# taylorlu/voicepuppet

Measured on AMD Instinct MI355X. Metric: PixReferNet G+D step frames/sec @256x256 bs=32, higher is better.
Workload: dtype bf16; 1 GPU; PixReferNet G+D training step (G + 3xD + VGG16-conv3_3 perceptual + TF-Adam x2), 256x256, ngf=ndf=64, global batch 32 = 32 per GPU; global_batch=32, per_gpu_batch=32, parallelism=dp1

## Files before the change

include/vp_hip.h:

```cpp
#ifndef VP_HIP_H_
#define VP_HIP_H_

#include <stddef.h>
#include <stdint.h>

#ifdef __cplusplus
extern "C" {
#endif

enum vp_status { VP_OK = 0, VP_ERR_ARG = -1, VP_ERR_HIP = -2, VP_ERR_WORKSPACE = -3, VP_ERR_STATE = -4 };
enum vp_dtype { VP_F32 = 0, VP_BF16 = 1 };
enum vp_act { VP_ACT_NONE = 0, VP_ACT_LRELU = 1, VP_ACT_RELU = 2, VP_ACT_TANH = 3, VP_ACT_SIGMOID = 4, VP_ACT_RELU6 = 5, VP_ACT_LEAKY = 6 };

int vp_version(void);
const char* vp_last_error(void);

typedef struct vp_pixrefer_desc {
  int batch;
  int height;
  int ngf, ndf;
  int dtype;
  int training;
  float l1_weight;
  float gan_weight;
  int per_sample_bn;
  int streams;
  int d_backward_fork;
  int d_beside_vgg;
} vp_pixrefer_desc;

size_t vp_pixrefer_desc_size(void);

typedef struct vp_pixrefer vp_pixrefer_t;

size_t vp_pixrefer_param_count(const vp_pixrefer_desc* d, int which);
int vp_pixrefer_param_info(const vp_pixrefer_desc* d, int which, int index, char* name, int name_cap,
                           size_t* offset, int* ndim, int64_t shape[4]);

size_t vp_pixrefer_workspace_bytes(const vp_pixrefer_desc* d);
int vp_pixrefer_validate_plan(const vp_pixrefer_desc* d);

int vp_pixrefer_create(const vp_pixrefer_desc* d, void* workspace, size_t workspace_bytes,
                       float* params_g, float* params_d, const float* params_vgg,
                       float* grads_g, float* grads_d, void* stream, vp_pixrefer_t** out);
void vp_pixrefer_destroy(vp_pixrefer_t* h);

int vp_pixrefer_params_changed(vp_pixrefer_t* h);
int vp_pixrefer_optimizer_stepped(vp_pixrefer_t* h);

int vp_pixrefer_forward(vp_pixrefer_t* h, const float* inputs, const float* fg_inputs,
                        const float* targets, const float* masks, void* stream);

int vp_pixrefer_forward_fg3(vp_pixrefer_t* h, const float* inputs, const float* fg_inputs3, const float* targets, void* stream);

int vp_pixrefer_backward(vp_pixrefer_t* h, void* stream);
int vp_pixrefer_backward_update(vp_pixrefer_t* h, float* m_g, float* v_g, float* m_d, float* v_d, int step_t_g, int step_t_d,
                                float lr, float beta1, float beta2, float eps, void* stream);

int vp_pixrefer_backward_d(vp_pixrefer_t* h, void* stream);
int vp_pixrefer_backward_g(vp_pixrefer_t* h, void* stream);
int vp_pixrefer_backward_d_fork(vp_pixrefer_t* h, void* stream);
int vp_pixrefer_backward_d_join(vp_pixrefer_t* h, void* stream);
void* vp_pixrefer_side_stream(vp_pixrefer_t* h);
int vp_reserve_streams(void);
void* vp_host_stream(void);
int vp_pixrefer_use_streams(vp_pixrefer_t* h, int n);
int vp_pixrefer_set_option(vp_pixrefer_t* h, const char* key, int value);
long long vp_pixrefer_counter(vp_pixrefer_t* h, const char* key);
int vp_pixrefer_fetch(vp_pixrefer_t* h, int what, void* dst, void* stream);
int vp_pixrefer_backward_g_stages(void);
int vp_pixrefer_backward_g_stage(vp_pixrefer_t* h, int stage, void* stream);
int vp_pixrefer_update_bucket(vp_pixrefer_t* h, int which, int bucket, float* m, float* v, int step_t, float lr, float beta1,
                              float beta2, float eps, void* stream);

int vp_pixrefer_tensor(vp_pixrefer_t* h, const char* name, void** ptr, int64_t shape[4], int* dtype);

int vp_profile_enable(int on);
size_t vp_profile_collect(char* json, size_t cap);

int vp_pixrefer_pack_frames(const unsigned char* example_frames, const unsigned char* current_frames, const int* crops,
                            int n, int img_size, float* inputs, float* fg_inputs, float* targets, float* masks, void* stream);

int vp_tune(const char* key, int value);
int vp_pixrefer_phase_ms(vp_pixrefer_t* h, float* ms, int cap);
float vp_pixrefer_mark_ms(vp_pixrefer_t* h, int from, int to);

int vp_grad_pack_bf16(const float* src, void* dst_bf16, size_t n, void* stream);
int vp_grad_unpack_bf16(const void* src_bf16, float* dst, size_t n, float scale, void* stream);

int vp_adam_tf(float* params, const float* grads, float* m, float* v, size_t n, int step_t,
               float lr, float beta1, float beta2, float eps, void* stream);

typedef struct vp_conv_desc {
  int kind;
  int n, h, w;
  int cin, cout;
  int ksize, stride, pad;
  int dtype;
  int in_act;
  int out_act;
} vp_conv_desc;

size_t vp_conv_workspace_bytes(const vp_conv_desc* d);
int vp_conv_fwd(const vp_conv_desc* d, const void* x, const float* in_scale, const float* in_shift,
                const float* w, const float* bias, void* y, void* workspace, void* stream);
int vp_conv_bwd_data(const vp_conv_desc* d, const void* dy, const float* w, void* dx, void* workspace, void* stream);
size_t vp_conv3x3_c64_bwd_data_pooled_workspace_bytes(const vp_conv_desc* d);
int vp_conv3x3_c64_bwd_data_pooled(const vp_conv_desc* d, const void* dy_pool, const unsigned char* code, const float* w, const void* ref,
                                   void* dx, void* workspace, int fused, void* stream);
int vp_conv_bwd_weight(const vp_conv_desc* d, const void* x, const float* in_scale, const float* in_shift,
                       const void* dy, float* dw, void* workspace, void* stream);

size_t vp_bn_workspace_bytes(int pixels, int c, int dtype);
int vp_bn_stats(const void* y, int pixels, int c, int dtype, const float* gamma, const float* beta, float eps,
                float* scale, float* shift, float* mean, float* rstd, void* workspace, void* stream);
int vp_bn_bwd(const void* y, const void* dz, void* dy, int pixels, int c, int dtype, const float* gamma,
              const float* mean, const float* rstd, float* dgamma, float* dbeta, void* workspace, void* stream);

typedef struct vp_logmel_desc {
  int sample_rate, num_mel_bins, win_length, hop_step, fft_length;
  float lower_hz, upper_hz;
  int batch, samples;
} vp_logmel_desc;
typedef struct vp_logmel vp_logmel_t;
size_t vp_logmel_workspace_bytes(const vp_logmel_desc* d);
int vp_logmel_frames(const vp_logmel_desc* d);
int vp_logmel_create(const vp_logmel_desc* d, void* workspace, size_t workspace_bytes, void* stream, vp_logmel_t** out);
void vp_logmel_destroy(vp_logmel_t* h);
int vp_logmel_forward(vp_logmel_t* h, const float* pcm, float* out, void* stream);

typedef struct vp_bfmnet_desc {
  int batch;
  int frames;
  int num_mel_bins;
  int trunk_dtype;
} vp_bfmnet_desc;
typedef struct vp_bfmnet vp_bfmnet_t;
size_t vp_bfmnet_param_count(void);
int vp_bfmnet_param_info(int index, char* name, int name_cap, size_t* offset, int* ndim, int64_t shape[4]);
size_t vp_bfmnet_workspace_bytes(const vp_bfmnet_desc* d);
int vp_bfmnet_create(const vp_bfmnet_desc* d, void* workspace, size_t workspace_bytes, const float* params,
                     void* stream, vp_bfmnet_t** out);
void vp_bfmnet_destroy(vp_bfmnet_t* h);
int vp_bfmnet_params_changed(vp_bfmnet_t* h);
int vp_bfmnet_forward(vp_bfmnet_t* h, const float* ears, const float* mfccs, const int* seq_len, float* out, void* stream);
int vp_bfmnet_set_decoder_dropout(vp_bfmnet_t* h, const float* mask0, const float* mask1);
int vp_bfmnet_tensor(vp_bfmnet_t* h, const char* name, void** ptr, int64_t shape[4]);

typedef struct vp_bfmstream_desc {
  int struct_bytes;
  int max_chunk_frames;
  int num_mel_bins;
  int trunk_dtype;
  int sample_rate;
  float lower_hz, upper_hz;
} vp_bfmstream_desc;
size_t vp_bfmstream_desc_size(void);
typedef struct vp_bfmstream vp_bfmstream_t;
int vp_bfmstream_context(const vp_bfmstream_desc* d, int* left_mel, int* right_mel, int* left_frames, int* right_frames, int* window_frames);
long long vp_bfmstream_frames_after(const vp_bfmstream_desc* d, long long samples, int finished);
size_t vp_bfmstream_workspace_bytes(const vp_bfmstream_desc* d);
int vp_bfmstream_create(const vp_bfmstream_desc* d, void* workspace, size_t workspace_bytes, const float* params, void* stream,
                        vp_bfmstream_t** out);
void vp_bfmstream_destroy(vp_bfmstream_t* h);
int vp_bfmstream_params_changed(vp_bfmstream_t* h);
int vp_bfmstream_reset(vp_bfmstream_t* h, void* stream);
int vp_bfmstream_ready(const vp_bfmstream_t* h, long long n_new_samples);
int vp_bfmstream_ready_finish(const vp_bfmstream_t* h);
int vp_bfmstream_push(vp_bfmstream_t* h, const float* pcm, long long n, const float* ears, float* coeff_out, void* stream);
int vp_bfmstream_finish(vp_bfmstream_t* h, const float* ears, float* coeff_out, void* stream);
int vp_bfmstream_tensor(vp_bfmstream_t* h, const char* name, void** ptr, int64_t shape[4]);
#define VP_BFMSTREAM_GROUP_MAX_SLOTS 128
typedef struct vp_bfmstream_group_desc {
  int struct_bytes;
  int slots;
  int max_chunk_frames;
  int num_mel_bins;
  int trunk_dtype;
  int sample_rate;
  float lower_hz, upper_hz;
} vp_bfmstream_group_desc;
size_t vp_bfmstream_group_desc_size(void);
typedef struct vp_bfmstream_group vp_bfmstream_group_t;
size_t vp_bfmstream_group_workspace_bytes(const vp_bfmstream_group_desc* d);
int vp_bfmstream_group_plan_info(const vp_bfmstream_group_desc* d, int bucket, int gemm, int info[8]);
int vp_bfmstream_group_create(const vp_bfmstream_group_desc* d, void* workspace, size_t workspace_bytes, const float* params, void* stream,
                              vp_bfmstream_group_t** out);
void vp_bfmstream_group_destroy(vp_bfmstream_group_t* h);
int vp_bfmstream_group_params_changed(vp_bfmstream_group_t* h);
// ... 379 lines not shown
```

voicepuppet_amd/_lib.py:

```python
import ctypes
import os

_HERE = os.path.dirname(os.path.abspath(__file__))
LIB_PATH = os.environ.get("VP_LIB", os.path.join(_HERE, "libvp_hip.so"))

VP_F32, VP_BF16 = 0, 1
ACT_NONE, ACT_LRELU, ACT_RELU, ACT_TANH, ACT_SIGMOID = 0, 1, 2, 3, 4
BN_PATH_PLANNER, BN_PATH_TWO_PASS, BN_PATH_ONE_LAUNCH = 0, 1, 2


class PixReferDesc(ctypes.Structure):
  _fields_ = [("batch", ctypes.c_int), ("height", ctypes.c_int), ("ngf", ctypes.c_int), ("ndf", ctypes.c_int),
              ("dtype", ctypes.c_int), ("training", ctypes.c_int), ("l1_weight", ctypes.c_float),
              ("gan_weight", ctypes.c_float), ("per_sample_bn", ctypes.c_int),
              ("streams", ctypes.c_int), ("d_backward_fork", ctypes.c_int), ("d_beside_vgg", ctypes.c_int)]


class ConvDesc(ctypes.Structure):
  _fields_ = [("kind", ctypes.c_int), ("n", ctypes.c_int), ("h", ctypes.c_int), ("w", ctypes.c_int),
              ("cin", ctypes.c_int), ("cout", ctypes.c_int), ("ksize", ctypes.c_int), ("stride", ctypes.c_int),
              ("pad", ctypes.c_int), ("dtype", ctypes.c_int), ("in_act", ctypes.c_int), ("out_act", ctypes.c_int)]


class LogMelDesc(ctypes.Structure):
  _fields_ = [("sample_rate", ctypes.c_int), ("num_mel_bins", ctypes.c_int), ("win_length", ctypes.c_int),
              ("hop_step", ctypes.c_int), ("fft_length", ctypes.c_int), ("lower_hz", ctypes.c_float),
              ("upper_hz", ctypes.c_float), ("batch", ctypes.c_int), ("samples", ctypes.c_int)]


class BfmNetDesc(ctypes.Structure):
  _fields_ = [("batch", ctypes.c_int), ("frames", ctypes.c_int), ("num_mel_bins", ctypes.c_int), ("trunk_dtype", ctypes.c_int)]


class BfmStreamDesc(ctypes.Structure):
  _fields_ = [("struct_bytes", ctypes.c_int), ("max_chunk_frames", ctypes.c_int), ("num_mel_bins", ctypes.c_int),
              ("trunk_dtype", ctypes.c_int), ("sample_rate", ctypes.c_int), ("lower_hz", ctypes.c_float), ("upper_hz", ctypes.c_float)]


class BfmStreamGroupDesc(ctypes.Structure):
  _fields_ = [("struct_bytes", ctypes.c_int), ("slots", ctypes.c_int), ("max_chunk_frames", ctypes.c_int), ("num_mel_bins", ctypes.c_int),
              ("trunk_dtype", ctypes.c_int), ("sample_rate", ctypes.c_int), ("lower_hz", ctypes.c_float), ("upper_hz", ctypes.c_float)]


BFMSTREAM_GROUP_MAX_SLOTS = 128


class PuppetDesc(ctypes.Structure):
  _fields_ = [("struct_bytes", ctypes.c_int), ("slots", ctypes.c_int), ("frame_batch", ctypes.c_int), ("img_size", ctypes.c_int),
              ("face_size", ctypes.c_int)]


PUPPET_MAX_SLOTS = 128


class JpegDesc(ctypes.Structure):
  _fields_ = [("struct_bytes", ctypes.c_uint32), ("max_frames", ctypes.c_int32), ("height", ctypes.c_int32), ("width", ctypes.c_int32),
              ("quality", ctypes.c_int32)]


class PngDesc(ctypes.Structure):
  _fields_ = [("struct_bytes", ctypes.c_uint32), ("max_frames", ctypes.c_int32), ("height", ctypes.c_int32), ("width", ctypes.c_int32),
              ("channels", ctypes.c_int32), ("filter", ctypes.c_int32)]


PNG_U8, PNG_F32 = 0, 1


class JpegDecDesc(ctypes.Structure):
  _fields_ = [("struct_bytes", ctypes.c_uint32), ("max_files", ctypes.c_int32), ("max_height", ctypes.c_int32), ("max_width", ctypes.c_int32),
              ("max_file_bytes", ctypes.c_int32), ("max_segments_per_file", ctypes.c_int32), ("bgr", ctypes.c_int32)]


class JpegDecFile(ctypes.Structure):
  _fields_ = [("meta_offset", ctypes.c_uint64), ("file_offset", ctypes.c_uint64), ("file_bytes", ctypes.c_int32), ("width", ctypes.c_int32),
              ("height", ctypes.c_int32), ("sampling", ctypes.c_int32), ("restart_interval", ctypes.c_int32), ("n_segments", ctypes.c_int32),
              ("tq", ctypes.c_uint8 * 3), ("td", ctypes.c_uint8 * 3), ("ta", ctypes.c_uint8 * 3), ("reserved", ctypes.c_uint8 * 3)]


JPEGDEC_META_BYTES = 6336


class PcmInDesc(ctypes.Structure):
  _fields_ = [("struct_bytes", ctypes.c_int), ("slots", ctypes.c_int), ("out_rate", ctypes.c_int), ("max_in_frames", ctypes.c_int),
              ("n_rates", ctypes.c_int), ("rates", ctypes.c_int * 8)]


PCMIN_MAX_SLOTS, PCMIN_MAX_CHANNELS = 128, 8
PCM_S16, PCM_F32 = 0, 1


class FrameMetricsDesc(ctypes.Structure):
  _fields_ = [("struct_bytes", ctypes.c_uint32), ("max_frames", ctypes.c_int32), ("max_height", ctypes.c_int32), ("max_width", ctypes.c_int32)]


FRAME_METRICS_MAX_FRAMES = 4096


class AviMuxDesc(ctypes.Structure):
  _fields_ = [("struct_bytes", ctypes.c_uint32), ("max_frames", ctypes.c_int32), ("row_bytes", ctypes.c_int32), ("slots", ctypes.c_int32),
              ("max_samples", ctypes.c_int32)]


AVIMUX_MAX_FRAMES, AVIMUX_MAX_SLOTS = 4096, 128


class TriptychDesc(ctypes.Structure):
  _fields_ = [("struct_bytes", ctypes.c_uint32), ("max_frames", ctypes.c_int32), ("size", ctypes.c_int32), ("face_size", ctypes.c_int32),
              ("max_side", ctypes.c_int32)]


TRIPTYCH_MAX_FRAMES, TRIPTYCH_MAX_SIZE = 4096, 1024


class BfmObserveOpts(ctypes.Structure):
  _fields_ = [("struct_bytes", ctypes.c_uint32), ("visibility", ctypes.c_int32), ("raster_scale", ctypes.c_int32), ("prefilter", ctypes.c_int32),
              ("depth_tol", ctypes.c_float)]


class BfmModel(ctypes.Structure):
  _fields_ = [("nver", ctypes.c_int), ("ntri", ctypes.c_int), ("meanshape", ctypes.c_void_p), ("idBase", ctypes.c_void_p),
              ("exBase", ctypes.c_void_p), ("meantex", ctypes.c_void_p), ("texBase", ctypes.c_void_p), ("tri", ctypes.c_void_p),
              ("point_buf", ctypes.c_void_p), ("center", ctypes.c_double * 3), ("focal", ctypes.c_double),
              ("image_center", ctypes.c_double), ("sh", ctypes.c_double * 5)]


_P = ctypes.c_void_p
_SIGNATURES = {
    "vp_version": (ctypes.c_int, []),
    "vp_last_error": (ctypes.c_char_p, []),
    "vp_pixrefer_param_count": (ctypes.c_size_t, [ctypes.POINTER(PixReferDesc), ctypes.c_int]),
    "vp_pixrefer_param_info": (ctypes.c_int, [ctypes.POINTER(PixReferDesc), ctypes.c_int, ctypes.c_int, ctypes.c_char_p,
                                              ctypes.c_int, ctypes.POINTER(ctypes.c_size_t), ctypes.POINTER(ctypes.c_int),
                                              ctypes.POINTER(ctypes.c_int64)]),
    "vp_pixrefer_workspace_bytes": (ctypes.c_size_t, [ctypes.POINTER(PixReferDesc)]),
    "vp_pixrefer_validate_plan": (ctypes.c_int, [ctypes.POINTER(PixReferDesc)]),
    "vp_pixrefer_create": (ctypes.c_int, [ctypes.POINTER(PixReferDesc), _P, ctypes.c_size_t, _P, _P, _P, _P, _P, _P,
                                          ctypes.POINTER(_P)]),
    "vp_pixrefer_destroy": (None, [_P]),
    "vp_pixrefer_params_changed": (ctypes.c_int, [_P]),
    "vp_pixrefer_optimizer_stepped": (ctypes.c_int, [_P]),
    "vp_pixrefer_forward": (ctypes.c_int, [_P, _P, _P, _P, _P, _P]),
    "vp_pixrefer_forward_fg3": (ctypes.c_int, [_P, _P, _P, _P, _P]),
    "vp_pixrefer_desc_size": (ctypes.c_size_t, []),
    "vp_pixrefer_backward": (ctypes.c_int, [_P, _P]),
    "vp_pixrefer_backward_update": (ctypes.c_int, [_P, _P, _P, _P, _P, ctypes.c_int, ctypes.c_int, ctypes.c_float, ctypes.c_float,
                                                   ctypes.c_float, ctypes.c_float, _P]),
    "vp_pixrefer_backward_d": (ctypes.c_int, [_P, _P]),
    "vp_pixrefer_backward_g": (ctypes.c_int, [_P, _P]),
    "vp_pixrefer_backward_d_fork": (ctypes.c_int, [_P, _P]),
    "vp_pixrefer_backward_d_join": (ctypes.c_int, [_P, _P]),
    "vp_pixrefer_backward_g_stages": (ctypes.c_int, []),
    "vp_pixrefer_backward_g_stage": (ctypes.c_int, [_P, ctypes.c_int, _P]),
    "vp_pixrefer_side_stream": (ctypes.c_void_p, [_P]),
    "vp_pixrefer_use_streams": (ctypes.c_int, [_P, ctypes.c_int]),
    "vp_pixrefer_set_option": (ctypes.c_int, [_P, ctypes.c_char_p, ctypes.c_int]),
    "vp_pixrefer_fetch": (ctypes.c_int, [_P, ctypes.c_int, _P, _P]),
    "vp_pixrefer_counter": (ctypes.c_longlong, [_P, ctypes.c_char_p]),
    "vp_crc32c": (ctypes.c_uint, [_P, ctypes.c_size_t, ctypes.c_uint]),
    "vp_pixrefer_phase_ms": (ctypes.c_int, [_P, ctypes.POINTER(ctypes.c_float), ctypes.c_int]),
    "vp_grad_pack_bf16": (ctypes.c_int, [_P, _P, ctypes.c_size_t, _P]),
    "vp_grad_unpack_bf16": (ctypes.c_int, [_P, _P, ctypes.c_size_t, ctypes.c_float, _P]),
    "vp_pixrefer_update_bucket": (ctypes.c_int, [_P, ctypes.c_int, ctypes.c_int, _P, _P, ctypes.c_int, ctypes.c_float, ctypes.c_float, ctypes.c_float,
                                                 ctypes.c_float, _P]),
    "vp_resize_paste_workspace_bytes": (ctypes.c_size_t, [ctypes.c_int, ctypes.c_int]),
    "vp_resize_paste_u8": (ctypes.c_int, [_P, ctypes.c_int, ctypes.c_int, ctypes.c_int, ctypes.c_int, ctypes.c_int, ctypes.c_int, _P, ctypes.c_int,
                                          ctypes.c_int, ctypes.c_int, ctypes.c_int, _P, _P]),
    "vp_resize_linear_table": (ctypes.c_int, [ctypes.c_int, ctypes.c_int, ctypes.c_int, _P, _P, _P, _P]),
    "vp_mm_workspace_bytes": (ctypes.c_size_t, [ctypes.c_int, ctypes.c_int, ctypes.c_int]),
    "vp_mm_fwd_f32": (ctypes.c_int, [_P, ctypes.c_int, _P, ctypes.c_int, ctypes.c_int, _P, _P, ctypes.c_int, ctypes.c_int, ctypes.c_int, ctypes.c_int, _P, _P]),
    "vp_mm_bwd_data_f32": (ctypes.c_int, [_P, ctypes.c_int, _P, ctypes.c_int, ctypes.c_int, _P, ctypes.c_int, ctypes.c_int, ctypes.c_int, ctypes.c_int,
                                          ctypes.c_int, _P, _P]),
    "vp_mm_bwd_weight_f32": (ctypes.c_int, [_P, ctypes.c_int, _P, ctypes.c_int, _P, ctypes.c_int, ctypes.c_int, ctypes.c_int, ctypes.c_int, _P, _P]),
    "vp_mm_packed_bytes": (ctypes.c_size_t, [ctypes.c_int, ctypes.c_int, ctypes.c_int, ctypes.c_int]),
    "vp_mm_pack_desc_bytes": (ctypes.c_size_t, []),
    "vp_mm_pack_desc": (ctypes.c_int, [ctypes.c_size_t, ctypes.c_int, ctypes.c_int, ctypes.c_int, ctypes.c_int, ctypes.c_int, ctypes.c_int, ctypes.c_size_t, _P]),
    "vp_mm_pack_table": (ctypes.c_int, [_P, ctypes.c_int, _P, _P, _P]),
    "vp_mm_fwd_f32_packed": (ctypes.c_int, [_P, ctypes.c_int, _P, _P, _P, ctypes.c_int, ctypes.c_int, ctypes.c_int, ctypes.c_int, _P, _P]),
    "vp_mm_bwd_data_f32_packed": (ctypes.c_int, [_P, ctypes.c_int, _P, _P, ctypes.c_int, ctypes.c_int, ctypes.c_int, ctypes.c_int, ctypes.c_int, _P, _P]),
    "vp_pixrefer_mark_ms": (ctypes.c_float, [_P, ctypes.c_int, ctypes.c_int]),
    "vp_profile_enable": (ctypes.c_int, [ctypes.c_int]),
    "vp_tune": (ctypes.c_int, [ctypes.c_char_p, ctypes.c_int]),
    "vp_reserve_streams": (ctypes.c_int, []),
    "vp_host_stream": (ctypes.c_void_p, []),
    "vp_pixrefer_pack_frames": (ctypes.c_int, [_P, _P, _P, ctypes.c_int, ctypes.c_int, _P, _P, _P, _P, _P]),
    "vp_profile_collect": (ctypes.c_size_t, [ctypes.c_char_p, ctypes.c_size_t]),
    "vp_pixrefer_tensor": (ctypes.c_int, [_P, ctypes.c_char_p, ctypes.POINTER(_P), ctypes.POINTER(ctypes.c_int64),
                                          ctypes.POINTER(ctypes.c_int)]),
    "vp_adam_tf": (ctypes.c_int, [_P, _P, _P, _P, ctypes.c_size_t, ctypes.c_int, ctypes.c_float, ctypes.c_float,
                                  ctypes.c_float, ctypes.c_float, _P]),
    "vp_conv_workspace_bytes": (ctypes.c_size_t, [ctypes.POINTER(ConvDesc)]),
    "vp_conv_fwd": (ctypes.c_int, [ctypes.POINTER(ConvDesc), _P, _P, _P, _P, _P, _P, _P, _P]),
    "vp_conv_bwd_data": (ctypes.c_int, [ctypes.POINTER(ConvDesc), _P, _P, _P, _P, _P]),
    "vp_conv_bwd_weight": (ctypes.c_int, [ctypes.POINTER(ConvDesc), _P, _P, _P, _P, _P, _P, _P]),
    "vp_conv3x3_c64_bwd_data_pooled_workspace_bytes": (ctypes.c_size_t, [ctypes.POINTER(ConvDesc)]),
    "vp_conv3x3_c64_bwd_data_pooled": (ctypes.c_int, [ctypes.POINTER(ConvDesc), _P, _P, _P, _P, _P, _P, ctypes.c_int, _P]),
    "vp_bn_workspace_bytes": (ctypes.c_size_t, [ctypes.c_int, ctypes.c_int, ctypes.c_int]),
    "vp_bn_stats": (ctypes.c_int, [_P, ctypes.c_int, ctypes.c_int, ctypes.c_int, _P, _P, ctypes.c_float, _P, _P, _P, _P, _P, _P]),
    "vp_logmel_workspace_bytes": (ctypes.c_size_t, [ctypes.POINTER(LogMelDesc)]),
    "vp_logmel_frames": (ctypes.c_int, [ctypes.POINTER(LogMelDesc)]),
    "vp_logmel_create": (ctypes.c_int, [ctypes.POINTER(LogMelDesc), _P, ctypes.c_size_t, _P, ctypes.POINTER(_P)]),
    "vp_logmel_destroy": (None, [_P]),
    "vp_logmel_forward": (ctypes.c_int, [_P, _P, _P, _P]),
    "vp_bfmnet_param_count": (ctypes.c_size_t, []),
    "vp_bfmnet_param_info": (ctypes.c_int, [ctypes.c_int, ctypes.c_char_p, ctypes.c_int, ctypes.POINTER(ctypes.c_size_t),
                                            ctypes.POINTER(ctypes.c_int), ctypes.POINTER(ctypes.c_int64)]),
    "vp_bfmnet_workspace_bytes": (ctypes.c_size_t, [ctypes.POINTER(BfmNetDesc)]),
    "vp_bfmnet_create": (ctypes.c_int, [ctypes.POINTER(BfmNetDesc), _P, ctypes.c_size_t, _P, _P, ctypes.POINTER(_P)]),
    "vp_bfmnet_destroy": (None, [_P]),
    "vp_bfmnet_params_changed": (ctypes.c_int, [_P]),
    "vp_bfmnet_forward": (ctypes.c_int, [_P, _P, _P, _P, _P, _P]),
    "vp_bfmnet_set_decoder_dropout": (ctypes.c_int, [_P, _P, _P]),
    "vp_bfmnet_tensor": (ctypes.c_int, [_P, ctypes.c_char_p, ctypes.POINTER(_P), ctypes.POINTER(ctypes.c_int64)]),
    "vp_bfmstream_desc_size": (ctypes.c_size_t, []),
    "vp_bfmstream_context": (ctypes.c_int, [ctypes.POINTER(BfmStreamDesc)] + [ctypes.POINTER(ctypes.c_int)] * 5),
    "vp_bfmstream_frames_after": (ctypes.c_longlong, [ctypes.POINTER(BfmStreamDesc), ctypes.c_longlong, ctypes.c_int]),
    "vp_bfmstream_workspace_bytes": (ctypes.c_size_t, [ctypes.POINTER(BfmStreamDesc)]),
    "vp_bfmstream_create": (ctypes.c_int, [ctypes.POINTER(BfmStreamDesc), _P, ctypes.c_size_t, _P, _P, ctypes.POINTER(_P)]),
    "vp_bfmstream_destroy": (None, [_P]),
    "vp_bfmstream_params_changed": (ctypes.c_int, [_P]),
    "vp_bfmstream_reset": (ctypes.c_int, [_P, _P]),
    "vp_bfmstream_ready": (ctypes.c_int, [_P, ctypes.c_longlong]),
    "vp_bfmstream_ready_finish": (ctypes.c_int, [_P]),
    "vp_bfmstream_push": (ctypes.c_int, [_P, _P, ctypes.c_longlong, _P, _P, _P]),
    "vp_bfmstream_finish": (ctypes.c_int, [_P, _P, _P, _P]),
    "vp_bfmstream_tensor": (ctypes.c_int, [_P, ctypes.c_char_p, ctypes.POINTER(_P), ctypes.POINTER(ctypes.c_int64)]),
    "vp_bfmstream_group_desc_size": (ctypes.c_size_t, []),
    "vp_puppet_desc_size": (ctypes.c_size_t, []),
    "vp_puppet_workspace_bytes": (ctypes.c_size_t, [ctypes.POINTER(PuppetDesc)]),
    "vp_puppet_create": (ctypes.c_int, [ctypes.POINTER(PuppetDesc), _P, ctypes.c_size_t, _P, ctypes.POINTER(_P)]),
    "vp_puppet_destroy": (None, [_P]),
    "vp_puppet_attach": (ctypes.c_int, [_P, ctypes.c_int, _P, _P, _P, ctypes.c_int, ctypes.c_int, ctypes.c_int, _P]),
    "vp_puppet_set_backgrounds": (ctypes.c_int, [_P, _P, ctypes.c_int]),
    "vp_puppet_splice": (ctypes.c_int, [_P, _P, ctypes.c_int, _P, ctypes.c_int, _P, _P]),
    "vp_puppet_condition": (ctypes.c_int, [_P, _P, ctypes.c_int, _P, ctypes.c_int, _P, _P, _P, _P]),
    "vp_puppet_tensor": (ctypes.c_int, [_P, ctypes.c_char_p, ctypes.POINTER(_P), ctypes.POINTER(ctypes.c_int64)]),
    "vp_puppet_slot_info": (ctypes.c_int, [_P, ctypes.c_int, ctypes.POINTER(ctypes.c_int)]),
    "vp_jpeg_desc_size": (ctypes.c_size_t, []),
    "vp_jpeg_workspace_bytes": (ctypes.c_size_t, [ctypes.POINTER(JpegDesc)]),
    "vp_jpeg_frame_capacity": (ctypes.c_size_t, [ctypes.POINTER(JpegDesc)]),
    "vp_jpeg_create": (ctypes.c_int, [ctypes.POINTER(JpegDesc), _P, ctypes.c_size_t, _P, ctypes.POINTER(_P)]),
    "vp_jpeg_encode": (ctypes.c_int, [_P, _P, ctypes.c_int, _P, ctypes.c_size_t, _P, _P]),
    "vp_jpeg_tensor": (ctypes.c_int, [_P, ctypes.c_char_p, ctypes.POINTER(_P), ctypes.POINTER(ctypes.c_int64)]),
    "vp_jpeg_header": (ctypes.c_int, [_P, _P, ctypes.c_size_t, ctypes.POINTER(ctypes.c_size_t)]),
    "vp_jpeg_destroy": (None, [_P]),
    "vp_png_desc_size": (ctypes.c_size_t, []),
    "vp_png_workspace_bytes": (ctypes.c_size_t, [ctypes.POINTER(PngDesc)]),
    "vp_png_frame_capacity": (ctypes.c_size_t, [ctypes.POINTER(PngDesc)]),
    "vp_png_rows_per_strip": (ctypes.c_int, [ctypes.POINTER(PngDesc)]),
    "vp_png_create": (ctypes.c_int, [ctypes.POINTER(PngDesc), _P, ctypes.c_size_t, _P, ctypes.POINTER(_P)]),
    "vp_png_encode": (ctypes.c_int, [_P, _P, ctypes.c_int, ctypes.c_int, ctypes.c_int, ctypes.c_int, _P, ctypes.c_size_t, _P, _P]),
    "vp_png_tensor": (ctypes.c_int, [_P, ctypes.c_char_p, ctypes.POINTER(_P), ctypes.POINTER(ctypes.c_int64)]),
    "vp_png_header": (ctypes.c_int, [_P, _P, ctypes.c_size_t, ctypes.POINTER(ctypes.c_size_t)]),
    "vp_png_destroy": (None, [_P]),
    "vp_jpegdec_desc_size": (ctypes.c_size_t, []),
    "vp_jpegdec_workspace_bytes": (ctypes.c_size_t, [ctypes.POINTER(JpegDecDesc)]),
    "vp_jpegdec_create": (ctypes.c_int, [ctypes.POINTER(JpegDecDesc), _P, ctypes.c_size_t, ctypes.POINTER(_P)]),
    "vp_jpegdec_destroy": (None, [_P]),
    "vp_jpegdec_decode": (ctypes.c_int, [_P, _P, ctypes.POINTER(JpegDecFile), ctypes.c_int, _P, ctypes.c_size_t, ctypes.c_size_t, _P, _P]),
    "vp_jpegdec_tensor": (ctypes.c_int, [_P, ctypes.c_char_p, ctypes.POINTER(_P), ctypes.POINTER(ctypes.c_int64)]),
    "vp_jpegdec_scan_workspace_bytes": (ctypes.c_size_t, [ctypes.POINTER(JpegDecDesc), ctypes.c_int]),
    "vp_jpegdec_enable_scan": (ctypes.c_int, [_P, _P, ctypes.c_size_t, ctypes.c_int, ctypes.c_int]),
    "vp_pcmin_desc_size": (ctypes.c_size_t, []),
    "vp_pcmin_ratio": (ctypes.c_int, [ctypes.c_int, ctypes.c_int] + [ctypes.POINTER(ctypes.c_int)] * 4),
    "vp_pcmin_bank": (ctypes.c_int, [ctypes.c_int, ctypes.c_int, _P]),
    "vp_pcmin_samples_after": (ctypes.c_longlong, [ctypes.c_int, ctypes.c_int, ctypes.c_longlong, ctypes.c_int]),
    "vp_pcmin_workspace_bytes": (ctypes.c_size_t, [ctypes.POINTER(PcmInDesc)]),
    "vp_pcmin_create": (ctypes.c_int, [ctypes.POINTER(PcmInDesc), _P, ctypes.c_size_t, _P, ctypes.POINTER(_P)]),
    "vp_pcmin_destroy": (None, [_P]),
    "vp_pcmin_open_slot": (ctypes.c_int, [_P, ctypes.c_int, ctypes.c_int, ctypes.c_int, ctypes.c_int, _P]),
    "vp_pcmin_ready": (ctypes.c_longlong, [_P, ctypes.POINTER(ctypes.c_longlong), ctypes.POINTER(ctypes.c_int), ctypes.POINTER(ctypes.c_longlong)]),
    "vp_pcmin_push": (ctypes.c_int, [_P, _P, ctypes.POINTER(ctypes.c_longlong), ctypes.POINTER(ctypes.c_int), _P, _P]),
    "vp_frame_metrics_desc_size": (ctypes.c_size_t, []),
    "vp_frame_metrics_workspace_bytes": (ctypes.c_size_t, [ctypes.POINTER(FrameMetricsDesc)]),
    "vp_frame_metrics_create": (ctypes.c_int, [ctypes.POINTER(FrameMetricsDesc), _P, ctypes.c_size_t, ctypes.POINTER(_P)]),
    "vp_frame_metrics_destroy": (None, [_P]),
# ... 178 lines not shown
```

voicepuppet_amd/csrc/conv_dispatch.h:

```cpp
#pragma once
#include <hip/hip_runtime.h>

#include "conv_args.h"

namespace vp {

enum ProfBytes {
  BYTES_DEFAULT,
  BYTES_ONE_CLASS,
  BYTES_F32_OUT,
};
constexpr int TILE_FROM_CFG = 0, TILE_ROWS_COUT = -1;

struct ConvKernelRow {
  int id;
  const char* name;
  int family;
  bool bf16_only;
  int& (*knob)();
  bool (*eligible)(const IgemmArgs&, int is_bf16);
  hipError_t (*launch)(const IgemmArgs&, int is_bf16, int cfg, hipStream_t);
  int prof_bc, prof_bp;
  ProfBytes prof_bytes;
};

const char* conv_kernel_name(int kern);
int conv_staging(int kern);
bool conv_kernel_ok(const IgemmArgs& a, int is_bf16);
int pick_conv_kernel(const IgemmArgs& v, int is_bf16);
hipError_t launch_igemm(const IgemmArgs& a, int is_bf16, int cfg, hipStream_t st);

}
```

voicepuppet_amd/csrc/conv_dispatch.hip:

```cpp
#include "conv_dispatch.h"

#include "conv_ops.h"
#include "conv_prof.h"
#include "errors.h"
#include "vp_common.h"

namespace vp {

typedef const IgemmArgs& Args;
hipError_t launch_igemm_generic(Args, int is_bf16, int cfg, hipStream_t);
hipError_t launch_igemm_patch(Args, int is_bf16, int bc, int bp, hipStream_t);
hipError_t launch_igemm_patch2(Args, int is_bf16, int bc, int bp, hipStream_t);
bool patch3_eligible(Args, int is_bf16); hipError_t launch_igemm_patch3(Args, int is_bf16, int bc, int bp, hipStream_t);
bool patch4_eligible(Args, int is_bf16); hipError_t launch_igemm_patch4(Args, hipStream_t);
hipError_t launch_igemm_smallp(Args, int is_bf16, hipStream_t);
bool conv_s2c64_eligible(Args, int is_bf16); hipError_t launch_conv_s2c64(Args, hipStream_t);
bool conv_cin8_eligible(Args, int is_bf16); hipError_t launch_conv_cin8(Args, hipStream_t);
bool conv_cout8_eligible(Args, int is_bf16); hipError_t launch_conv_cout8(Args, hipStream_t);
bool conv_dcout8_eligible(Args, int is_bf16); hipError_t launch_conv_dcout8(Args, hipStream_t);
bool conv_cout4_eligible(Args, int is_bf16); hipError_t launch_conv_cout4(Args, hipStream_t);
bool conv_c64_eligible(Args, int is_bf16); hipError_t launch_conv_c64(Args, hipStream_t);
bool conv_dc256_eligible(Args, int is_bf16); hipError_t launch_conv_dc256(Args, hipStream_t);
bool conv_dc64_eligible(Args, int is_bf16); hipError_t launch_conv_dc64(Args, hipStream_t);

#define VP_TILED(fn) [](Args a, int bf, int cfg, hipStream_t st) { int bc, bp; igemm_tile(cfg, &bc, &bp); return fn(a, bf, bc, bp, st); }
#define VP_BF16(fn) [](Args a, int, int, hipStream_t st) { return fn(a, st); }

static const ConvKernelRow kTable[] = {
    {CK_SMALLP, "smallp", CK_SMALLP, false, nullptr, nullptr, [](Args a, int bf, int, hipStream_t st) { return launch_igemm_smallp(a, bf, st); },
     TILE_FROM_CFG, 0, BYTES_DEFAULT},
    {CK_S2C64, "s2c64", CK_S2C64, true, nullptr, conv_s2c64_eligible, VP_BF16(launch_conv_s2c64), 128, 64, BYTES_DEFAULT},
    {CK_CIN8, "cin8", CK_IGEMM, true, nullptr, conv_cin8_eligible, VP_BF16(launch_conv_cin8), 64, 16, BYTES_ONE_CLASS},
    {CK_COUT8, "cout8", CK_IGEMM, true, nullptr, conv_cout8_eligible, VP_BF16(launch_conv_cout8), 16, 64, BYTES_ONE_CLASS},
    {CK_DCOUT8, "dcout8", CK_IGEMM, true, nullptr, conv_dcout8_eligible, VP_BF16(launch_conv_dcout8), 32, 64, BYTES_DEFAULT},
    {CK_COUT4, "cout4", CK_IGEMM, true, nullptr, conv_cout4_eligible, VP_BF16(launch_conv_cout4), 16, 16, BYTES_F32_OUT},
    {CK_C64, "c64", CK_PATCH, true, c64_knob, conv_c64_eligible, VP_BF16(launch_conv_c64), TILE_ROWS_COUT, 64, BYTES_DEFAULT},
    {CK_DC256, "dc256", CK_PATCH2, true, dc64_knob, conv_dc256_eligible, VP_BF16(launch_conv_dc256), 64, 128, BYTES_DEFAULT},
    {CK_DC64, "dc64", CK_PATCH2, true, dc64_knob, conv_dc64_eligible, VP_BF16(launch_conv_dc64), 64, 128, BYTES_DEFAULT},
    {CK_PATCH4, "patch4", CK_PATCH, true, patch4_knob, patch4_eligible, VP_BF16(launch_igemm_patch4), 128, 256, BYTES_DEFAULT},
    {CK_PATCH3, "patch3", CK_PATCH, false, patch3_knob, patch3_eligible, VP_TILED(launch_igemm_patch3), TILE_FROM_CFG, 0, BYTES_DEFAULT},
    {CK_PATCH, "patch", CK_PATCH, false, nullptr, nullptr, VP_TILED(launch_igemm_patch), TILE_FROM_CFG, 0, BYTES_DEFAULT},
    {CK_PATCH2, "patch2", CK_PATCH2, false, nullptr, nullptr, VP_TILED(launch_igemm_patch2), TILE_FROM_CFG, 0, BYTES_DEFAULT},
    {CK_IGEMM, "igemm", CK_IGEMM, false, nullptr, nullptr, launch_igemm_generic, TILE_FROM_CFG, 0, BYTES_DEFAULT},
};
#undef VP_TILED
#undef VP_BF16

static const ConvKernelRow* conv_kernel_row(int kern) {
  for (const ConvKernelRow& r : kTable) if (r.id == kern) return &r;
  return nullptr;
}
const char* conv_kernel_name(int kern) { const ConvKernelRow* r = conv_kernel_row(kern); return r ? r->name : "?"; }
int conv_staging(int kern) { const ConvKernelRow* r = conv_kernel_row(kern); return r ? r->family : CK_IGEMM; }

bool conv_kernel_ok(const IgemmArgs& a, int is_bf16) {
  if (a.pool_src && a.kern != CK_C64) return false;
  const ConvKernelRow* r = conv_kernel_row(a.kern);
  if (!r || (r->bf16_only && !is_bf16)) return false;
  return !r->eligible || r->eligible(a, is_bf16);
}

int pick_conv_kernel(const IgemmArgs& v, int is_bf16) {
  const int fam = conv_staging(v.kern);
  for (const ConvKernelRow& r : kTable) {
    if (r.id == r.family) { if (r.id == fam) return fam; continue; }
    if ((r.bf16_only && !is_bf16) || (r.knob && !r.knob())) continue;
    if (r.eligible(v, is_bf16)) return r.id;
  }
  return fam;
}

hipError_t launch_igemm(const IgemmArgs& a, int is_bf16, int cfg, hipStream_t st) {
  if (!conv_kernel_ok(a, is_bf16)) {
    set_err("launch_igemm: the arguments are outside the preconditions of the plan's kernel %s (%s, %d x %d x %d -> %d channels)",
            conv_kernel_name(a.kern), is_bf16 ? "bf16" : "f32", a.N, a.Hg, a.Wg, a.Cout);
    return hipErrorInvalidValue;
  }
  const ConvKernelRow& r = *conv_kernel_row(a.kern);
  int pbc = r.prof_bc, pbp = r.prof_bp;
  if (pbc == TILE_FROM_CFG) igemm_tile(cfg, &pbc, &pbp);
  else if (pbc == TILE_ROWS_COUT) pbc = a.Cout;
  const double Pn = (double)a.N * a.Hg * a.Wg * a.nclass;
  const double kreal = (double)a.ntaps * a.cin_real;
  const double es = is_bf16 ? 2 : 4;
  const double flops = 2.0 * Pn * a.Cout * kreal;
  const double xfull = (double)a.N * a.Hin * a.Win * a.cin_real;
  double bytes;
  if (r.prof_bytes == BYTES_ONE_CLASS) bytes = es * (xfull + kreal * a.Cout + Pn * a.Cout);
  else if (r.prof_bytes == BYTES_F32_OUT) bytes = es * (xfull + kreal * a.nclass * a.Cout) + 4.0 * Pn * a.Cout;
  else {
    const double xbytes = a.pool_src ? (es + 1) * ((double)a.N * (a.Hin / 2) * (a.Win / 2) * a.cin_real) : es * xfull;
    bytes = xbytes + es * (kreal * a.nclass * a.Cout + Pn * a.Cout);
  }
  ProfScope prof(r.name, is_bf16, pbc, pbp, flops, bytes, st);
  return r.launch(a, is_bf16, cfg, st);
}

}
```

voicepuppet_amd/csrc/conv_ops.h:

```cpp
#pragma once
#include <stdlib.h>
#include <string.h>

#include "launch.h"

namespace vp {

struct ConvGeomX : ConvGeom {
  int CoutT;
};

inline ConvGeomX make_geom(int kind, int ks, int stride, int pad, int N, int Hin, int Win, int Cin, int Cin_real, int Cout) {
  ConvGeomX g;
  g.kind = kind; g.ks = ks; g.stride = stride; g.pad = pad;
  g.N = N; g.Hin = Hin; g.Win = Win;
  if (kind == 0) { g.Hout = (Hin + 2 * pad - ks) / stride + 1; g.Wout = (Win + 2 * pad - ks) / stride + 1; }
  else { g.Hout = 2 * Hin; g.Wout = 2 * Win; }
  g.Cin = Cin; g.Cin_real = Cin_real; g.Cout = Cout;
  g.CoutT = Cout < 8 ? 8 : Cout;
  return g;
}

inline int kc_elems(int is_bf16) { return is_bf16 ? 32 : 16; }

inline int& wgrad_cost_knob(int i) { static int v[3] = {80, 15, 150}; return v[i]; }
inline int& plan_misc_knob(int i) { static int v[4] = {384, 8, 4, 512}; return v[i]; }
inline int& igemm_small_grid_knob() { static int v = 128; return v; }
inline int& thin_blocks_knob(int i) { static int v[4] = {1024, 512, 512, 512}; return v[i]; }

inline int pick_igemm_cfg(int rows, int P, int Kpad = 0) {
  if (P >= 96) {
    if (rows % 128 == 0 && igemm_small_grid_knob() > 0 && (long long)((P + 127) / 128) * (rows / 128) <= igemm_small_grid_knob()) return IG_64x128;
    if (rows % 256 == 0 && P >= 256 * 256 && Kpad >= 4096) return IG_256x256;
    if (rows % 128 == 0 && P >= 256 * 512) return IG_128x256;
    if (rows % 128 == 0) return IG_128x128;
    if (rows % 64 == 0) return IG_64x128;
    if (rows <= 16) return IG_16x128;
    return rows > 64 ? IG_128x128 : IG_64x128;
  }
  if (rows <= 64) return IG_64x32;
  return P > 16 ? IG_128x32 : IG_128x16;
}

constexpr int IGEMM_SPLITK_TARGET_DEFAULT = 64;
inline int& igemm_splitk_target_knob() { static int v = IGEMM_SPLITK_TARGET_DEFAULT; return v; }
inline int pick_igemm_splitk(int blocks, int nchunk) {
  const int target = igemm_splitk_target_knob();
  const int cap = plan_misc_knob(1);
  const int minchunk = plan_misc_knob(2);
  if (blocks >= 256 || blocks >= target) return 1;
  int s = (target + blocks - 1) / blocks;
  if (s > nchunk / minchunk) s = nchunk / minchunk;
  if (s > cap) s = cap;
  return s < 1 ? 1 : s;
}

inline void set_single_src(PixSrc& x, const void* p, int C, const float* a, const float* b, int act, int group_n) {
  x.ptr[0] = p; x.ptr[1] = nullptr; x.C[0] = C; x.C[1] = 0;
  x.aff_a[0] = a; x.aff_b[0] = b; x.aff_a[1] = nullptr; x.aff_b[1] = nullptr;
  x.act = act; x.group_n = group_n > 0 ? group_n : (1 << 30);
}

struct LaunchForm {
  bool bias = false, ref = false, xa_lrelu = false, xa_relu = false, x_affine = false;
  bool stats = false;
  int x_act = 0, ref_act = 0;
};

struct IgemmPlan {
  IgemmArgs a;
  int cfg;
  LaunchForm form;
  PackDesc pack;
  size_t pack_elems;
  size_t partial_bytes;
};

struct IgemmPin { int cfg, splitk; };

inline void finish_igemm(IgemmPlan& p, int rows, int is_bf16, const IgemmPin* pin = nullptr) {
  IgemmArgs& a = p.a;
  const int P = a.N * a.Hg * a.Wg;
  a.Kpad = round_up(a.ntaps * a.Cin, kc_elems(is_bf16));
  p.cfg = pick_igemm_cfg(rows, P, a.Kpad);
  if (!is_bf16 && a.ntaps == 1 && p.cfg == IG_128x128) {
    const long long b128 = (long long)((P + 127) / 128) * (rows / 128), b64 = 2 * b128;
    if (((b64 + 255) / 256) * 64 < ((b128 + 255) / 256) * 128) p.cfg = IG_64x128;
  }
  if (pin) p.cfg = pin->cfg;
  int bc, bp;
  igemm_tile(p.cfg, &bc, &bp);
  a.CoutPad = round_up(rows, bc);
  if (a.ntaps == 1) { a.log2Cin = 30; a.cin_mask = 0x3fffffff; }
  else { a.log2Cin = ilog2(a.Cin); a.cin_mask = a.Cin - 1; }
  const int blocks = ((P + bp - 1) / bp) * (a.CoutPad / bc) * a.nclass;
  a.splitk = pin ? pin->splitk : pick_igemm_splitk(blocks, a.Kpad / kc_elems(is_bf16));
  p.partial_bytes = a.splitk > 1 ? (size_t)a.nclass * a.splitk * P * a.CoutPad * sizeof(float) : 0;
  {
    const bool tc4 = p.cfg == IG_128x128 || p.cfg == IG_64x128 || p.cfg == IG_128x256 || p.cfg == IG_256x256;
    a.rowperm = (tc4 && rows % 64 == 0) ? 1 : 0;
    p.pack.perm = a.rowperm;
  }
  a.wp_rows = round_up(rows, 128);
  p.pack.rows_pad = a.wp_rows;
  p.pack.Kpad = a.Kpad;
  p.pack.kc = kc_elems(is_bf16);
  p.pack_elems = (size_t)a.nclass * a.wp_rows * a.Kpad;
}

inline int& patch_tiles_knob() { static int v = 7; return v; }
inline int& patch_small_knob() { static int v = 3; return v; }
inline int& patch_longk_knob() { static int v = 1; return v; }
inline int& patch3_knob() { static int v = 1; return v; }
inline int& wgrad_big_knob() { static int v = 1; return v; }
inline int& patch4_knob() { static int v = 1; return v; }
inline int& c64_knob() { static int v = 1; return v; }
inline int& pool_bwd_fused_knob() { static int v = 1; return v; }
inline int& cout1_knob() { static int v = 256; return v; }
inline int& wgrad1_rows_knob() { static int v = 512; return v; }
inline int& dc64_knob() { static int v = 1; return v; }
inline int& s2c64_knob() { static int v = 512; return v; }
inline int& s2c64_pair_knob() { static int v = 1; return v; }
constexpr int PATCH_MIN_BLOCKS_DEFAULT = 192;
inline int& patch_minblk_knob() { static int v = PATCH_MIN_BLOCKS_DEFAULT; return v; }

inline void patch_tile_hw(int bp, int* th, int* tw) { *th = bp == 128 ? 8 : 16; *tw = bp == 512 ? 32 : 16; }
inline int patch_tile_pixels(int bc) {
  const int k = patch_small_knob();
  if (bc == 256) return (k & 2) ? 128 : 256;
  return (k & 1) ? 256 : 512;
}

inline int patch_tile_rows(int rows, int on) {
  if ((on & 1) && rows % 256 == 0) return 256;
  if ((on & 2) && rows % 128 == 0) return 128;
  if ((on & 4) && rows % 64 == 0) return 64;
  return 0;
}

inline bool plan_patch_eligible(const IgemmPlan& p, int rows, int is_bf16, bool single_src, bool any_grid = false) {
  const int on = patch_tiles_knob();
  const int minblk = any_grid ? 0 : patch_minblk_knob();
  const IgemmArgs& a = p.a;
  const int kc = kc_elems(is_bf16);
  if (!on || !single_src || a.nclass != 1 || a.sh != 1 || a.sw != 1 || a.os != 1 || a.ntaps < 9 || a.Cin % kc || a.Cin < kc) return false;
  if (rows % 64 || a.Cout % 8 || a.ldY % 8 || a.Hg < 16 || a.Wg < 16 || a.Hof != a.Hg || a.Wof != a.Wg) return false;
  const bool p4 = patch4_knob() && is_bf16 && a.ntaps == 16 && rows % 128 == 0;
  if (!p4 && patch_longk_knob() && rows >= 512 && rows % 256 == 0 && a.ntaps * a.Cin >= 4096 && (long long)a.N * a.Hg * a.Wg >= 256 * 256) return false;
  const int bc = p4 ? 128 : patch_tile_rows(rows, on);
  if (!bc) return false;
  int th, tw;
  patch_tile_hw(p4 ? 256 : patch_tile_pixels(bc), &th, &tw);
  const long long blocks = (long long)a.N * ((a.Hg + th - 1) / th) * ((a.Wg + tw - 1) / tw) * (rows / bc);
  const long long p4min = (long long)a.ntaps * a.Cin >= 8192 ? 256 : 512;
  if (p4 && !any_grid && patch_minblk_knob() > 1) {
    if (blocks < p4min) return false;
  } else if (blocks < minblk) return false;
  if ((size_t)a.N * a.Hin * a.Win * a.Cin * (is_bf16 ? 2 : 4) >= 0x70000000ull) return false;
  int ks = 0;
  while (ks * ks < a.ntaps) ++ks;
  if (ks * ks != a.ntaps) return false;
  const int sh = a.taps[0].dh[ks] - a.taps[0].dh[0], sw = a.taps[0].dw[1] - a.taps[0].dw[0];
  if ((sh != 1 && sh != -1) || (sw != 1 && sw != -1)) return false;
  for (int t = 0; t < a.ntaps; ++t)
    if (a.taps[0].dh[t] != a.taps[0].dh[0] + (t / ks) * sh || a.taps[0].dw[t] != a.taps[0].dw[0] + (t % ks) * sw) return false;
  return true;
}
inline void plan_make_patch(IgemmPlan& p, int rows, int is_bf16) {
  IgemmArgs& a = p.a;
  const bool p4 = patch4_knob() && is_bf16 && a.ntaps == 16 && rows % 128 == 0;
  const int bc = p4 ? 128 : patch_tile_rows(rows, patch_tiles_knob());
  int ks = 0;
  while (ks * ks < a.ntaps) ++ks;
  a.kern = CK_PATCH; a.p_kw = ks;
  a.p_dhf = a.taps[0].dh[0]; a.p_dwf = a.taps[0].dw[0];
  a.p_dhs = a.taps[0].dh[ks] - a.taps[0].dh[0]; a.p_dws = a.taps[0].dw[1] - a.taps[0].dw[0];
  const int bp = p4 ? 256 : patch_tile_pixels(bc);
  p.cfg = bc == 256 ? (bp == 128 ? PATCH_256x128 : PATCH_256x256) : (bc == 128 ? (bp == 256 ? PATCH_128x256 : PATCH_128x512) : (bp == 256 ? PATCH_64x256 : PATCH_64x512));
  a.CoutPad = round_up(rows, bc);
  a.splitk = 1;
  p.partial_bytes = 0;
  a.rowperm = 1;
  p.pack.perm = 1;
  p.pack.kswap = 1;
}

inline int& patch_xcd_knob() { static int v = 0; return v; }
inline int& patch2_knob() { static int v = 1; return v; }
inline bool plan_patch2_eligible(const IgemmPlan& p, int rows, int is_bf16, int c0, int c1) {
  const IgemmArgs& a = p.a;
  const int kc = kc_elems(is_bf16);
  if (!patch2_knob() || a.nclass != 4 || a.ntaps != 4 || a.os != 2 || a.sh != 1 || a.sw != 1) return false;
  if (c0 + c1 != a.Cin || c0 % (2 * kc) || c1 % (2 * kc) || c0 < 2 * kc) return false;
  if (rows % 64 || rows > 128 || a.Cout % 8 || a.ldY % 8 || a.Hg < 16 || a.Wg < 16 || a.Hof != 2 * a.Hg || a.Wof != 2 * a.Wg) return false;
  const long long blocks = (long long)a.N * ((a.Hg + 15) / 16) * ((a.Wg + 15) / 16) * 4;
  if (blocks < patch_minblk_knob()) return false;
  const size_t cmax = c0 > c1 ? c0 : c1;
  if ((size_t)a.N * a.Hin * a.Win * cmax * (is_bf16 ? 2 : 4) >= 0x70000000ull) return false;
  for (int cls = 0; cls < 4; ++cls)
    for (int t = 0; t < 4; ++t)
      if (a.taps[cls].dh[t] != a.taps[cls].dh[3] + 1 - (t >> 1) || a.taps[cls].dw[t] != a.taps[cls].dw[3] + 1 - (t & 1)) return false;
  return true;
}
inline void plan_make_patch2(IgemmPlan& p, int rows, int is_bf16) {
  IgemmArgs& a = p.a;
// ... 11 lines not shown
inline int& smallp_knob() { static int v = 256; return v; }
inline bool plan_smallp_eligible(const IgemmPlan& p, int rows, int is_bf16, int c0, int c1) {
  const IgemmArgs& a = p.a;
  const int kc = kc_elems(is_bf16);
  const long long Pc = (long long)a.N * a.Hg * a.Wg;
  if (smallp_knob() <= 0 || Pc > smallp_knob() || a.ntaps > 16 || a.nclass > 4) return false;
  if (rows % 32 || a.Cout != rows || a.ldY % 8) return false;
  if (a.Cin < kc || (a.Cin & (a.Cin - 1)) || c0 + c1 != a.Cin || c0 % kc || c1 % kc) return false;
  if ((long long)a.N * a.Hin * a.Win * (c0 > c1 ? c0 : c1) >= (1ll << 30)) return false;
  return true;
}
inline int smallp_counters(const IgemmArgs& a) {
  const int PT = a.sp_npt * 16;
  const int Pc = a.N * a.Hg * a.Wg;
  return (a.CoutPad / 32) * a.nclass * ((Pc + PT - 1) / PT) + a.CoutPad / 32;
}
inline void plan_make_smallp(IgemmPlan& p, int rows, int is_bf16) {
  IgemmArgs& a = p.a;
  const int kc = kc_elems(is_bf16);
  const int Pc = a.N * a.Hg * a.Wg;
  a.kern = CK_SMALLP;
  a.sp_npt = Pc <= 16 ? 1 : (Pc <= 32 ? 2 : 4);
  p.cfg = a.sp_npt == 1 ? SMALLP_32x16 : (a.sp_npt == 2 ? SMALLP_32x32 : SMALLP_32x64);
  a.sp_lcpt = ilog2(a.Cin / kc);
  a.CoutPad = round_up(rows, 32);
  a.rowperm = 0; p.pack.perm = 0; p.pack.kswap = 0;
  int minchunks = 1 << 30;
  for (int cls = 0; cls < a.nclass; ++cls) {
    unsigned m = 0;
    for (int t = 0; t < a.ntaps; ++t) {
      bool okh = false, okw = false;
      for (int q = 0; q < a.Hg && !okh; ++q) { const int ih = q * a.sh + a.taps[cls].dh[t]; okh = ih >= 0 && ih < a.Hin; }
      for (int r = 0; r < a.Wg && !okw; ++r) { const int iw = r * a.sw + a.taps[cls].dw[t]; okw = iw >= 0 && iw < a.Win; }
      if (okh && okw) m |= 1u << t;
    }
    a.sp_mask[cls] = (unsigned short)m;
    const int chunks = __builtin_popcount(m) * (a.Cin / kc);
    if (chunks < minchunks) minchunks = chunks;
  }
  const int PT = a.sp_npt * 16;
  const int tiles = (a.CoutPad / 32) * a.nclass * ((Pc + PT - 1) / PT);
  const int target = plan_misc_knob(0);
  int s = (target + tiles - 1) / tiles;
  if (s > minchunks / 8) s = minchunks / 8;
  if (s > 64) s = 64;
  if (s < 1) s = 1;
  a.splitk = s;
  p.partial_bytes = s > 1 ? (size_t)s * tiles * PT * 32 * sizeof(float) : 0;
}

inline bool plan_s2c64_eligible(const IgemmPlan& p, int rows, int is_bf16, int c0, int c1) {
  const IgemmArgs& a = p.a;
  if (s2c64_knob() <= 0 || !is_bf16 || a.nclass != 1 || a.ntaps != 16 || a.os != 1 || a.sh != 2 || a.sw != 2) return false;
  if ((rows != 128 && rows != 256) || a.Cout != rows || a.ldY != 128 || a.Cin != 64 || c0 != 64 || c1 != 0 || a.Kpad != 1024) return false;
  if (a.Hg % 4 || a.Wg % 16 || a.Hin != 2 * a.Hg || a.Win != 2 * a.Wg || a.Hof != a.Hg || a.Wof != a.Wg) return false;
  for (int t = 0; t < 16; ++t)
    if (a.taps[0].dh[t] != (t >> 2) - 1 || a.taps[0].dw[t] != (t & 3) - 1) return false;
  if (a.N * (a.Hg / 4) * (a.Wg / 16) < s2c64_knob()) return false;
  return (size_t)a.N * a.Hin * a.Win * 64 * 2 < 0x70000000ull;
}
inline void plan_make_s2c64(IgemmPlan& p) {
  IgemmArgs& a = p.a;
  a.kern = CK_S2C64;
  p.cfg = IG_128x128;
  a.CoutPad = a.Cout; a.wp_rows = a.Cout; p.pack.rows_pad = a.Cout;
  p.pack_elems = (size_t)a.wp_rows * a.Kpad;
  a.splitk = 1; p.partial_bytes = 0;
  a.rowperm = 1; p.pack.perm = 1; p.pack.kswap = 0;
}

inline IgemmArgs launch_view(const IgemmPlan& p, const LaunchForm& f) {
  static char set[16] = {};
  IgemmArgs v = p.a;
  v.Y = set; v.zeros = set;
  if (v.split_c) v.Y2 = set;
  if (f.bias) v.bias = (const float*)set;
  if (f.ref) { v.ref = set; v.ref_act = f.ref_act; if (v.split_c) v.ref2 = set; }
  if (f.xa_lrelu) v.xa_lrelu = set;
  if (f.xa_relu) v.xa_relu = set;
  if (f.x_affine) v.x.aff_a[0] = (const float*)set;
  v.x.act = f.x_act;
  if (f.stats) v.bn_part = (double*)set;
  return v;
}

enum { FAM_SMALLP = 1, FAM_PATCH = 2, FAM_PATCH2 = 4, FAM_S2C64 = 8, FAM_ALL = 15 };

inline void plan_kernel(IgemmPlan& p, int rows, int is_bf16, int c0, int c1, unsigned fams, const LaunchForm& f, bool any_grid = false) {
  if ((fams & FAM_SMALLP) && plan_smallp_eligible(p, rows, is_bf16, c0, c1)) plan_make_smallp(p, rows, is_bf16);
  else if ((fams & FAM_PATCH) && plan_patch_eligible(p, rows, is_bf16, c1 == 0 && c0 == p.a.Cin, any_grid)) plan_make_patch(p, rows, is_bf16);
  else if ((fams & FAM_PATCH2) && plan_patch2_eligible(p, rows, is_bf16, c0, c1)) plan_make_patch2(p, rows, is_bf16);
  else if ((fams & FAM_S2C64) && plan_s2c64_eligible(p, rows, is_bf16, c0, c1)) plan_make_s2c64(p);
  p.form = f;
  p.a.x.C[0] = c0; p.a.x.C[1] = c1;
  p.a.kern = pick_conv_kernel(launch_view(p, f), is_bf16);
}

inline IgemmPlan plan_fwd(const ConvGeomX& g, size_t w_off, int is_bf16, const IgemmPin* pin = nullptr) {
  IgemmPlan p;
  memset(&p, 0, sizeof(p));
  IgemmArgs& a = p.a;
  a.N = g.N; a.Hin = g.Hin; a.Win = g.Win; a.Cin = g.Cin; a.cin_real = g.Cin_real;
  a.Cout = g.Cout; a.ldY = g.Cout; a.Hof = g.Hout; a.Wof = g.Wout;
  a.ref_group_n = 1 << 30;
  PackDesc& d = p.pack;
  d.src_off = w_off; d.rows_real = g.Cout; d.C = g.Cin; d.C_real = g.Cin_real;
  if (g.kind == 0) {
    a.Hg = g.Hout; a.Wg = g.Wout; a.sh = a.sw = g.stride; a.os = 1;
    a.ntaps = g.ks * g.ks; a.nclass = 1;
    for (int t = 0; t < a.ntaps; ++t) {
      a.taps[0].dh[t] = (int8_t)(t / g.ks - g.pad); a.taps[0].dw[t] = (int8_t)(t % g.ks - g.pad);
      d.kh[0][t] = (int8_t)(t / g.ks); d.kw[0][t] = (int8_t)(t % g.ks);
    }
    d.s_kh = g.ks * g.Cin_real * g.Cout; d.s_kw = g.Cin_real * g.Cout; d.s_ch = g.Cout; d.s_row = 1;
  } else {
    a.Hg = g.Hin; a.Wg = g.Win; a.sh = a.sw = 1; a.os = 2;
    a.ntaps = 4; a.nclass = 4;
    for (int cls = 0; cls < 4; ++cls) {
      const int ph = cls >> 1, pw = cls & 1;
      a.o0h[cls] = ph; a.o0w[cls] = pw;
      for (int t = 0; t < 4; ++t) {
        const int ta = t >> 1, tb = t & 1;
        a.taps[cls].dh[t] = (int8_t)(ph - ta); a.taps[cls].dw[t] = (int8_t)(pw - tb);
        d.kh[cls][t] = (int8_t)((1 - ph) + 2 * ta); d.kw[cls][t] = (int8_t)((1 - pw) + 2 * tb);
      }
    }
    d.s_kh = 4 * g.Cout * g.Cin_real; d.s_kw = g.Cout * g.Cin_real; d.s_row = g.Cin_real; d.s_ch = 1;
  }
  d.nclass = a.nclass; d.ntaps = a.ntaps;
  finish_igemm(p, g.Cout, is_bf16, pin);
  return p;
}

inline IgemmPlan plan_bwd_data(const ConvGeomX& g, size_t w_off, int row0, int rows, int rows_real, int ldX, int is_bf16) {
  IgemmPlan p;
  memset(&p, 0, sizeof(p));
  IgemmArgs& a = p.a;
  a.N = g.N; a.Hin = g.Hout; a.Win = g.Wout; a.Cin = g.CoutT; a.cin_real = g.Cout;
  a.Cout = rows; a.ldY = ldX; a.Hof = g.Hin; a.Wof = g.Win;
  a.ref_group_n = 1 << 30;
  PackDesc& d = p.pack;
  d.rows_real = rows_real; d.C = g.CoutT; d.C_real = g.Cout;
  if (g.kind == 0) {
    d.s_kh = g.ks * g.Cin_real * g.Cout; d.s_kw = g.Cin_real * g.Cout; d.s_row = g.Cout; d.s_ch = 1;
    if (g.stride == 1) {
      a.Hg = g.Hin; a.Wg = g.Win; a.sh = a.sw = 1; a.os = 1;
      a.ntaps = g.ks * g.ks; a.nclass = 1;
      for (int t = 0; t < a.ntaps; ++t) {
        const int kh = t / g.ks, kw = t % g.ks;
        a.taps[0].dh[t] = (int8_t)(g.pad - kh); a.taps[0].dw[t] = (int8_t)(g.pad - kw);
        d.kh[0][t] = (int8_t)kh; d.kw[0][t] = (int8_t)kw;
      }
    } else {
      a.Hg = g.Hout; a.Wg = g.Wout; a.sh = a.sw = 1; a.os = 2;
      a.ntaps = 4; a.nclass = 4;
      for (int cls = 0; cls < 4; ++cls) {
        const int ph = cls >> 1, pw = cls & 1;
        a.o0h[cls] = ph; a.o0w[cls] = pw;
        for (int t = 0; t < 4; ++t) {
          const int ta = t >> 1, tb = t & 1;
          a.taps[cls].dh[t] = (int8_t)(ph - ta); a.taps[cls].dw[t] = (int8_t)(pw - tb);
          d.kh[cls][t] = (int8_t)((1 - ph) + 2 * ta); d.kw[cls][t] = (int8_t)((1 - pw) + 2 * tb);
        }
      }
    }
  } else {
// ... 82 lines not shown
```

voicepuppet_amd/csrc/conv_patch2.hip:

```cpp
#include <stdlib.h>

#include "conv_ops.h"
#include "igemm_device.h"
#include "launch.h"
#include "patch_device.h"

namespace vp {

template <typename T, int WC, int WP, int TC, int TP, int TH, int TW>
using Patch2Geom = PatchGeom<T, WC, WP, TC, TP, TH, TW, 1, 4>;

template <typename T, int WC, int WP, int TC, int TP, int TH, int TW, int STATS, int OCC, bool TWOSRC>
__global__ __launch_bounds__(512, OCC) void igemm_patch2_kernel(const IgemmArgs a) {
  using G = Patch2Geom<T, WC, WP, TC, TP, TH, TW>;
  constexpr int NSTW = G::NSTW, NSTEP = 8;
  constexpr int E = G::E, KC = G::KC, NW = G::NW, JA = G::JA, PW = G::PW, JP = G::JP, PBUFB = G::PBUFB, WSTB = G::WSTB, WBASE = G::WBASE;
  static_assert(JP <= 4, "one patch DMA per tap step");
  extern __shared__ __attribute__((aligned(16))) char smem[];

  const int tid = threadIdx.x, lane = tid & 63;
  const int wave = __builtin_amdgcn_readfirstlane(tid >> 6);
  const int c_base = blockIdx.y * G::BC;
  const int cls = blockIdx.z;
  const PatchTile tile = patch_tile_origin<TH, TW>(a);
  const int n = tile.n, y0 = tile.y0, x0 = tile.x0;
  const int dh0 = a.taps[cls].dh[3], dw0 = a.taps[cls].dw[3];
  const unsigned es = sizeof(T);
  const int C0 = a.x.C[0], C1 = TWOSRC ? a.x.C[1] : 0;
  const int n0 = C0 / KC, nchunkc = (C0 + C1) / KC;

  __amdgpu_buffer_rsrc_t rsW = make_rsrc(reinterpret_cast<const T*>(a.Wp) + (size_t)cls * a.wp_rows * a.Kpad, 0xFFFFFFFFu);
  __amdgpu_buffer_rsrc_t rsX0 = make_rsrc(a.x.ptr[0], (unsigned)((size_t)a.N * a.Hin * a.Win * C0 * es));
  __amdgpu_buffer_rsrc_t rsX1 = make_rsrc(a.x.ptr[1] ? a.x.ptr[1] : a.x.ptr[0], (unsigned)((size_t)a.N * a.Hin * a.Win * C1 * es));

  unsigned pvo0[JP], pvo1[TWOSRC ? JP : 1];
#pragma unroll
  for (int j = 0; j < JP; ++j) {
    const int pp = (wave + NW * j) * 16 + (lane >> 2);
    const int py = pp / PW, px = pp - py * PW;
    const int ih = y0 + dh0 + py, iw = x0 + dw0 + px;
    const bool ok = pp < G::NPATCH && (unsigned)ih < (unsigned)a.Hin && (unsigned)iw < (unsigned)a.Win;
    const int piece = (lane & 3) ^ ((px >> 2) & 3);
    const int pix = (n * a.Hin + ih) * a.Win + iw;
    pvo0[j] = ok ? (unsigned)((pix * C0 + piece * E) * es) : DMA_OOB;
    if (TWOSRC) pvo1[TWOSRC ? j : 0] = ok ? (unsigned)((pix * C1 + piece * E) * es) : DMA_OOB;
  }
  const PatchWeightDma<G> wdma(c_base, wave, lane);
  const unsigned wstep = (unsigned)(a.wp_rows * KC * es);
  auto issue_w = [&](int u, int chunk, int stage) {
    wdma.issue(rsW, (unsigned)((3 - u) * nchunkc + chunk) * wstep, reinterpret_cast<uint4*>(smem + WBASE + stage * WSTB));
  };
  auto issue_p = [&](int chunk, int buf, int j) {
    uint4* lb = reinterpret_cast<uint4*>(smem + buf * PBUFB) + (wave + NW * j) * 64;
    if (!TWOSRC || chunk < n0) dma16_buf(rsX0, pvo0[j], (unsigned)(chunk * KC) * es, lb);
    else dma16_buf(rsX1, pvo1[TWOSRC ? j : 0], (unsigned)((chunk - n0) * KC) * es, lb);
  };

  const int wc = wave / WP, wpi = wave - wc * WP;
  const int blkA0 = wc * TC, blkB0 = wpi * TP;
  const int fi = lane & 15, fg = lane >> 4;
  const int aaddr = WBASE + (blkA0 * 64 + fi * 4 + (fg ^ rb_swz(fi))) * 16;
  int tb0[2][TP];
#pragma unroll
  for (int c = 0; c < 2; ++c)
#pragma unroll
    for (int q = 0; q < TP; ++q) {
      constexpr int BPR = TW / 16;
      const int pb = blkB0 + q;
      const int px = (pb % BPR) * 16 + fi + c;
      const int pp = (pb / BPR) * PW + px;
      tb0[c][q] = (pp << 6) + (((fg ^ (px >> 2)) & 3) << 4) + ((fg & 1) << 3);
    }

  f32x4 acc[TC][TP];
#pragma unroll
  for (int i = 0; i < TC; ++i)
#pragma unroll
    for (int j = 0; j < TP; ++j) acc[i][j] = (f32x4){0.f, 0.f, 0.f, 0.f};

#pragma unroll
  for (int j = 0; j < JP; ++j) issue_p(0, 0, j);
#pragma unroll
  for (int d = 0; d < NSTW - 1; ++d) issue_w(d, 0, d);

  for (int c = 0; c < nchunkc; c += 2) {
    const bool last_pair = c + 2 >= nchunkc;
    auto step = [&](auto uc) {
      constexpr int U = decltype(uc)::value;
      constexpr int cc = U / 4, u = U % 4, pr = u / 2, pc = u % 2, stage = U % NSTW;
      constexpr int PC0 = JP - JP / 2, PC1 = JP / 2;
      constexpr int NV = (NSTW - 2) * JA + (u == 0 ? 0 : u == 1 ? PC0 : PC0 + PC1);
      constexpr int NLAST = NV - (U + 1 >= NSTEP ? JA : 0) - (U + 2 >= NSTEP ? JA : 0);
      if (U >= NSTEP - 2 && last_pair) wait_vm<NLAST>();
      else wait_vm<NV>();
      __builtin_amdgcn_s_barrier();
      asm volatile("" ::: "memory");
      {
        constexpr int U3 = (U + NSTW - 1) % NSTEP;
        if (U + NSTW - 1 < NSTEP) issue_w(U3 % 4, c + U3 / 4, (U + NSTW - 1) % NSTW);
        else if (!last_pair) issue_w(U3 % 4, c + 2 + U3 / 4, (U + NSTW - 1) % NSTW);
      }
      if constexpr (u == 0) {
#pragma unroll
        for (int j = 0; j < PC0; ++j) issue_p(c + cc + 1, 1 - cc, j);
      } else if constexpr (u == 1) {
#pragma unroll
        for (int j = PC0; j < JP; ++j) issue_p(c + cc + 1, 1 - cc, j);
      }
      constexpr int NA = TC == 8 ? 4 : ((TC == 4 && OCC == 4) ? 2 : TC);
      patch_step_mma<T, TC, TP, NA, stage * WSTB, cc * PBUFB + pr * PW * 64, false>(aaddr, tb0[pc], acc);
    };
    static_steps(step, std::make_integer_sequence<int, NSTEP>{});
  }
  asm volatile("s_waitcnt vmcnt(0)" ::: "memory");

  staged_epilogue<T, TC, TP, G::BC, G::BP, G::NPASS, G::NT, STATS>(a, PatchTilePix<TW, true>{a, n, y0, x0, a.o0h[cls], a.o0w[cls]}, c_base, blkA0, blkB0,
                                                                   acc, smem, tile.bt, cls);
}

template <typename T, int WC, int WP, int TC, int TP, int TH, int TW, int OCC>
static hipError_t launch_patch2_t(const IgemmArgs& b, hipStream_t st) {
  const bool two = b.x.C[1] > 0;
  const bool bst = b.bst_y != nullptr;
  if (bst && two) return hipErrorInvalidValue;
  auto kern = bst ? igemm_patch2_kernel<T, WC, WP, TC, TP, TH, TW, 2, OCC, false>
            : b.bn_part ? (two ? igemm_patch2_kernel<T, WC, WP, TC, TP, TH, TW, 1, OCC, true> : igemm_patch2_kernel<T, WC, WP, TC, TP, TH, TW, 1, OCC, false>)
                        : (two ? igemm_patch2_kernel<T, WC, WP, TC, TP, TH, TW, 0, OCC, true> : igemm_patch2_kernel<T, WC, WP, TC, TP, TH, TW, 0, OCC, false>);
  return launch_patch_grid<Patch2Geom<T, WC, WP, TC, TP, TH, TW>>(kern, b, b.nclass, st);
}

hipError_t launch_igemm_patch2(const IgemmArgs& a, int is_bf16, int bc, int bp, hipStream_t st) {
  IgemmArgs b = a;
  b.vec_epi = 1;
  if (bp != 256) return hipErrorInvalidValue;
#define VP_PATCH2_GO(WC, WP, TC, TP, TH, TW, OCC) \
  (is_bf16 ? launch_patch2_t<bf16, WC, WP, TC, TP, TH, TW, OCC>(b, st) : launch_patch2_t<float, WC, WP, TC, TP, TH, TW, OCC>(b, st))
  if (bc == 128) return VP_PATCH2_GO(2, 4, 4, 4, 16, 16, 4);
  if (bc == 64) return VP_PATCH2_GO(2, 4, 2, 4, 16, 16, 4);
#undef VP_PATCH2_GO
  return hipErrorInvalidValue;
}

}
```

voicepuppet_amd/csrc/conv_patch3.hip:

```cpp
#include <stdlib.h>
#ifndef VP_P3_NO_NT
#define VP_NT_STORE 1
#endif
#ifndef VP_P3_ABL
#define VP_P3_ABL 0
#endif

#include <utility>

#include "conv_ops.h"
#include "igemm_device.h"
#include "launch.h"
#include "patch_device.h"

namespace vp {

template <typename T, int WC, int WP, int TC, int TP, int TH, int TW, int NSTW, int KW>
using Patch3Geom = PatchGeom<T, WC, WP, TC, TP, TH, TW, KW - 1, NSTW>;

template <typename T, int WC, int WP, int TC, int TP, int TH, int TW, int STATS, int OCC, int NSTW = 3, int KW = 3>
__global__ __launch_bounds__(512, OCC) void igemm_patch3_kernel(const IgemmArgs a) {
  using G = Patch3Geom<T, WC, WP, TC, TP, TH, TW, NSTW, KW>;
  constexpr int E = G::E, KC = G::KC, NW = G::NW, LA = NSTW - 1;
  constexpr int KS2 = KW * KW, TRIP = 2 * KS2;
  static_assert(TRIP % NSTW == 0 && NSTW >= 3, "ring stages");
  constexpr int JA = G::JA, PW = G::PW, JP = G::JP, PBUFB = G::PBUFB, WSTB = G::WSTB, WBASE = G::WBASE;
  static_assert(JP + LA <= KS2, "one patch DMA per tap step, none in the last LA steps of a chunk");
  extern __shared__ __attribute__((aligned(16))) char smem[];

  const int tid = threadIdx.x, lane = tid & 63;
  const int wave = __builtin_amdgcn_readfirstlane(tid >> 6);
  const int c_base = blockIdx.y * G::BC;
  const PatchTile tile = patch_tile_origin<TH, TW>(a, a.xcd_remap);
  const int n = tile.n, y0 = tile.y0, x0 = tile.x0;
  const bool flip = a.p_dhs < 0;
  const int dh0 = flip ? a.p_dhf - (KW - 1) : a.p_dhf, dw0 = flip ? a.p_dwf - (KW - 1) : a.p_dwf;
  const unsigned es = sizeof(T);
  const int C0 = a.x.C[0];
  const int nchunkc = C0 / KC;

  __amdgpu_buffer_rsrc_t rsW = make_rsrc(reinterpret_cast<const T*>(a.Wp), 0xFFFFFFFFu);
  __amdgpu_buffer_rsrc_t rsX = make_rsrc(a.x.ptr[0], (unsigned)((size_t)a.N * a.Hin * a.Win * C0 * es));

  unsigned pvo[JP];
#pragma unroll
  for (int j = 0; j < JP; ++j) {
    const int pp = (wave + NW * j) * 16 + (lane >> 2);
    const int py = pp / PW, px = pp - py * PW;
    const int ih = y0 + dh0 + py, iw = x0 + dw0 + px;
    const bool ok = pp < G::NPATCH && (unsigned)ih < (unsigned)a.Hin && (unsigned)iw < (unsigned)a.Win;
    const int piece = (lane & 3) ^ ((px >> 2) & 3);
    pvo[j] = ok ? (unsigned)((((n * a.Hin + ih) * a.Win + iw) * C0 + piece * E) * es) : DMA_OOB;
  }
  const PatchWeightDma<G> wdma(c_base, wave, lane);
  const unsigned wstep = (unsigned)(a.wp_rows * KC * es);
  auto issue_w = [&](int u, int chunk, int stage) {
    const int tap = flip ? KS2 - 1 - u : u;
    wdma.issue(rsW, (unsigned)(tap * nchunkc + chunk) * wstep, reinterpret_cast<uint4*>(smem + WBASE + stage * WSTB));
  };
  auto issue_p = [&](int chunk, int buf, int j) {
    uint4* lb = reinterpret_cast<uint4*>(smem + buf * PBUFB);
    dma16_buf(rsX, pvo[j], (unsigned)(chunk * KC) * es, lb + (wave + NW * j) * 64);
  };

  const int wc = wave / WP, wpi = wave - wc * WP;
  const int blkA0 = wc * TC, blkB0 = wpi * TP;
  const int fi = lane & 15, fg = lane >> 4;
  const int aaddr = WBASE + (blkA0 * 64 + fi * 4 + (fg ^ rb_swz(fi))) * 16;
  int tb0[KW][TP];
#pragma unroll
  for (int c = 0; c < KW; ++c)
#pragma unroll
    for (int q = 0; q < TP; ++q) {
      constexpr int BPR = TW / 16;
      const int pb = blkB0 + q;
      const int px = (pb % BPR) * 16 + fi + c;
      const int pp = (pb / BPR) * PW + px;
      tb0[c][q] = (pp << 6) + (((fg ^ (px >> 2)) & 3) << 4) + ((fg & 1) << 3);
    }

  f32x4 acc[TC][TP];
#pragma unroll
  for (int i = 0; i < TC; ++i)
#pragma unroll
    for (int j = 0; j < TP; ++j) acc[i][j] = (f32x4){0.f, 0.f, 0.f, 0.f};

#pragma unroll
  for (int j = 0; j < JP; ++j) issue_p(0, 0, j);
#pragma unroll
  for (int d = 0; d < LA; ++d) issue_w(d % KS2, d / KS2, d % NSTW);

  for (int c = 0; c < ((VP_P3_ABL & 16) ? 0 : nchunkc); c += 2) {
    const bool last_pair = c + 2 >= nchunkc;
    auto step = [&](auto uc) {
      constexpr int U = decltype(uc)::value;
      constexpr int cc = U / KS2, u = U % KS2, pr = u / KW, pc = u % KW, stage = U % NSTW;
      constexpr int NPIECE = [] { int n = 0; for (int k = 1; k <= LA; ++k) n += ((U + TRIP - k) % TRIP % KS2) < JP ? 1 : 0; return n; }();
      constexpr int NV = (LA - 1) * JA + NPIECE;
      constexpr int WLAST = (TRIP - 1 - U < LA - 1 ? TRIP - 1 - U : LA - 1);
#if !(VP_P3_ABL & 2)
      if (U + LA - 1 > TRIP - 1 && last_pair) wait_vm<WLAST * JA + NPIECE>();
      else wait_vm<NV>();
#endif
#if !(VP_P3_ABL & 1)
      __builtin_amdgcn_s_barrier();
#endif
      asm volatile("" ::: "memory");
#if !(VP_P3_ABL & 4)
      {
        constexpr int UL = (U + LA) % TRIP;
        if (U + LA < TRIP) issue_w(UL % KS2, c + UL / KS2, (U + LA) % NSTW);
        else if (!last_pair) issue_w(UL % KS2, c + 2 + UL / KS2, (U + LA) % NSTW);
      }
      if constexpr (u < JP) issue_p(c + cc + 1, 1 - cc, u);
#endif
      constexpr int NA = TC == 8 ? 4 : ((TC == 4 && OCC == 4) ? 2 : TC);
      patch_step_mma<T, TC, TP, NA, stage * WSTB, cc * PBUFB + pr * PW * 64, true>(aaddr, tb0[pc], acc);
    };
    static_steps(step, std::make_integer_sequence<int, TRIP>{});
  }
  asm volatile("s_waitcnt vmcnt(0)" ::: "memory");

#ifndef VP_P3_NO_FASTEPI
  constexpr int NPASS16 = G::BC == 64 ? epi_passes16(G::BC, G::BP, WP, G::RINGB) : 0;
#else
  constexpr int NPASS16 = 0;
#endif
  if (!(VP_P3_ABL & 8) || acc[0][0][0] == 1.2345f) staged_epilogue<T, TC, TP, G::BC, G::BP, G::NPASS, G::NT, STATS, NPASS16>(a, PatchTilePix<TW>{a, n, y0, x0}, c_base, blkA0, blkB0, acc, smem, tile.bt, 0);
}

template <typename T, int WC, int WP, int TC, int TP, int TH, int TW, int OCC, int NSTW = 3, int KW = 3>
static hipError_t launch_patch3_t(const IgemmArgs& b, hipStream_t st) {
  auto kern = b.bn_part ? igemm_patch3_kernel<T, WC, WP, TC, TP, TH, TW, 1, OCC, NSTW, KW> : igemm_patch3_kernel<T, WC, WP, TC, TP, TH, TW, 0, OCC, NSTW, KW>;
  if (b.bst_y) {
    if constexpr (KW == 4) kern = igemm_patch3_kernel<T, WC, WP, TC, TP, TH, TW, 2, OCC, NSTW, KW>;
    else return hipErrorInvalidValue;
  }
  return launch_patch_grid<Patch3Geom<T, WC, WP, TC, TP, TH, TW, NSTW, KW>>(kern, b, 1, st);
}

bool patch3_eligible(const IgemmArgs& a, int is_bf16) {
  const int kc = is_bf16 ? 32 : 16;
  return conv_staging(a.kern) == CK_PATCH && a.ntaps == 9 && a.p_kw == 3 && a.p_dhs == a.p_dws && (a.p_dhs == 1 || a.p_dhs == -1) && a.x.C[0] % (2 * kc) == 0 &&
         a.x.C[1] == 0;
}

bool patch4_eligible(const IgemmArgs& a, int is_bf16) {
  return is_bf16 && conv_staging(a.kern) == CK_PATCH && a.ntaps == 16 && a.p_kw == 4 && a.p_dhs == a.p_dws && (a.p_dhs == 1 || a.p_dhs == -1) &&
         a.x.C[0] % 64 == 0 && a.x.C[1] == 0 && a.CoutPad % 128 == 0 && !a.pool_out;
}
hipError_t launch_igemm_patch4(const IgemmArgs& a, hipStream_t st) {
  IgemmArgs b = a;
  b.vec_epi = 1;
  b.xcd_remap = patch_xcd_knob();
  return launch_patch3_t<bf16, 2, 4, 4, 4, 16, 16, 4, 4, 4>(b, st);
}

hipError_t launch_igemm_patch3(const IgemmArgs& a, int is_bf16, int bc, int bp, hipStream_t st) {
  IgemmArgs b = a;
  b.vec_epi = 1;
  b.xcd_remap = patch_xcd_knob();
#define VP_PATCH3_GO(WC, WP, TC, TP, TH, TW, OCC) \
  (is_bf16 ? launch_patch3_t<bf16, WC, WP, TC, TP, TH, TW, OCC>(b, st) : launch_patch3_t<float, WC, WP, TC, TP, TH, TW, OCC>(b, st))
#define VP_PATCH3_GO6(WC, WP, TC, TP, TH, TW, OCC) \
  (is_bf16 ? launch_patch3_t<bf16, WC, WP, TC, TP, TH, TW, OCC, 6>(b, st) : launch_patch3_t<float, WC, WP, TC, TP, TH, TW, OCC, 6>(b, st))
  if (bc == 256) return bp == 128 ? VP_PATCH3_GO(2, 4, 8, 2, 8, 16, 4) : VP_PATCH3_GO(2, 4, 8, 4, 16, 16, 2);
  if (bc == 128) return bp == 512 ? VP_PATCH3_GO(1, 8, 8, 4, 16, 32, 2) : VP_PATCH3_GO(2, 4, 4, 4, 16, 16, 4);
  if (bp == 512) return VP_PATCH3_GO(1, 8, 4, 4, 16, 32, 2);
  return VP_PATCH3_GO6(2, 4, 2, 4, 16, 16, 4);
#undef VP_PATCH3_GO6
#undef VP_PATCH3_GO
}

}
```

voicepuppet_amd/csrc/igemm_device.h:

```cpp
#pragma once
#include "conv_args.h"
#include "vp_common.h"

namespace vp {

__device__ __forceinline__ int rb_swz(int i) { return (0x78 >> ((i >> 1) & 6)) & 3; }

template <typename T, int TC, int TP, int BC, int BP>
__device__ __forceinline__ void mma_chunk_rb(const uint4* __restrict__ ldsA, const uint4* __restrict__ ldsB,
                                             int blkA0, int blkB0, int lane, f32x4 (&acc)[TC][TP]) {
  const int i = lane & 15, g = lane >> 4;
  const int so = i * 4 + (g ^ rb_swz(i));
  uint4 fa[TC], fb[TP];
#pragma unroll
  for (int t = 0; t < TC; ++t) fa[t] = ldsA[(blkA0 + t) * 64 + so];
#pragma unroll
  for (int t = 0; t < TP; ++t) fb[t] = ldsB[(blkB0 + t) * 64 + so];
#pragma unroll
  for (int tc = 0; tc < TC; ++tc)
#pragma unroll
    for (int tp = 0; tp < TP; ++tp) acc[tc][tp] = mma16<T>(fa[tc], fb[tp], acc[tc][tp]);
}

__device__ __forceinline__ void dma16(const void* src, uint4* lds_dst_wave_uniform) {
  __builtin_amdgcn_global_load_lds((const __attribute__((address_space(1))) void*)src,
                                   (__attribute__((address_space(3))) void*)lds_dst_wave_uniform, 16, 0, 0);
}

__device__ __forceinline__ __amdgpu_buffer_rsrc_t make_rsrc(const void* base, unsigned bytes) {
  return __builtin_amdgcn_make_buffer_rsrc(const_cast<void*>(base), (short)0, (int)bytes, 0x27000);
}
__device__ __forceinline__ void dma16_buf(__amdgpu_buffer_rsrc_t rsrc, unsigned voff, unsigned soff, uint4* lds_dst_wave_uniform) {
  __builtin_amdgcn_raw_ptr_buffer_load_lds(rsrc, (__attribute__((address_space(3))) void*)lds_dst_wave_uniform, 16, (int)voff, (int)soff, 0, 0);
}
constexpr unsigned DMA_OOB = 0xF0000000u;

template <typename F, typename = void> struct pix_has_pool { static constexpr bool value = false; };
template <typename F> struct pix_has_pool<F, decltype((void)F::HAS_POOL)> { static constexpr bool value = F::HAS_POOL; };

struct LinearPix {
  const IgemmArgs& a; int cls, p_base, P;
  __device__ __forceinline__ long long operator()(int row) const {
    const int pidx = p_base + row;
    if (pidx >= P) return -1;
    const int hw = a.Hg * a.Wg;
    const int n = pidx / hw, rem = pidx - n * hw, q = rem / a.Wg, r = rem - q * a.Wg;
    long long off = (((long long)n * a.Hof + (q * a.os + a.o0h[cls])) * a.Wof + (r * a.os + a.o0w[cls])) * a.ldY;
    return (off << 8) | (long long)(n / a.ref_group_n);
  }
};

constexpr int epi_passes(int BC, int BP, int WP, int ring_bytes) {
  for (int np = 1; np <= WP; np *= 2)
    if ((BP / np) * (BC * 4 + 16) + (BP / np) * 8 <= ring_bytes) return np;
  return WP;
}

constexpr int epi_passes16(int BC, int BP, int WP, int ring_bytes) {
  for (int np = 1; np <= WP; np *= 2)
    if ((BP / np) * (BC * 2 + 16) + (BP / np) * 8 <= ring_bytes) return np;
  return WP;
}

template <typename T, bool DUAL = false>
__device__ __forceinline__ void epi_store8(const IgemmArgs& a, long long ot, int c0, size_t off, float (&v)[8]) {
  void* Yp = a.Y;
  const void* refp = a.ref;
  int accu = a.accumulate, yf32 = a.y_f32;
  if constexpr (DUAL) {
    if (c0 >= a.split_c) {
      Yp = a.Y2; refp = a.ref2; accu = a.accumulate2; yf32 = a.y2_f32;
      c0 -= a.split_c; off -= (size_t)a.split_c;
    }
  }
  if (a.bias) {
#pragma unroll
    for (int e = 0; e < 8; ++e) v[e] += a.bias[c0 + e];
  }
  if (a.out_act != ACT_NONE) {
#pragma unroll
    for (int e = 0; e < 8; ++e) v[e] = act_apply(a.out_act, v[e]);
  }
  if (refp) {
    float z[8];
    const T* rp = reinterpret_cast<const T*>(refp) + off;
    if (sizeof(T) == 2) Elem<bf16>::unpack(*reinterpret_cast<const uint4*>(rp), z);
    else {
      Elem<float>::unpack(reinterpret_cast<const uint4*>(rp)[0], z);
      Elem<float>::unpack(reinterpret_cast<const uint4*>(rp)[1], z + 4);
    }
    if (a.ref_a) {
      const int goff = (int)(ot & 255) * a.Cout + c0;
#pragma unroll
      for (int e = 0; e < 8; ++e) z[e] = fmaf(a.ref_a[goff + e], z[e], a.ref_b[goff + e]);
    }
#pragma unroll
    for (int e = 0; e < 8; ++e) v[e] *= act_grad(a.ref_act, z[e]);
  }
  if (yf32 || sizeof(T) == 4) {
    float* yp = reinterpret_cast<float*>(Yp) + off;
    if (accu) {
      const float4 e0 = reinterpret_cast<const float4*>(yp)[0], e1 = reinterpret_cast<const float4*>(yp)[1];
      v[0] += e0.x; v[1] += e0.y; v[2] += e0.z; v[3] += e0.w; v[4] += e1.x; v[5] += e1.y; v[6] += e1.z; v[7] += e1.w;
    }
#ifdef VP_NT_STORE
#pragma unroll
    for (int e = 0; e < 8; ++e) __builtin_nontemporal_store(v[e], yp + e);
#else
    reinterpret_cast<float4*>(yp)[0] = make_float4(v[0], v[1], v[2], v[3]);
    reinterpret_cast<float4*>(yp)[1] = make_float4(v[4], v[5], v[6], v[7]);
#endif
  } else {
    bf16* yp = reinterpret_cast<bf16*>(Yp) + off;
    if (accu) {
      float e[8];
      Elem<bf16>::unpack(*reinterpret_cast<const uint4*>(yp), e);
#pragma unroll
      for (int k = 0; k < 8; ++k) v[k] += e[k];
    }
#ifdef VP_NT_STORE
    { const uint4 pk = Elem<bf16>::pack(v); __builtin_nontemporal_store(pk.x, reinterpret_cast<unsigned*>(yp)); __builtin_nontemporal_store(pk.y, reinterpret_cast<unsigned*>(yp) + 1);
      __builtin_nontemporal_store(pk.z, reinterpret_cast<unsigned*>(yp) + 2); __builtin_nontemporal_store(pk.w, reinterpret_cast<unsigned*>(yp) + 3); }
#else
    *reinterpret_cast<uint4*>(yp) = Elem<bf16>::pack(v);
#endif
  }
}


__device__ __forceinline__ unsigned pool_code_of(float v0, float v1, float v2, float v3) {
  unsigned best = 0;
  float m = v0;
  if (v1 > m) { m = v1; best = 1; }
  if (v2 > m) { m = v2; best = 2; }
  if (v3 > m) { m = v3; best = 3; }
  return m > 0.f ? 1u + best : 0u;
}

template <typename T, int TC, int TP, int BC, int BP, int NPASS, int NT, int STATS = 0, int NPASS16 = 0, bool DUAL = false, typename PixFn>
__device__ __forceinline__ void staged_epilogue(const IgemmArgs& a, const PixFn& pixfn, int c_base, int blkA0, int blkB0,
                                                f32x4 (&acc)[TC][TP], char* smem, int pt = 0, int cls = 0) {
  if constexpr (NPASS16 > 0 && sizeof(T) == 2 && STATS == 0) {
    if (!a.ref && !a.accumulate && !a.y_f32 && (a.out_act == ACT_NONE || a.out_act == ACT_RELU)) {
      constexpr int PITCHB = BC * 2 + 16, CGB = BC / 8, RPB = BP / NPASS16;
      static_assert(RPB % (TP * 16) == 0, "a wave's pixel rows must fall into one pass");
      const int tid = threadIdx.x, lane = tid & 63;
      long long* otab = reinterpret_cast<long long*>(smem + RPB * PITCHB);
#pragma unroll
      for (int ps = 0; ps < NPASS16; ++ps) {
        __syncthreads();
        if (tid < RPB) otab[tid] = pixfn(ps * RPB + tid);
        if (blkB0 * 16 >= ps * RPB && blkB0 * 16 < (ps + 1) * RPB) {
#pragma unroll
          for (int tc = 0; tc < TC; ++tc) {
            const int ch = tile_chan0(a.rowperm, blkA0 + tc, lane >> 4);
            float b4[4] = {0.f, 0.f, 0.f, 0.f};
            if (a.bias && c_base + ch < a.Cout) {
#pragma unroll
              for (int e = 0; e < 4; ++e) b4[e] = a.bias[c_base + ch + e];
            }
#pragma unroll
            for (int tp = 0; tp < TP; ++tp) {
              const int row = (blkB0 + tp) * 16 + (lane & 15) - ps * RPB;
              float v[4];
#pragma unroll
              for (int e = 0; e < 4; ++e) {
                v[e] = acc[tc][tp][e];
                if (a.bias) v[e] += b4[e];
                if (a.out_act != ACT_NONE) v[e] = act_apply(a.out_act, v[e]);
              }
              uint2 pk;
              pk.x = Elem<bf16>::pack2(v[0], v[1]); pk.y = Elem<bf16>::pack2(v[2], v[3]);
              *reinterpret_cast<uint2*>(smem + row * PITCHB + ch * 2) = pk;
            }
            __builtin_amdgcn_sched_barrier(0);
          }
        }
        __syncthreads();
        bool store_y = true;
        if constexpr (pix_has_pool<PixFn>::value) store_y = !(a.pool_out != nullptr && a.pool_only);
        if (store_y)
          for (int idx = tid; idx < RPB * CGB; idx += NT) {
            const int p = idx / CGB, cgp = idx - p * CGB;
            const long long ot = otab[p];
            const int c0 = c_base + cgp * 8;
            if (ot < 0 || c0 >= a.Cout) continue;
            const uint4 pk = *reinterpret_cast<const uint4*>(smem + p * PITCHB + cgp * 16);
            unsigned* yp = reinterpret_cast<unsigned*>(reinterpret_cast<bf16*>(a.Y) + (size_t)(ot >> 8) + c0);
#ifdef VP_NT_STORE
            __builtin_nontemporal_store(pk.x, yp); __builtin_nontemporal_store(pk.y, yp + 1);
            __builtin_nontemporal_store(pk.z, yp + 2); __builtin_nontemporal_store(pk.w, yp + 3);
#else
            *reinterpret_cast<uint4*>(yp) = pk;
#endif
          }
        if constexpr (pix_has_pool<PixFn>::value) {
          if (a.pool_out != nullptr) {
            static_assert(RPB % 32 == 0, "a pass must hold whole pairs of tile rows");
            constexpr int PR = RPB / 4;
            for (int idx = tid; idx < PR * CGB; idx += NT) {
              const int pp = idx / CGB, cgp = idx - pp * CGB;
              const int pyl = pp >> 3, pxl = pp & 7;
              const int c0 = c_base + cgp * 8;
              const long long po = pixfn.pool(ps * (RPB / 32) + pyl, pxl);
              if (po < 0 || c0 >= a.Cout) continue;
              const int r00 = pyl * 32 + pxl * 2;
              float m[8];
#pragma unroll
              for (int k = 0; k < 4; ++k) {
                const int rr = r00 + (k >> 1) * 16 + (k & 1);
                float v[8];
                Elem<bf16>::unpack(*reinterpret_cast<const uint4*>(smem + rr * PITCHB + cgp * 16), v);
#pragma unroll
                for (int e = 0; e < 8; ++e) m[e] = k == 0 ? v[e] : fmaxf(m[e], v[e]);
              }
              *reinterpret_cast<uint4*>(reinterpret_cast<bf16*>(a.pool_out) + po + c0) = Elem<bf16>::pack(m);
              if (a.pool_code) {
                float vv[4][8];
#pragma unroll
                for (int k = 0; k < 4; ++k)
                  Elem<bf16>::unpack(*reinterpret_cast<const uint4*>(smem + (r00 + (k >> 1) * 16 + (k & 1)) * PITCHB + cgp * 16), vv[k]);
                unsigned w[2] = {0u, 0u};
#pragma unroll
                for (int e = 0; e < 8; ++e) w[e >> 2] |= pool_code_of(vv[0][e], vv[1][e], vv[2][e], vv[3][e]) << (8 * (e & 3));
                *reinterpret_cast<uint2*>(a.pool_code + po + c0) = make_uint2(w[0], w[1]);
              }
            }
          }
        }
      }
      return;
    }
  }
  constexpr int PITCH = BC * 4 + 16;
  constexpr int CG = BC / 8;
  constexpr int RP = BP / NPASS;
  static_assert(RP % (TP * 16) == 0, "a wave's pixel rows must fall into one pass");
  const int tid = threadIdx.x, lane = tid & 63;
  long long* otab = reinterpret_cast<long long*>(smem + RP * PITCH);
  static_assert(STATS != 1 || NT % BC == 0, "column sums: whole thread groups per channel");
  static_assert(STATS != 2 || NT % CG == 0, "backward sums: a thread keeps one channel group");
  float bsum = 0.f, bsq = 0.f;
  float gs0[STATS == 2 ? 8 : 1], gs1[STATS == 2 ? 8 : 1];
  const T* gy = nullptr;
  if constexpr (STATS == 2) {
    int c0 = c_base + (tid % CG) * 8;
    const void* yb = a.bst_y;
    int ct = a.Cout;
    if constexpr (DUAL) {
      ct = a.split_c;
      if (c0 >= a.split_c) { yb = a.bst_y2; c0 -= a.split_c; }
    }
#pragma unroll
    for (int e = 0; e < 8; ++e) { gs0[e] = 0.f; gs1[e] = 0.f; }
    if (yb && c0 < ct) gy = reinterpret_cast<const T*>(yb);
  }
#pragma unroll
  for (int ps = 0; ps < NPASS; ++ps) {
    __syncthreads();
    if (tid < RP) otab[tid] = pixfn(ps * RP + tid);
    if (blkB0 * 16 >= ps * RP && blkB0 * 16 < (ps + 1) * RP) {
#pragma unroll
      for (int tp = 0; tp < TP; ++tp)
#pragma unroll
        for (int tc = 0; tc < TC; ++tc) {
          const int row = (blkB0 + tp) * 16 + (lane & 15) - ps * RP;
          const int ch = tile_chan0(a.rowperm, blkA0 + tc, lane >> 4);
          *reinterpret_cast<f32x4*>(smem + row * PITCH + ch * 4) = acc[tc][tp];
          __builtin_amdgcn_sched_barrier(0);
        }
    }
    __syncthreads();
    if constexpr (STATS == 1) {
      const int col = tid % BC;
      for (int rr = tid / BC; rr < RP; rr += NT / BC) {
        if (otab[rr] < 0) continue;
        float x = *reinterpret_cast<const float*>(smem + rr * PITCH + col * 4);
        if (sizeof(T) == 2) x = bf16_bits_to_f32(f32_to_bf16_bits(x));
        bsum += x; bsq = fmaf(x, x, bsq);
      }
    }
    bool store_y = true;
    if constexpr (pix_has_pool<PixFn>::value) store_y = !(a.pool_out != nullptr && a.pool_only);
    if (store_y)
    for (int idx = tid; idx < RP * CG; idx += NT) {
      const int p = idx / CG, cgp = idx - p * CG;
      const long long ot = otab[p];
      const int c0 = c_base + cgp * 8;
      if (ot < 0 || c0 >= a.Cout) continue;
      const size_t off = (size_t)(ot >> 8) + c0;
      float v[8];
      {
        const float4 v0 = *reinterpret_cast<const float4*>(smem + p * PITCH + cgp * 32);
        const float4 v1 = *reinterpret_cast<const float4*>(smem + p * PITCH + cgp * 32 + 16);
        v[0] = v0.x; v[1] = v0.y; v[2] = v0.z; v[3] = v0.w; v[4] = v1.x; v[5] = v1.y; v[6] = v1.z; v[7] = v1.w;
      }
      uint4 ry0 = make_uint4(0, 0, 0, 0), ry1 = make_uint4(0, 0, 0, 0);
      if constexpr (STATS == 2) {
        if (gy) {
          size_t yo = off;
          if constexpr (DUAL) { if (c0 >= a.split_c) yo -= (size_t)a.split_c; }
          ry0 = reinterpret_cast<const uint4*>(gy + yo)[0];
          if (sizeof(T) == 4) ry1 = reinterpret_cast<const uint4*>(gy + yo)[1];
        }
      }
      epi_store8<T, DUAL>(a, ot, c0, off, v);
      if constexpr (STATS == 2) {
        if (gy) {
          float fy[8];
          if (sizeof(T) == 2) Elem<bf16>::unpack(ry0, fy);
          else { Elem<float>::unpack(ry0, fy); Elem<float>::unpack(ry1, fy + 4); }
#pragma unroll
          for (int e = 0; e < 8; ++e) {
            const float d = sizeof(T) == 2 ? bf16_bits_to_f32(f32_to_bf16_bits(v[e])) : v[e];
            gs0[e] += d;
            gs1[e] = fmaf(d, fy[e], gs1[e]);
          }
        }
      }
    }
    if constexpr (pix_has_pool<PixFn>::value) {
      if (a.pool_out != nullptr) {
        static_assert(RP % 32 == 0, "a pass must hold whole pairs of tile rows");
        constexpr int PR = RP / 4;
        for (int idx = tid; idx < PR * CG; idx += NT) {
          const int pp = idx / CG, cgp = idx - pp * CG;
          const int pyl = pp >> 3, pxl = pp & 7;
          const int c0 = c_base + cgp * 8;
          const long long po = pixfn.pool(ps * (RP / 32) + pyl, pxl);
          if (po < 0 || c0 >= a.Cout) continue;
          const int r00 = pyl * 32 + pxl * 2;
          float m[8];
#pragma unroll
          for (int k = 0; k < 4; ++k) {
            const int rr = r00 + (k >> 1) * 16 + (k & 1);
            const float4 v0 = *reinterpret_cast<const float4*>(smem + rr * PITCH + cgp * 32);
            const float4 v1 = *reinterpret_cast<const float4*>(smem + rr * PITCH + cgp * 32 + 16);
            const float v[8] = {v0.x, v0.y, v0.z, v0.w, v1.x, v1.y, v1.z, v1.w};
#pragma unroll
            for (int e = 0; e < 8; ++e) m[e] = k == 0 ? v[e] : fmaxf(m[e], v[e]);
          }
          if (a.bias) {
            const float4 b0 = *reinterpret_cast<const float4*>(a.bias + c0), b1 = *reinterpret_cast<const float4*>(a.bias + c0 + 4);
            m[0] += b0.x; m[1] += b0.y; m[2] += b0.z; m[3] += b0.w; m[4] += b1.x; m[5] += b1.y; m[6] += b1.z; m[7] += b1.w;
          }
          if (a.out_act != ACT_NONE) {
#pragma unroll
            for (int e = 0; e < 8; ++e) m[e] = act_apply(a.out_act, m[e]);
          }
          if constexpr (sizeof(T) == 2) {
            if (a.pool_code) {
              float vv[4][8];
#pragma unroll
              for (int k = 0; k < 4; ++k) {
                const int rr = r00 + (k >> 1) * 16 + (k & 1);
                const float4 v0 = *reinterpret_cast<const float4*>(smem + rr * PITCH + cgp * 32);
                const float4 v1 = *reinterpret_cast<const float4*>(smem + rr * PITCH + cgp * 32 + 16);
                float v[8] = {v0.x, v0.y, v0.z, v0.w, v1.x, v1.y, v1.z, v1.w};
#pragma unroll
                for (int e = 0; e < 8; ++e) {
                  if (a.bias) v[e] += a.bias[c0 + e];
                  if (a.out_act != ACT_NONE) v[e] = act_apply(a.out_act, v[e]);
                }
                Elem<bf16>::unpack(Elem<bf16>::pack(v), vv[k]);
              }
              unsigned w[2] = {0u, 0u};
#pragma unroll
              for (int e = 0; e < 8; ++e) w[e >> 2] |= pool_code_of(vv[0][e], vv[1][e], vv[2][e], vv[3][e]) << (8 * (e & 3));
              *reinterpret_cast<uint2*>(a.pool_code + po + c0) = make_uint2(w[0], w[1]);
            }
          }
          if (sizeof(T) == 2) *reinterpret_cast<uint4*>(reinterpret_cast<bf16*>(a.pool_out) + po + c0) = Elem<bf16>::pack(m);
          else {
            float* o = reinterpret_cast<float*>(a.pool_out) + po + c0;
            reinterpret_cast<float4*>(o)[0] = make_float4(m[0], m[1], m[2], m[3]);
            reinterpret_cast<float4*>(o)[1] = make_float4(m[4], m[5], m[6], m[7]);
          }
        }
      }
    }
  }
  if constexpr (STATS == 2) {
    __syncthreads();
    float* red = reinterpret_cast<float*>(smem);
    {
      float* r0 = red + (tid / CG) * 2 * BC + (tid % CG) * 8;
#pragma unroll
      for (int e = 0; e < 8; ++e) { r0[e] = gs0[e]; r0[BC + e] = gs1[e]; }
    }
    __syncthreads();
    const int grp = pt / a.bn_tpg, chunk = cls * a.bn_tpg + (pt - grp * a.bn_tpg);
    for (int j = tid; j < 2 * BC; j += NT) {
      float t = 0.f;
      for (int m = 0; m < NT / CG; ++m) t += red[m * 2 * BC + j];
      int c = c_base + (j % BC), ct = a.Cout;
      double* part = a.bn_part;
      if constexpr (DUAL) {
        ct = a.split_c;
        if (c >= a.split_c) { part = a.bn_part2; c -= a.split_c; }
      }
      if (part && c < ct) part[((size_t)(grp * a.bn_nchunk + chunk) * 2 + j / BC) * ct + c] = (double)t;
    }
  }
  if constexpr (STATS == 1) {
    __syncthreads();
    float* red = reinterpret_cast<float*>(smem);
    red[(tid / BC) * 2 * BC + tid % BC] = bsum;
    red[(tid / BC) * 2 * BC + BC + tid % BC] = bsq;
    __syncthreads();
    if (tid < 2 * BC || (NT < 2 * BC && tid < BC)) {
      const int grp = pt / a.bn_tpg, chunk = cls * a.bn_tpg + (pt - grp * a.bn_tpg);
      for (int j = tid; j < 2 * BC; j += NT) {
        float t = 0.f;
        for (int m = 0; m < NT / BC; ++m) t += red[m * 2 * BC + j];
        const int c = c_base + (j % BC);
        if (c < a.Cout) a.bn_part[((size_t)(grp * a.bn_nchunk + chunk) * 2 + j / BC) * a.Cout + c] = (double)t;
      }
    }
  }
}

}
```

voicepuppet_amd/csrc/ops_api.hip:

```cpp
#include <string.h>

#include <string>

#include "conv_ops.h"
#include "errors.h"
#include "audio_args.h"
#include "launch.h"
#include "vp_common.h"
#include "workspace.h"

using namespace vp;

namespace {

bool conv_desc_ok(const vp_conv_desc* d) {
  if (!d || d->n < 1 || d->h < 1 || d->w < 1) return false;
  if (d->cin < 8 || (d->cin & (d->cin - 1))) return false;
  if (d->kind == 1 && (d->ksize != 4 || d->stride != 2 || d->pad != 1)) return false;
  if (d->kind != 0 && d->kind != 1) return false;
  if (d->ksize < 1 || d->ksize > 4 || d->stride < 1 || d->stride > 2) return false;
  if (d->kind == 0 && d->stride == 2 && (d->ksize != 4 || d->pad != 1 || (d->h & 1) || (d->w & 1))) return false;
  return d->dtype == VP_F32 || d->dtype == VP_BF16;
}

ConvGeomX geom_of(const vp_conv_desc* d) {
  return make_geom(d->kind, d->ksize, d->stride, d->pad, d->n, d->h, d->w, d->cin, d->cin, d->cout);
}

const void* zero_page(char* ws, size_t used, hipStream_t st) {
  char* z = ws + align256(used);
  (void)hipMemsetAsync(z, 0, 256, st);
  return z;
}

}

extern "C" {

int vp_pixrefer_pack_frames(const unsigned char* example_frames, const unsigned char* current_frames, const int* crops,
                            int n, int img_size, float* inputs, float* fg_inputs, float* targets, float* masks, void* stream) {
  if (!example_frames || !current_frames || !crops || !inputs || !fg_inputs || !targets || !masks || n < 1 || img_size < 2) {
    set_err("vp_pixrefer_pack_frames: bad argument");
    return VP_ERR_ARG;
  }
  FramePackArgs a;
  a.ex = example_frames; a.cur = current_frames; a.crops = crops;
  a.inputs = inputs; a.fg_inputs = fg_inputs; a.targets = targets; a.masks = masks;
  a.N = n; a.S = img_size;
  VP_HIP_CHECK(launch_frame_pack(a, (hipStream_t)stream));
  return VP_OK;
}

extern "C" void vp_phase_marks_enable(int on);

enum TuneRule {
  TUNE_PLAIN,
  TUNE_POSITIVE,
  TUNE_NEG_RESETS,
  TUNE_0_TO_4,
};
struct TuneRow { const char* key; int* knob; TuneRule rule; int dflt; };

int vp_tune(const char* key, int value) {
  if (!key) return VP_ERR_ARG;
  static const TuneRow rows[] = {
      {"patch_tiles", &patch_tiles_knob(), TUNE_PLAIN},
      {"patch_min_blocks", &patch_minblk_knob(), TUNE_NEG_RESETS, PATCH_MIN_BLOCKS_DEFAULT},
      {"patch_small_tiles", &patch_small_knob(), TUNE_PLAIN},
      {"patch_long_k_on_256", &patch_longk_knob(), TUNE_PLAIN},
      {"wgrad_tr", &wgrad_tr_knob(), TUNE_PLAIN},
      {"patch3", &patch3_knob(), TUNE_PLAIN},
      {"c64", &c64_knob(), TUNE_PLAIN},
      {"dc64", &dc64_knob(), TUNE_PLAIN},
      {"pool_bwd_fused", &pool_bwd_fused_knob(), TUNE_0_TO_4, 1},
      {"cout1_wgrad_rows", &wgrad1_rows_knob(), TUNE_POSITIVE},
      {"cout1_bwd", &cout1_knob(), TUNE_NEG_RESETS, 256},
      {"s2c64", &s2c64_knob(), TUNE_PLAIN},
      {"wgrad_big", &wgrad_big_knob(), TUNE_PLAIN},
      {"patch4", &patch4_knob(), TUNE_PLAIN},
      {"s2c64_pair", &s2c64_pair_knob(), TUNE_PLAIN},
      {"bfm_dwproj", &bfm_dwproj_knob(), TUNE_PLAIN},
      {"patch2", &patch2_knob(), TUNE_PLAIN},
      {"patch_xcd", &patch_xcd_knob(), TUNE_PLAIN},
      {"smallp_max_pixels", &smallp_knob(), TUNE_PLAIN},
      {"igemm_splitk_target", &igemm_splitk_target_knob(), TUNE_NEG_RESETS, IGEMM_SPLITK_TARGET_DEFAULT},
      {"wgrad_fixed_x10", &wgrad_cost_knob(0), TUNE_PLAIN},
      {"wgrad_slab_x100", &wgrad_cost_knob(1), TUNE_PLAIN},
      {"wgrad_slab_tile_x1000", &wgrad_cost_knob(2), TUNE_NEG_RESETS, 150},
      {"smallp_split_target", &plan_misc_knob(0), TUNE_PLAIN},
      {"igemm_splitk_cap", &plan_misc_knob(1), TUNE_PLAIN},
      {"igemm_splitk_minchunk", &plan_misc_knob(2), TUNE_PLAIN},
      {"wgrad_resident_blocks", &plan_misc_knob(3), TUNE_PLAIN},
      {"igemm_small_grid", &igemm_small_grid_knob(), TUNE_PLAIN},
      {"thin_blocks_cout8", &thin_blocks_knob(0), TUNE_POSITIVE},
      {"thin_blocks_dcout8", &thin_blocks_knob(1), TUNE_POSITIVE},
      {"thin_blocks_cout4", &thin_blocks_knob(2), TUNE_POSITIVE},
      {"thin_blocks_cin8", &thin_blocks_knob(3), TUNE_POSITIVE},
  };
  if (!strcmp(key, "phase_marks")) { vp_phase_marks_enable(value); return VP_OK; }
  for (const TuneRow& r : rows) {
    if (strcmp(key, r.key)) continue;
    if (r.rule == TUNE_POSITIVE && value <= 0) break;
    const bool reset = (r.rule == TUNE_NEG_RESETS && value < 0) || (r.rule == TUNE_0_TO_4 && (value < 0 || value > 4));
    *r.knob = reset ? r.dflt : value;
    return VP_OK;
  }
  set_err("vp_tune: unknown key %s", key);
  return VP_ERR_ARG;
}

static unsigned* smallp_counter_page(char* ws, size_t used, const IgemmArgs& a, hipStream_t st) {
  unsigned* c = (unsigned*)(ws + align256(used) + 256);
  (void)hipMemsetAsync(c, 0, (size_t)smallp_counters(a) * sizeof(unsigned), st);
  return c;
}

size_t vp_conv_workspace_bytes(const vp_conv_desc* d) {
  if (!conv_desc_ok(d)) return 0;
  const int bf = d->dtype == VP_BF16, es = bf ? 2 : 4;
  const ConvGeomX g = geom_of(d);
  size_t best = 0;
  {
    IgemmPlan p = plan_fwd(g, 0, bf);
    best = align256(p.pack_elems * es) + p.partial_bytes;
    plan_kernel(p, g.Cout, bf, d->cin, 0, FAM_SMALLP, LaunchForm{});
    if (p.a.kern == CK_SMALLP) {
      const size_t b = align256(p.pack_elems * es) + align256(p.partial_bytes) + 512 + (size_t)smallp_counters(p.a) * sizeof(unsigned);
      if (b > best) best = b;
    }
  }
  if ((d->cout & (d->cout - 1)) == 0 && d->cout >= 8) {
    IgemmPlan p = plan_bwd_data(g, 0, 0, d->cin, d->cin, d->cin, bf);
    size_t b = align256(p.pack_elems * es) + p.partial_bytes;
    if (b > best) best = b;
    plan_kernel(p, d->cin, bf, d->cout, 0, FAM_SMALLP, LaunchForm{});
    if (p.a.kern == CK_SMALLP) {
      b = align256(p.pack_elems * es) + align256(p.partial_bytes) + 512 + (size_t)smallp_counters(p.a) * sizeof(unsigned);
      if (b > best) best = b;
    }
    for (int plain = 0; plain < 2; ++plain) {
      WgradPlan w = plan_wgrad(g, bf, plain != 0);
      if (w.partial_bytes + 512 > best) best = w.partial_bytes + 512;
    }
  }
  return best + 1024;
}

int vp_conv_fwd(const vp_conv_desc* d, const void* x, const float* in_scale, const float* in_shift,
                const float* w, const float* bias, void* y, void* workspace, void* stream) {
  if (!conv_desc_ok(d) || !x || !w || !y || !workspace) { set_err("vp_conv_fwd: bad argument"); return VP_ERR_ARG; }
  const int bf = d->dtype == VP_BF16, es = bf ? 2 : 4;
  hipStream_t st = (hipStream_t)stream;
  const ConvGeomX g = geom_of(d);
  IgemmPlan p = plan_fwd(g, 0, bf);
  p.a.out_act = d->out_act;
  LaunchForm f;
  f.bias = bias != nullptr; f.x_affine = in_scale != nullptr; f.x_act = d->in_act;
  const bool plain = d->in_act == ACT_NONE && !in_scale;
  plan_kernel(p, g.Cout, bf, d->cin, 0, plain ? (FAM_SMALLP | FAM_PATCH | FAM_PATCH2 | (d->out_act == ACT_NONE ? FAM_S2C64 : 0)) : 0, f);
  char* ws = (char*)workspace;
  VP_HIP_CHECK(launch_pack_weights_one(p.pack, w, ws, bf, st));
  IgemmArgs a = p.a;
  set_single_src(a.x, x, d->cin, in_scale, in_shift, d->in_act, 0);
  a.Wp = ws;
  a.partial = (float*)(ws + align256(p.pack_elems * es));
  a.Y = y; a.bias = bias;
  a.zeros = zero_page(ws, align256(p.pack_elems * es) + p.partial_bytes, st);
  if (a.kern == CK_SMALLP) a.sp_cnt = smallp_counter_page(ws, align256(p.pack_elems * es) + p.partial_bytes, a, st);
  VP_HIP_CHECK(launch_igemm(a, bf, p.cfg, st));
  return VP_OK;
}

int vp_conv_bwd_data(const vp_conv_desc* d, const void* dy, const float* w, void* dx, void* workspace, void* stream) {
  if (!conv_desc_ok(d) || !dy || !w || !dx || !workspace) { set_err("vp_conv_bwd_data: bad argument"); return VP_ERR_ARG; }
  if (d->cout < 8 || (d->cout & (d->cout - 1))) { set_err("vp_conv_bwd_data: cout must be a power of two >= 8"); return VP_ERR_ARG; }
  const int bf = d->dtype == VP_BF16, es = bf ? 2 : 4;
  hipStream_t st = (hipStream_t)stream;
  const ConvGeomX g = geom_of(d);
  IgemmPlan p = plan_bwd_data(g, 0, 0, d->cin, d->cin, d->cin, bf);
  plan_kernel(p, d->cin, bf, d->cout, 0, FAM_SMALLP | FAM_PATCH | FAM_PATCH2, LaunchForm{});
  char* ws = (char*)workspace;
  VP_HIP_CHECK(launch_pack_weights_one(p.pack, w, ws, bf, st));
  IgemmArgs a = p.a;
  set_single_src(a.x, dy, d->cout, nullptr, nullptr, ACT_NONE, 0);
  a.Wp = ws;
  a.partial = (float*)(ws + align256(p.pack_elems * es));
  a.Y = dx;
  a.zeros = zero_page(ws, align256(p.pack_elems * es) + p.partial_bytes, st);
  if (a.kern == CK_SMALLP) a.sp_cnt = smallp_counter_page(ws, align256(p.pack_elems * es) + p.partial_bytes, a, st);
  VP_HIP_CHECK(launch_igemm(a, bf, p.cfg, st));
  return VP_OK;
}

static bool pooled_desc_ok(const vp_conv_desc* d) {
  return conv_desc_ok(d) && d->kind == 0 && d->ksize == 3 && d->stride == 1 && d->pad == 1 && d->dtype == VP_BF16 && d->cin == d->cout &&
         (d->cin == 64 || d->cin == 128) && d->h % 4 == 0 && d->w % 16 == 0 && d->h >= 16;
}

size_t vp_conv3x3_c64_bwd_data_pooled_workspace_bytes(const vp_conv_desc* d) {
  if (!pooled_desc_ok(d)) return 0;
  return align256(vp_conv_workspace_bytes(d)) + align256((size_t)d->n * d->h * d->w * d->cout * 2) + 256;
}

int vp_conv3x3_c64_bwd_data_pooled(const vp_conv_desc* d, const void* dy_pool, const unsigned char* code, const float* w, const void* ref,
                                   void* dx, void* workspace, int fused, void* stream) {
  if (!pooled_desc_ok(d) || !dy_pool || !code || !w || !ref || !dx || !workspace) { set_err("vp_conv3x3_c64_bwd_data_pooled: bad argument"); return VP_ERR_ARG; }
  hipStream_t st = (hipStream_t)stream;
  const ConvGeomX g = geom_of(d);
  IgemmPlan p = plan_bwd_data(g, 0, 0, d->cin, d->cin, d->cin, 1);
  LaunchForm f;
  f.ref = true; f.ref_act = ACT_RELU;
  plan_kernel(p, d->cin, 1, d->cout, 0, FAM_PATCH, f);
  if (p.a.kern != CK_C64) {
    set_err("vp_conv3x3_c64_bwd_data_pooled: %d x %d x %d x %d is planned on kernel %s, not c64", d->n, d->h, d->w, d->cin, conv_kernel_name(p.a.kern));
    return VP_ERR_ARG;
  }
  char* ws = (char*)workspace;
  VP_HIP_CHECK(launch_pack_weights_one(p.pack, w, ws, 1, st));
  IgemmArgs a = p.a;
  a.Wp = ws;
  a.partial = (float*)(ws + align256(p.pack_elems * 2));
  a.Y = dx;
  a.ref = ref; a.ref_act = ACT_RELU;
  a.zeros = zero_page(ws, align256(p.pack_elems * 2) + p.partial_bytes, st);
  if (fused) {
    set_single_src(a.x, dy_pool, d->cout, nullptr, nullptr, ACT_NONE, 0);
    a.pool_code = const_cast<unsigned char*>(code);
    a.pool_src = 1;
  } else {
    char* full = ws + align256(vp_conv_workspace_bytes(d));
    VP_HIP_CHECK(launch_maxpool_bwd_code(code, dy_pool, full, d->n, d->h, d->w, d->cout, 1, st));
    set_single_src(a.x, full, d->cout, nullptr, nullptr, ACT_NONE, 0);
  }
  VP_HIP_CHECK(launch_igemm(a, 1, p.cfg, st));
  return VP_OK;
}

int vp_conv_bwd_weight(const vp_conv_desc* d, const void* x, const float* in_scale, const float* in_shift,
                       const void* dy, float* dw, void* workspace, void* stream) {
  if (!conv_desc_ok(d) || !x || !dy || !dw || !workspace) { set_err("vp_conv_bwd_weight: bad argument"); return VP_ERR_ARG; }
  if (d->cout < 8 || (d->cout & (d->cout - 1))) { set_err("vp_conv_bwd_weight: cout must be a power of two >= 8"); return VP_ERR_ARG; }
  const int bf = d->dtype == VP_BF16;
  hipStream_t st = (hipStream_t)stream;
  const ConvGeomX g = geom_of(d);
  WgradPlan p = plan_wgrad(g, bf, !in_scale && d->in_act == ACT_NONE);
  WgradArgs a = p.a;
  PixSrc xs, ds;
  set_single_src(xs, x, d->cin, in_scale, in_shift, d->in_act, 0);
  set_single_src(ds, dy, d->cout, nullptr, nullptr, ACT_NONE, 0);
  if (d->kind == 0) { a.g = xs; a.d = ds; } else { a.g = ds; a.d = xs; }
  a.partial = (float*)workspace;
  a.dW = dw;
  a.zeros = zero_page((char*)workspace, p.partial_bytes, st);
  VP_HIP_CHECK(launch_wgrad(a, bf, p.cfg, st));
  return VP_OK;
}

size_t vp_bn_workspace_bytes(int pixels, int c, int dtype) {
  if (pixels < 1 || c < 8) return 0;
  const int nch = bn_nchunk(pixels, c, 1, dtype == VP_BF16);
  return (size_t)nch * 2 * c * sizeof(double) + 4 * (size_t)c * sizeof(float) + 1024;
}

static bool bn_ok(int pixels, int c, int dtype) {
  const int e = dtype == VP_BF16 ? 8 : 4;
  return pixels >= 1 && c >= e && c % e == 0 && 256 % (c / e) == 0 && (dtype == VP_F32 || dtype == VP_BF16);
}

int vp_bn_stats(const void* y, int pixels, int c, int dtype, const float* gamma, const float* beta, float eps,
                float* scale, float* shift, float* mean, float* rstd, void* workspace, void* stream) {
  if (!bn_ok(pixels, c, dtype) || !y || !gamma || !beta || !scale || !shift || !mean || !rstd || !workspace) {
    set_err("vp_bn_stats: bad argument");
    return VP_ERR_ARG;
  }
  BnArgs b;
  memset(&b, 0, sizeof(b));
// ... 390 lines not shown
```

voicepuppet_amd/csrc/plan_pixrefer.hip:

```cpp
#include <math.h>
#include <stdio.h>
#include <string.h>

#include <mutex>
#include <string>
#include <utility>
#include <vector>

#include "conv_ops.h"
#include "conv_prof.h"
#include "errors.h"
#include "launch.h"
#include "smallp_args.h"
#include "vp_common.h"
#include "workspace.h"

namespace vp {

thread_local char g_err[512] = "";
void set_err(const char* fmt, ...) {
  va_list ap;
  va_start(ap, fmt);
  vsnprintf(g_err, sizeof(g_err), fmt, ap);
  va_end(ap);
// ... 169 lines not shown
  L.g = make_geom(kind, ks, stride, pad, n.batch, t0.H, t0.W, cin, cin_real, cout);
  L.in_act = in_act; L.out_act = out_act; L.has_bn = has_bn;
  const std::string base = prefix + scope + "/";
  if (kind == 0) add_param(n, base + wname, {ks, ks, cin_real, cout}, &L.w_off);
  else add_param(n, base + wname, {4, 4, cout, cin_real}, &L.w_off);
  add_param(n, base + bname, {cout}, &L.b_off);
  if (has_bn) {
    add_param(n, base + "batch_normalization/gamma", {cout}, &L.gamma_off);
    add_param(n, base + "batch_normalization/beta", {cout}, &L.beta_off);
  }
  L.out = add_tensor(n, scope, n.batch, L.g.Hout, L.g.Wout, L.g.CoutT, has_bn, false);
  n.t[L.out].producer = (int)n.l.size();
  n.l.push_back(L);
  return L.out;
}

static void build_generator(Net& n, int N, int H, int ngf, int groups = 1) {
  n.batch = N; n.groups = groups;
  const int tin = add_tensor(n, "inputs", N, H, H, 8, false, true);
  const int tfg = add_tensor(n, "fg_inputs", N, H, H, 8, false, true);
  const char* CK = "conv2d/kernel"; const char* CB = "conv2d/bias";
  const char* DK = "conv2d_transpose/kernel"; const char* DB = "conv2d_transpose/bias";
  const std::string P = "generator/";
  int e1 = add_layer(n, P, "encoder_1", 0, 4, 2, 1, {tin}, 6, ngf, false, ACT_NONE, ACT_NONE, CK, CB);
  int e2 = add_layer(n, P, "encoder_2", 0, 4, 2, 1, {e1}, ngf, ngf * 2, true, ACT_LRELU, ACT_NONE, CK, CB);
  int e3 = add_layer(n, P, "encoder_3", 0, 4, 2, 1, {e2}, ngf * 2, ngf * 2, true, ACT_LRELU, ACT_NONE, CK, CB);
  int e4 = add_layer(n, P, "encoder_4", 0, 4, 2, 1, {e3}, ngf * 2, ngf * 4, true, ACT_LRELU, ACT_NONE, CK, CB);
  int f1 = add_layer(n, P, "encoder_fg_1", 0, 4, 2, 1, {tfg}, 3, ngf, false, ACT_NONE, ACT_NONE, CK, CB);
  int f2 = add_layer(n, P, "encoder_fg_2", 0, 4, 2, 1, {f1}, ngf, ngf * 2, true, ACT_LRELU, ACT_NONE, CK, CB);
  int f3 = add_layer(n, P, "encoder_fg_3", 0, 4, 2, 1, {f2}, ngf * 2, ngf * 2, true, ACT_LRELU, ACT_NONE, CK, CB);
  int f4 = add_layer(n, P, "encoder_fg_4", 0, 4, 2, 1, {f3}, ngf * 2, ngf * 4, true, ACT_LRELU, ACT_NONE, CK, CB);
  int m2 = add_layer(n, P, "merged_encoder_2", 0, 4, 2, 1, {e4, f4}, ngf * 8, ngf * 4, true, ACT_LRELU, ACT_NONE, CK, CB);
  int m3 = add_layer(n, P, "merged_encoder_3", 0, 4, 2, 1, {m2}, ngf * 4, ngf * 8, true, ACT_LRELU, ACT_NONE, CK, CB);
  int m4 = add_layer(n, P, "merged_encoder_4", 0, 4, 2, 1, {m3}, ngf * 8, ngf * 8, true, ACT_LRELU, ACT_NONE, CK, CB);
  int m5 = add_layer(n, P, "merged_encoder_5", 0, 4, 2, 1, {m4}, ngf * 8, ngf * 8, true, ACT_LRELU, ACT_NONE, CK, CB);
  int d5 = add_layer(n, P, "merged_decoder_5", 1, 4, 2, 1, {m5}, ngf * 8, ngf * 8, true, ACT_RELU, ACT_NONE, DK, DB);
  int d4 = add_layer(n, P, "merged_decoder_4", 1, 4, 2, 1, {d5, m4}, ngf * 16, ngf * 8, true, ACT_RELU, ACT_NONE, DK, DB);
  int d3 = add_layer(n, P, "merged_decoder_3", 1, 4, 2, 1, {d4, m3}, ngf * 16, ngf * 4, true, ACT_RELU, ACT_NONE, DK, DB);
  int d2 = add_layer(n, P, "merged_decoder_2", 1, 4, 2, 1, {d3, m2}, ngf * 8, ngf * 4, true, ACT_RELU, ACT_NONE, DK, DB);
  int c4 = add_layer(n, P, "merged2_decoder_4", 1, 4, 2, 1, {d2, e4}, ngf * 8, ngf * 2, true, ACT_RELU, ACT_NONE, DK, DB);
  int c3 = add_layer(n, P, "merged2_decoder_3", 1, 4, 2, 1, {c4, e3}, ngf * 4, ngf * 2, true, ACT_RELU, ACT_NONE, DK, DB);
  int c2 = add_layer(n, P, "merged2_decoder_2", 1, 4, 2, 1, {c3, e2}, ngf * 4, ngf, true, ACT_RELU, ACT_NONE, DK, DB);
  int d1 = add_layer(n, P, "decoder_1", 1, 4, 2, 1, {c2, e1}, ngf * 2, 4, false, ACT_RELU, ACT_NONE, DK, DB);
  n.t[d1].is_f32 = true;
  for (int f : {f1, f2, f3, f4}) n.l[n.t[f].producer].fg = true;
  n.i_me2 = n.t[m2].producer; n.i_md5 = n.t[d5].producer;
}

static void build_discriminator(Net& n, int N, int H, int ndf) {
  n.batch = 3 * N; n.groups = 3;
  const int tin = add_tensor(n, "d_inputs", 3 * N, H, H, 8, false, true);
  const char* CK = "conv2d/kernel"; const char* CB = "conv2d/bias";
  const std::string P = "discriminator/";
  int l1 = add_layer(n, P, "layer_1", 0, 4, 2, 1, {tin}, 6, ndf, false, ACT_NONE, ACT_NONE, CK, CB);
  int l2 = add_layer(n, P, "layer_2", 0, 4, 2, 1, {l1}, ndf, ndf * 2, true, ACT_LRELU, ACT_NONE, CK, CB);
  int l3 = add_layer(n, P, "layer_3", 0, 4, 2, 1, {l2}, ndf * 2, ndf * 4, true, ACT_LRELU, ACT_NONE, CK, CB);
  int l4 = add_layer(n, P, "layer_4", 0, 4, 1, 1, {l3}, ndf * 4, ndf * 8, true, ACT_LRELU, ACT_NONE, CK, CB);
  int l5 = add_layer(n, P, "layer_5", 0, 4, 1, 1, {l4}, ndf * 8, 1, false, ACT_LRELU, ACT_NONE, CK, CB);
  n.t[l5].is_f32 = true;
}

static void build_vgg(Net& n, int N, int H) {
  n.batch = 2 * N; n.groups = 1;
  const int tin = add_tensor(n, "v_inputs", 2 * N, H, H, 8, false, true);
  const std::string P = "vgg_16/";
  auto add_pool = [&](int k, int conv) {
    const Tens tc = n.t[conv];
    const int p = add_tensor(n, k ? "pool2" : "pool1", tc.N, tc.H / 2, tc.W / 2, tc.C, false, false);
    n.t[p].pool = k; n.t[p].pool_src = conv;
    n.l[tc.producer].pool = k; n.l[tc.producer].pool_t = p;
    return p;
  };
  int c11 = add_layer(n, P, "conv1/conv1_1", 0, 3, 1, 1, {tin}, 3, 64, false, ACT_NONE, ACT_RELU, "weights", "biases");
  int c12 = add_layer(n, P, "conv1/conv1_2", 0, 3, 1, 1, {c11}, 64, 64, false, ACT_NONE, ACT_RELU, "weights", "biases");
  const int p1 = add_pool(0, c12);
  int c21 = add_layer(n, P, "conv2/conv2_1", 0, 3, 1, 1, {p1}, 64, 128, false, ACT_NONE, ACT_RELU, "weights", "biases");
  int c22 = add_layer(n, P, "conv2/conv2_2", 0, 3, 1, 1, {c21}, 128, 128, false, ACT_NONE, ACT_RELU, "weights", "biases");
  const int p2 = add_pool(1, c22);
  int c31 = add_layer(n, P, "conv3/conv3_1", 0, 3, 1, 1, {p2}, 128, 256, false, ACT_NONE, ACT_RELU, "weights", "biases");
  int c32 = add_layer(n, P, "conv3/conv3_2", 0, 3, 1, 1, {c31}, 256, 256, false, ACT_NONE, ACT_RELU, "weights", "biases");
  add_layer(n, P, "conv3/conv3_3", 0, 3, 1, 1, {c32}, 256, 256, false, ACT_NONE, ACT_RELU, "weights", "biases");
}

static int epi_stat_chunks(const IgemmPlan& p, int batch, int groups);
static bool first_layer_shape(int bf16, const Net& n, const Layer& L) {
  if (!bf16 || L.has_bn || L.tapgemm || L.out_act != ACT_NONE) return false;
  const Tens& to = n.t[L.out];
  return to.need_act[ACT_LRELU] && !to.is_f32;
}
constexpr int BST_MAX_CHUNKS = 8192;

static void plan_net(Net& n, int bf16, bool training, bool want_wgrad, int alt_batch, size_t* scratch_max, bool fwd_halves = false) {
  size_t pk = 0;
  auto take = [&](IgemmPlan& p) {
    p.pack.dst_off = pk;
    pk += (p.pack_elems + 63) & ~(size_t)63;
    n.descs.push_back(p.pack);
    if (p.partial_bytes > *scratch_max) *scratch_max = p.partial_bytes;
  };
  for (Layer& L : n.l) {
    L.desc0 = n.descs.size();
    Tens& to = n.t[L.out];
    const int c0 = n.t[L.src[0]].C, c1 = L.nsrc > 1 ? n.t[L.src[1]].C : 0;
    L.tapgemm = training && L.g.kind == 0 && L.g.stride == 1 && L.g.ks == 4 && L.g.Cout == 1 && L.nsrc == 1 && !L.has_bn &&
                L.g.Cin == L.g.Cin_real;
    if (L.tapgemm) {
      ConvGeomX g1 = make_geom(0, 1, 1, 0, L.g.N, L.g.Hin, L.g.Win, L.g.Cin, L.g.Cin, 16);
      L.fwd = plan_fwd(g1, L.w_off, bf16);
      L.fwd.pack.s_row = L.g.Cin; L.fwd.pack.s_ch = 1; L.fwd.pack.s_kh = 0; L.fwd.pack.s_kw = 0;
      L.fwd.a.y_f32 = 1;
      plan_kernel(L.fwd, 16, bf16, L.g.Cin, 0, 0, LaunchForm{});
    } else {
      L.fwd = plan_fwd(L.g, L.w_off, bf16);
      L.fwd.a.ldY = to.is_f32 ? L.g.Cout : to.C; L.fwd.a.y_f32 = to.is_f32 ? 1 : 0; L.fwd.a.out_act = L.out_act;
      LaunchForm f;
      f.bias = !L.has_bn;
      if (first_layer_shape(bf16, n, L)) { f.xa_lrelu = true; f.xa_relu = to.need_act[ACT_RELU]; }
      const unsigned fams = (n.groups == 1 && alt_batch == 0 ? FAM_SMALLP : 0) | FAM_PATCH | FAM_PATCH2 |
                            (L.has_bn && L.out_act == ACT_NONE ? FAM_S2C64 : 0);
      plan_kernel(L.fwd, L.g.Cout, bf16, c0, c1, fams, f);
      const IgemmArgs& a = L.fwd.a;
      const bool own_rows = (a.kern == CK_DC256 && n.groups == 1) || a.kern == CK_S2C64;
      const int chunks = epi_stat_chunks(L.fwd, n.batch, n.groups);
      if (L.has_bn && !own_rows && chunks > 0 && L.g.Cout % 8 == 0 && a.ldY % 8 == 0 && !a.y_f32 &&
          (size_t)n.groups * chunks * 2 * to.C <= (size_t)1024 * 2 * 512) {
        L.fwd_stats = L.fwd.form.stats = true;
        L.fwd.a.kern = pick_conv_kernel(launch_view(L.fwd, L.fwd.form), bf16);
      }
    }
    take(L.fwd);
    L.pk_fwd = L.fwd.pack.dst_off;
    if (fwd_halves && alt_batch > 0 && !L.tapgemm && !L.has_bn) {
      ConvGeomX g2 = L.g;
      g2.N = alt_batch;
      L.fwd_half = plan_fwd(g2, L.w_off, bf16);
      L.fwd_half.a.ldY = to.C; L.fwd_half.a.out_act = L.out_act;
      LaunchForm f;
      f.bias = true;
      plan_kernel(L.fwd_half, g2.Cout, bf16, c0, c1, conv_staging(L.fwd.a.kern) == CK_PATCH ? FAM_PATCH : 0, f, true);
      const PackDesc &pa = L.fwd.pack, &pb = L.fwd_half.pack;
      if (L.fwd_half.a.splitk == 1) {
        if (pa.kswap != pb.kswap || pa.perm != pb.perm || pa.kc != pb.kc || pa.Kpad != pb.Kpad || pa.rows_pad != pb.rows_pad) {
          take(L.fwd_half);
          L.pk_fwd_half = L.fwd_half.pack.dst_off;
        } else {
          L.pk_fwd_half = L.pk_fwd;
        }
        L.has_fwd_half = true;
      }
    }
    if (!training) continue;
    int row0 = 0;
    for (int s = 0; s < L.nsrc; ++s) {
      const Tens& ts = n.t[L.src[s]];
      const int rows = ts.C;
      int rows_real = rows;
      if (ts.is_input) rows_real = L.g.Cin_real;
      L.need_bwd[s] = !ts.is_input || (n.groups == 3) || (n.l[0].g.ks == 3);
      if (L.need_bwd[s]) {
        LaunchForm f;
        f.ref_act = L.in_act != ACT_NONE ? L.in_act : (ts.producer >= 0 && n.l[ts.producer].out_act == ACT_RELU ? ACT_RELU : ACT_NONE);
        f.ref = !ts.is_input && f.ref_act != ACT_NONE;
        L.bwd[s] = plan_bwd_data(L.g, L.w_off, row0, rows, rows_real, ts.C, bf16);
        if (alt_batch > 0) {
          ConvGeomX g2 = L.g;
          g2.N = alt_batch;
          L.bwd_alt[s] = plan_bwd_data(g2, L.w_off, row0, rows, rows_real, ts.C, bf16);
// ... 209 lines not shown
  }
  h->scratch_bytes = smax + 256;
  h->params_dirty = true;
  h->vgg_dirty = true;
}

static bool valid_desc(const vp_pixrefer_desc* d) {
  if (!d) { set_err("pixrefer descriptor: null"); return false; }
  if (d->batch < 1 || d->height < 256 || d->height % 256 != 0) { set_err("pixrefer descriptor: batch %d / height %d (height must be a multiple of 256)", d->batch, d->height); return false; }
  if (d->ngf < 8 || (d->ngf & (d->ngf - 1)) || d->ndf < 8 || (d->ndf & (d->ndf - 1))) { set_err("pixrefer descriptor: ngf %d / ndf %d must be powers of two >= 8", d->ngf, d->ndf); return false; }
  if (d->ngf > 64 || d->ndf > 64) { set_err("pixrefer descriptor: ngf %d / ndf %d > 64 exceed the batch-norm workspace (512 channels)", d->ngf, d->ndf); return false; }
  if (!d->training && d->per_sample_bn && d->batch > 1024) { set_err("pixrefer descriptor: per-sample batch-norm supports at most 1024 frames per call (got %d)", d->batch); return false; }
  if (d->dtype != VP_F32 && d->dtype != VP_BF16) { set_err("pixrefer descriptor: dtype %d", d->dtype); return false; }
  if ((d->streams != 0 && d->streams != 1 && d->streams != 3 && d->streams != 4) || d->d_backward_fork < 0 || d->d_backward_fork > 3 || d->d_beside_vgg < 0 ||
      d->d_beside_vgg > 2) {
    set_err("pixrefer descriptor: schedule fields streams %d / d_backward_fork %d / d_beside_vgg %d", d->streams, d->d_backward_fork, d->d_beside_vgg);
    return false;
  }
  return true;
}

static char* at_sample(const Tens& t, const void* base, int sample0, int es) {
  return (char*)base + (size_t)sample0 * t.H * t.W * t.C * es;
}

static void fill_src(const Net& n, const Layer& L, PixSrc& x, int group_n, int sample0, int es) {
  for (int s = 0; s < 2; ++s) {
    x.ptr[s] = nullptr; x.C[s] = 0; x.aff_a[s] = nullptr; x.aff_b[s] = nullptr;
  }
  for (int s = 0; s < L.nsrc; ++s) {
    const Tens& t = n.t[L.src[s]];
    x.ptr[s] = at_sample(t, (L.in_act != ACT_NONE) ? t.xa[L.in_act] : t.y, sample0, es);
    x.C[s] = t.C;
  }
  x.act = ACT_NONE;
  x.group_n = group_n;
}

static Lane caller_lane(const vp_pixrefer* h, void* stream) {
  return Lane{(hipStream_t)stream, h->lane[LANE_CALLER].scratch, h->lane[LANE_CALLER].bn_partial};
}

static int after(hipEvent_t ev, hipStream_t from, hipStream_t to) {
  VP_HIP_CHECK(hipEventRecord(ev, from));
  VP_HIP_CHECK(hipStreamWaitEvent(to, ev, 0));
  return VP_OK;
}

static int run_pack(vp_pixrefer* h, Net& n, hipStream_t st) {
  if (n.descs.empty()) return VP_OK;
  VP_HIP_CHECK(launch_pack_weights(n.d_descs, (int)n.descs.size(), n.params, n.packed, h->bf16, st));
  return VP_OK;
}

static int run_bn_stats(vp_pixrefer* h, Net& n, Layer& L, int fused_chunks, const Lane& ln) {
  hipStream_t st = ln.s;
  Tens& t = n.t[L.out];
  BnArgs b;
  memset(&b, 0, sizeof(b));
  b.y = t.y; b.C = t.C; b.G = n.groups; b.Pg = (n.batch / n.groups) * t.H * t.W;
  b.nchunk = bn_nchunk(b.Pg, b.C, b.G, h->bf16);
  b.partial = ln.bn_partial;
  b.gamma = n.params + L.gamma_off; b.beta = n.params + L.beta_off;
  b.aff_a = t.bn.a; b.aff_b = t.bn.b; b.mu = t.bn.mu; b.rstd = t.bn.rstd;
  b.eps = 1e-5f;
  if (fused_chunks > 0) { b.nchunk = fused_chunks; VP_HIP_CHECK(launch_bn_finalize(b, st)); return VP_OK; }
  if (bn_small(b)) {
    VP_HIP_CHECK(launch_bn_small_fwd(b, t.xa[ACT_LRELU], t.xa[ACT_RELU], h->bf16, st));
    return 1;
  }
  VP_HIP_CHECK(launch_bn_stats(b, h->bf16, st));
  return VP_OK;
}

static bool plan_can_pool(const IgemmPlan& p) {
  if (conv_staging(p.a.kern) != CK_PATCH || (p.a.Hg & 1) || (p.a.Wg & 1)) return false;
  int bc, bp;
  igemm_tile(p.cfg, &bc, &bp);
  int th, tw;
  patch_tile_hw(bp, &th, &tw);
  return tw == 16 && th % 2 == 0;
}

static int epi_stat_chunks(const IgemmPlan& p, int batch, int groups) {
  const IgemmArgs& a = p.a;
  const int fam = conv_staging(a.kern);
  if (a.splitk != 1 || fam == CK_SMALLP || fam == CK_S2C64 || batch % groups) return 0;
  int bc, bp;
  igemm_tile(p.cfg, &bc, &bp);
  const int pg = (batch / groups) * a.Hg * a.Wg;
  if (!(fam || groups == 1 || pg % bp == 0)) return 0;
  int pth = 16, ptw = 16;
  patch_tile_hw(bp, &pth, &ptw);
  const int tpg = fam ? (batch / groups) * ((a.Hg + pth - 1) / pth) * ((a.Wg + ptw - 1) / ptw) : (pg + bp - 1) / bp;
  return a.nclass * tpg;
}

static int run_layer_fwd_half(vp_pixrefer* h, Net& n, Layer& L, int half, const Lane& ln, void* pool_out = nullptr, bool pool_only = false,
                              unsigned char* pool_code = nullptr) {
  IgemmArgs a = L.fwd_half.a;
  a.pool_out = pool_out;
  a.pool_only = pool_out && pool_only ? 1 : 0;
  a.pool_code = a.pool_only ? pool_code : nullptr;
  const int nb = a.N;
  fill_src(n, L, a.x, nb, half * nb, h->es);
  a.Wp = n.packed + L.pk_fwd_half * h->es;
  Tens& to = n.t[L.out];
  a.Y = at_sample(to, to.y, half * nb, h->es);
  a.bias = n.params + L.b_off;
  a.partial = nullptr;
  a.zeros = h->zeros;
  profile_tag((L.scope + (half ? ":fwd1" : ":fwd0")).c_str());
  VP_HIP_CHECK(launch_igemm(a, h->bf16, L.fwd_half.cfg, ln.s));
  return VP_OK;
}

static bool first_layer_acts_fused(const vp_pixrefer* h, const Net& n, const Layer& L) {
  return first_layer_shape(h->bf16, n, L) && L.fwd.a.kern == CK_CIN8;
}

static SmallPArgs smallp_args(const IgemmArgs& a, unsigned* cnt, const Lane& ln) {
  SmallPArgs sp;
  memset(&sp, 0, sizeof(sp));
  sp.g = a;
  sp.g.sp_cnt = cnt;
  for (int c = 0; c < 4; ++c) sp.tap_mask[c] = a.sp_mask[c];
  sp.slab = a.partial; sp.cnt = cnt; sp.part = ln.bn_partial;
  return sp;
}

static void smallp_bn_bwd(SmallPArgs& sp, Net& n, Tens& t) {
  const Layer& Lp = n.l[t.producer];
  sp.mode = SP_BWD_BN;
  if (t.hi) { sp.hi = 1; sp.dy_out = t.dz; }
  sp.bn_y = t.y; sp.bn_mu = t.bn.mu; sp.bn_rstd = t.bn.rstd; sp.bn_gamma = n.params + Lp.gamma_off;
  sp.c1 = t.bn.c1; sp.c2 = t.bn.c2;
  sp.dgamma = n.grads + Lp.gamma_off; sp.dbeta = n.grads + Lp.beta_off; sp.dbias_zero = n.grads + Lp.b_off;
  t.bn_bwd_done = true;
}

static int run_layer_fwd(vp_pixrefer* h, Net& n, Layer& L, const Lane& ln, void* pool_out = nullptr) {
  hipStream_t st = ln.s;
  IgemmArgs a = L.fwd.a;
  a.pool_out = pool_out;
  fill_src(n, L, a.x, n.batch / n.groups, 0, h->es);
  a.Wp = n.packed + L.pk_fwd * h->es;
  Tens& to = n.t[L.out];
  a.Y = L.tapgemm ? L.tap_S : to.y;
  a.bias = L.has_bn || L.tapgemm ? nullptr : n.params + L.b_off;
  a.partial = (float*)ln.scratch;
  a.zeros = h->zeros;
  if (a.kern == CK_SMALLP) {
    SmallPArgs sp = smallp_args(a, L.sp_cnt_fwd, ln);
    sp.mode = L.has_bn ? SP_FWD_BN : SP_PLAIN;
    sp.hi = to.hi ? 1 : 0;
    if (L.has_bn) {
      sp.gamma = n.params + L.gamma_off; sp.beta = n.params + L.beta_off;
      sp.aff_a = to.bn.a; sp.aff_b = to.bn.b; sp.mu = to.bn.mu; sp.rstd = to.bn.rstd;
      sp.out_lrelu = to.need_act[ACT_LRELU] ? to.xa[ACT_LRELU] : nullptr;
      sp.out_relu = to.need_act[ACT_RELU] ? to.xa[ACT_RELU] : nullptr;
      sp.eps = 1e-5f;
    }
    profile_tag((L.scope + ":fwd").c_str());
    VP_HIP_CHECK(launch_smallp(sp, h->bf16, st));
    if (!L.has_bn && (to.need_act[ACT_LRELU] || to.need_act[ACT_RELU]))
      VP_HIP_CHECK(launch_act_apply(to.y, nullptr, nullptr, to.C, (n.batch / n.groups) * to.H * to.W, (size_t)to.N * to.H * to.W,
                                    to.xa[ACT_LRELU], to.xa[ACT_RELU], h->bf16, st));
    return VP_OK;
  }
  bool fused_stats = false;
  int stat_chunks = 0;
  if (L.has_bn && a.kern == CK_DC256 && n.groups == 1) {
    stat_chunks = 2 * conv_dc256_grid(a);
    a.bn_part = ln.bn_partial; a.bn_tpg = 1 << 30; a.bn_nchunk = stat_chunks;
    fused_stats = true;
  } else if (L.has_bn && a.kern == CK_S2C64) {
    const int grid = conv_s2c64_grid(a);
    if ((size_t)n.groups * grid * 2 * to.C <= (size_t)1024 * 2 * 512 && n.groups <= 32) {
      stat_chunks = grid;
      a.bn_part = ln.bn_partial; a.bn_tpg = (n.batch / n.groups) * conv_s2c64_tiles_per_image(a); a.bn_nchunk = grid;
// ... 340 lines not shown
      const int k = ti.pool;
      if (h->pool_codes_written && h->pool_fuse_ok[k]) {
        h->pool_dz_stale[k] = true;
        h->pool_bwd_fused = true;
      } else if (h->pool_codes_written) VP_HIP_CHECK(launch_maxpool_bwd_code(h->vpool_code[k], ti.dz, tc.dz, N, tc.H, tc.W, tc.C, bf, ln.s));
      else VP_HIP_CHECK(launch_maxpool_bwd(xin, ti.dz, tc.dz, N, tc.H, tc.W, tc.C, bf, ln.s));
    }
  }
  return VP_OK;
}

}

extern "C" {

static bool g_phase_marks = false;
static bool g_phase_detail = false;
void vp_phase_marks_enable(int on) { g_phase_marks = on != 0; g_phase_detail = on > 1; }
static void phase_mark(vp_pixrefer* h, hipStream_t st, int idx) {
  if (!g_phase_marks || idx >= 64) return;
  if (!h->marks_made) { for (int i = 0; i < 64; ++i) (void)hipEventCreate(&h->mark[i]); h->marks_made = true; }
  (void)hipEventRecord(h->mark[idx], st);
  if (idx + 1 > h->nmark) h->nmark = idx + 1;
}
float vp_pixrefer_mark_ms(vp_pixrefer_t* h, int from, int to) {
  if (!h || !h->marks_made || from < 0 || to < 0 || from >= 64 || to >= 64) return -1.f;
  float t = -1.f;
  if (hipEventSynchronize(h->mark[to]) != hipSuccess || hipEventElapsedTime(&t, h->mark[from], h->mark[to]) != hipSuccess) { (void)hipGetLastError(); return -1.f; }
  return t;
}
int vp_pixrefer_phase_ms(vp_pixrefer_t* h, float* ms, int cap) {
  if (!h || !ms) return 0;
  int n = 0;
  for (int i = 0; i + 1 < (h->nmark < 8 ? h->nmark : 8) && n < cap; ++i) {
    float t = 0.f;
    if (hipEventSynchronize(h->mark[i + 1]) != hipSuccess || hipEventElapsedTime(&t, h->mark[i], h->mark[i + 1]) != hipSuccess) {
      (void)hipGetLastError();
      break;
    }
    ms[n++] = t;
  }
  return n;
}
int vp_version(void) { return 100; }
const char* vp_last_error(void) { return g_err; }

static Net* manifest_net(const vp_pixrefer_desc* d, int which, vp_pixrefer* tmp) {
  if (which == 0) { build_generator(tmp->G, d->batch, d->height, d->ngf); return &tmp->G; }
  if (which == 1) { build_discriminator(tmp->D, d->batch, d->height, d->ndf); return &tmp->D; }
  if (which == 2) { build_vgg(tmp->V, d->batch, d->height); return &tmp->V; }
  return nullptr;
}

size_t vp_pixrefer_param_count(const vp_pixrefer_desc* d, int which) {
  if (!valid_desc(d)) return 0;
  vp_pixrefer tmp{};
  Net* n = manifest_net(d, which, &tmp);
  return n ? n->nparams : 0;
}

int vp_pixrefer_param_info(const vp_pixrefer_desc* d, int which, int index, char* name, int name_cap,
                           size_t* offset, int* ndim, int64_t shape[4]) {
  if (!valid_desc(d)) return VP_ERR_ARG;
  vp_pixrefer tmp{};
  Net* n = manifest_net(d, which, &tmp);
  if (!n || index < 0 || index >= (int)n->manifest.size()) return VP_ERR_ARG;
  const ParamInfo& p = n->manifest[index];
  if (name && name_cap > 0) { strncpy(name, p.name.c_str(), name_cap - 1); name[name_cap - 1] = 0; }
  if (offset) *offset = p.off;
  if (ndim) *ndim = p.ndim;
  if (shape) for (int i = 0; i < 4; ++i) shape[i] = p.shape[i];
  return VP_OK;
}

size_t vp_pixrefer_workspace_bytes(const vp_pixrefer_desc* d) {
  if (!valid_desc(d)) return 0;
  vp_pixrefer* h = new vp_pixrefer{};
  init_handle(h, d);
  const size_t n = carve_all(h, nullptr, 0);
  delete h;
  return n;
}

int vp_pixrefer_validate_plan(const vp_pixrefer_desc* d) {
  if (!valid_desc(d)) return VP_ERR_ARG;
  vp_pixrefer* h = new vp_pixrefer{};
  init_handle(h, d);
  const size_t need = carve_all(h, nullptr, 0);
  std::vector<std::pair<size_t, size_t>> regs;
  char* const base = reinterpret_cast<char*>((uintptr_t)1 << 40);
  carve_all(h, base, need, &regs);
  int rc = VP_OK;
  auto fail = [&](const char* fmt, auto... args) { if (rc == VP_OK) { set_err(fmt, args...); rc = VP_ERR_STATE; } };
  size_t prev_end = 0;
  for (size_t i = 0; i < regs.size(); ++i) {
    if (regs[i].first % 256) fail("region %zu at %zu: not 256-byte aligned", i, regs[i].first);
    if (regs[i].first < prev_end) fail("region %zu at %zu overlaps the previous one (ends %zu)", i, regs[i].first, prev_end);
    prev_end = regs[i].first + regs[i].second;
  }
  if (prev_end + 256 > need + 256 || prev_end > need) fail("carved %zu bytes of a %zu-byte workspace", prev_end, need);
  auto region_of = [&](const void* p, size_t bytes, const char* what) {
    if (!p) { fail("%s: null", what); return; }
    const size_t off = (size_t)((const char*)p - base);
    for (const auto& r : regs)
      if (off >= r.first && off + bytes <= r.first + r.second) return;
    fail("%s: [%zu, +%zu) is not inside a carved region", what, off, bytes);
  };
  const int es = h->es;
  for (Net* n : {&h->G, &h->D, &h->V}) {
    if (n->t.empty()) continue;
    for (const Tens& t : n->t) {
      const std::string nm = t.name;
      if (t.is_f32) continue;
      region_of(t.y, t.elems() * (t.hi ? 4 : es), (nm + ".y").c_str());
      for (int k = 1; k < 3; ++k) if (t.need_act[k]) region_of(t.xa[k], t.elems() * es, (nm + ".xa").c_str());
      if (t.has_bn) {
        const size_t gc = (size_t)n->groups * t.C * sizeof(float);
        for (const float* p : {t.bn.a, t.bn.b, t.bn.mu, t.bn.rstd, t.bn.c1, t.bn.c2, t.bn.c1g, t.bn.c2g}) region_of(p, gc, (nm + ".bn").c_str());
        if (d->training && t.pb_cap) region_of(t.bn.pb, (size_t)n->groups * t.pb_cap * 2 * t.C * sizeof(double), (nm + ".bn.pb").c_str());
        if (d->training && t.pbg_cap) region_of(t.bn.pbg, (size_t)t.pbg_cap * 2 * t.C * sizeof(double), (nm + ".bn.pbg").c_str());
        if ((size_t)n->groups * t.C > (size_t)1024 * 512) fail("%s: %d groups x %d channels exceed the batch-norm partial rows", nm.c_str(), n->groups, t.C);
      }
      if (t.cs_part) region_of(t.cs_part, (size_t)512 * 2 * 64 * sizeof(double), (nm + ".cs_part").c_str());
      if (d->training && !t.is_input) {
        const size_t div = n == &h->V ? 2 : 1;
        region_of(t.dz, t.elems() / div * es, (nm + ".dz").c_str());
        if (t.hi) region_of(t.dz32, t.elems() * 4, (nm + ".dz32").c_str());
        if (n == &h->D) region_of(t.dz2, t.elems() / 3 * es, (nm + ".dz2").c_str());
      }
    }
    region_of(n->packed, n->packed_elems * es, "packed weights");
    region_of(n->d_descs, n->descs.size() * sizeof(PackDesc), "pack descriptors");
    for (const PackDesc& p : n->descs) {
      const size_t pe = (size_t)p.nclass * p.Kpad * p.rows_pad;
      if (p.dst_off + pe > n->packed_elems) fail("pack block [%zu, +%zu) outside the %zu-element packed arena", p.dst_off, pe, n->packed_elems);
      if (p.src_off >= n->nparams) fail("pack source %zu outside the %zu-float parameter arena", p.src_off, n->nparams);
    }
    size_t pend = 0;
    for (const ParamInfo& p : n->manifest) {
      size_t cnt = 1;
      for (int i = 0; i < 4; ++i) cnt *= (size_t)p.shape[i];
      if (p.off != pend) fail("parameter %s at %zu: arena not contiguous (expected %zu)", p.name.c_str(), p.off, pend);
      pend = p.off + cnt;
    }
    if (pend != n->nparams) fail("parameter manifest covers %zu of %zu floats", pend, n->nparams);
    for (const Layer& L : n->l) {
      auto plan_ok = [&](const IgemmPlan& p, const char* what) {
        if (p.partial_bytes > h->scratch_bytes) fail("%s %s: split-K slab %zu > scratch %zu", L.scope.c_str(), what, p.partial_bytes, h->scratch_bytes);
        if (p.a.splitk < 1 || p.a.CoutPad < p.a.Cout) fail("%s %s: splitk %d CoutPad %d", L.scope.c_str(), what, p.a.splitk, p.a.CoutPad);
        if (!conv_kernel_ok(launch_view(p, p.form), h->bf16))
          fail("%s %s: the launch is outside the preconditions of its kernel %s", L.scope.c_str(), what, conv_kernel_name(p.a.kern));
      };
      plan_ok(L.fwd, "fwd");
      if (L.has_fwd_half) plan_ok(L.fwd_half, "fwd_half");
      if (d->training && L.has_pair) plan_ok(L.bwd_pair, "bwd_pair");
      if (d->training)
        for (int s2 = 0; s2 < L.nsrc; ++s2) if (L.need_bwd[s2]) { plan_ok(L.bwd[s2], "bwd"); if (n == &h->D || n == &h->V) plan_ok(L.bwd_alt[s2], "bwd_alt"); }
      if (d->training && n != &h->V && L.wg.partial_bytes > h->scratch_bytes) fail("%s wgrad: slab %zu > scratch %zu", L.scope.c_str(), L.wg.partial_bytes, h->scratch_bytes);
      if (L.tapgemm) { region_of(L.tap_S, (size_t)L.g.N * L.g.Hin * L.g.Win * 16 * 4, "tap_S"); region_of(L.tap_dyS, (size_t)L.g.N * L.g.Hin * L.g.Win * 16 * es, "tap_dyS"); }
    }
  }
  const size_t px = (size_t)d->batch * d->height * d->height;
  region_of(h->gin, px * 8 * es, "gin"); region_of(h->gfg, px * 8 * es, "gfg");
  region_of(h->y4, px * 4 * 4, "y4"); region_of(h->o4, px * 4 * 4, "o4");
  region_of(h->outputs, px * 3 * 4, "outputs"); region_of(h->outputs_fg, px * 3 * 4, "outputs_fg");
  static const char* const lane_scratch[4] = {"scratch", "scratch2", "scratch3", "scratch4"};
// ... 615 lines not shown
```

Measured before the change: 4608 frames/s.

## Add compile-time specialized conv epilogues for common bias/activation/reference forms

Adds template-specialized epilogue policies (bias+relu, raw, relu/lrelu reference product, accumulate) to the patch2/patch3/patch4 implicit-GEMM kernels. A runtime classifier picks a specialized kernel when the launch matches one of these forms. The specialized store pass batches its loads and drops the generic branches. The aim is to cut epilogue instruction and branch overhead in the bf16 conv forward and backward-data launches. It also adds query and test APIs, and it grows the number of kernel instantiations and code size.

```diff
diff --git a/include/vp_hip.h b/include/vp_hip.h
--- a/include/vp_hip.h
+++ b/include/vp_hip.h
@@ -39,6 +39,8 @@
 
 size_t vp_pixrefer_workspace_bytes(const vp_pixrefer_desc* d);
 int vp_pixrefer_validate_plan(const vp_pixrefer_desc* d);
+
+long vp_pixrefer_epilogue_forms(const vp_pixrefer_desc* d, char* buf, size_t cap);
 
 int vp_pixrefer_create(const vp_pixrefer_desc* d, void* workspace, size_t workspace_bytes,
                        float* params_g, float* params_d, const float* params_vgg,
@@ -105,6 +107,21 @@
 int vp_conv_fwd(const vp_conv_desc* d, const void* x, const float* in_scale, const float* in_shift,
                 const float* w, const float* bias, void* y, void* workspace, void* stream);
 int vp_conv_bwd_data(const vp_conv_desc* d, const void* dy, const float* w, void* dx, void* workspace, void* stream);
+
+typedef struct vp_conv_epi {
+  const float* bias;
+  const void* ref;
+  int ref_act;
+  int accumulate;
+  double* bn_part;
+  int bn_groups;
+  const void* bst_y;
+  const void* x2;
+} vp_conv_epi;
+int vp_conv_fwd_epi(const vp_conv_desc* d, const void* x, const float* w, const vp_conv_epi* e, void* y, void* workspace, void* stream);
+int vp_conv_bwd_data_epi(const vp_conv_desc* d, const void* dy, const float* w, const vp_conv_epi* e, void* dx, void* workspace, void* stream);
+int vp_conv_epi_query(const vp_conv_desc* d, int backward, const vp_conv_epi* e, char* buf, size_t cap);
+int vp_conv_epi_stat_rows(const vp_conv_desc* d, int backward, const vp_conv_epi* e);
 size_t vp_conv3x3_c64_bwd_data_pooled_workspace_bytes(const vp_conv_desc* d);
 int vp_conv3x3_c64_bwd_data_pooled(const vp_conv_desc* d, const void* dy_pool, const unsigned char* code, const float* w, const void* ref,
                                    void* dx, void* workspace, int fused, void* stream);
diff --git a/voicepuppet_amd/_lib.py b/voicepuppet_amd/_lib.py
--- a/voicepuppet_amd/_lib.py
+++ b/voicepuppet_amd/_lib.py
@@ -20,6 +20,11 @@
   _fields_ = [("kind", ctypes.c_int), ("n", ctypes.c_int), ("h", ctypes.c_int), ("w", ctypes.c_int),
               ("cin", ctypes.c_int), ("cout", ctypes.c_int), ("ksize", ctypes.c_int), ("stride", ctypes.c_int),
               ("pad", ctypes.c_int), ("dtype", ctypes.c_int), ("in_act", ctypes.c_int), ("out_act", ctypes.c_int)]
+
+
+class ConvEpi(ctypes.Structure):
+  _fields_ = [("bias", ctypes.c_void_p), ("ref", ctypes.c_void_p), ("ref_act", ctypes.c_int), ("accumulate", ctypes.c_int),
+              ("bn_part", ctypes.c_void_p), ("bn_groups", ctypes.c_int), ("bst_y", ctypes.c_void_p), ("x2", ctypes.c_void_p)]
 
 
 class LogMelDesc(ctypes.Structure):
@@ -134,6 +139,7 @@
                                               ctypes.POINTER(ctypes.c_int64)]),
     "vp_pixrefer_workspace_bytes": (ctypes.c_size_t, [ctypes.POINTER(PixReferDesc)]),
     "vp_pixrefer_validate_plan": (ctypes.c_int, [ctypes.POINTER(PixReferDesc)]),
+    "vp_pixrefer_epilogue_forms": (ctypes.c_long, [ctypes.POINTER(PixReferDesc), ctypes.c_char_p, ctypes.c_size_t]),
     "vp_pixrefer_create": (ctypes.c_int, [ctypes.POINTER(PixReferDesc), _P, ctypes.c_size_t, _P, _P, _P, _P, _P, _P,
                                           ctypes.POINTER(_P)]),
     "vp_pixrefer_destroy": (None, [_P]),
@@ -191,6 +197,10 @@
     "vp_conv_workspace_bytes": (ctypes.c_size_t, [ctypes.POINTER(ConvDesc)]),
     "vp_conv_fwd": (ctypes.c_int, [ctypes.POINTER(ConvDesc), _P, _P, _P, _P, _P, _P, _P, _P]),
     "vp_conv_bwd_data": (ctypes.c_int, [ctypes.POINTER(ConvDesc), _P, _P, _P, _P, _P]),
+    "vp_conv_fwd_epi": (ctypes.c_int, [ctypes.POINTER(ConvDesc), _P, _P, ctypes.POINTER(ConvEpi), _P, _P, _P]),
+    "vp_conv_bwd_data_epi": (ctypes.c_int, [ctypes.POINTER(ConvDesc), _P, _P, ctypes.POINTER(ConvEpi), _P, _P, _P]),
+    "vp_conv_epi_query": (ctypes.c_int, [ctypes.POINTER(ConvDesc), ctypes.c_int, ctypes.POINTER(ConvEpi), ctypes.c_char_p, ctypes.c_size_t]),
+    "vp_conv_epi_stat_rows": (ctypes.c_int, [ctypes.POINTER(ConvDesc), ctypes.c_int, ctypes.POINTER(ConvEpi)]),
     "vp_conv_bwd_weight": (ctypes.c_int, [ctypes.POINTER(ConvDesc), _P, _P, _P, _P, _P, _P, _P]),
     "vp_conv3x3_c64_bwd_data_pooled_workspace_bytes": (ctypes.c_size_t, [ctypes.POINTER(ConvDesc)]),
     "vp_conv3x3_c64_bwd_data_pooled": (ctypes.c_int, [ctypes.POINTER(ConvDesc), _P, _P, _P, _P, _P, _P, ctypes.c_int, _P]),
diff --git a/voicepuppet_amd/csrc/conv_dispatch.h b/voicepuppet_amd/csrc/conv_dispatch.h
--- a/voicepuppet_amd/csrc/conv_dispatch.h
+++ b/voicepuppet_amd/csrc/conv_dispatch.h
@@ -28,6 +28,7 @@
 int conv_staging(int kern);
 bool conv_kernel_ok(const IgemmArgs& a, int is_bf16);
 int pick_conv_kernel(const IgemmArgs& v, int is_bf16);
+int conv_epi_form(const IgemmArgs& a, int is_bf16, int cfg);
 hipError_t launch_igemm(const IgemmArgs& a, int is_bf16, int cfg, hipStream_t st);
 
 }
diff --git a/voicepuppet_amd/csrc/conv_dispatch.hip b/voicepuppet_amd/csrc/conv_dispatch.hip
--- a/voicepuppet_amd/csrc/conv_dispatch.hip
+++ b/voicepuppet_amd/csrc/conv_dispatch.hip
@@ -13,6 +13,8 @@
 hipError_t launch_igemm_patch2(Args, int is_bf16, int bc, int bp, hipStream_t);
 bool patch3_eligible(Args, int is_bf16); hipError_t launch_igemm_patch3(Args, int is_bf16, int bc, int bp, hipStream_t);
 bool patch4_eligible(Args, int is_bf16); hipError_t launch_igemm_patch4(Args, hipStream_t);
+int patch3_epi_form(Args, int is_bf16, int bc, int bp);
+int patch2_epi_form(Args, int is_bf16, int bc, int bp);
 hipError_t launch_igemm_smallp(Args, int is_bf16, hipStream_t);
 bool conv_s2c64_eligible(Args, int is_bf16); hipError_t launch_conv_s2c64(Args, hipStream_t);
 bool conv_cin8_eligible(Args, int is_bf16); hipError_t launch_conv_cin8(Args, hipStream_t);
@@ -70,6 +72,14 @@
   return fam;
 }
 
+int conv_epi_form(const IgemmArgs& a, int is_bf16, int cfg) {
+  int bc, bp;
+  igemm_tile(cfg, &bc, &bp);
+  if (a.kern == CK_PATCH3 || a.kern == CK_PATCH4) return patch3_epi_form(a, is_bf16, bc, bp);
+  if (a.kern == CK_PATCH2) return patch2_epi_form(a, is_bf16, bc, bp);
+  return EPI_GENERIC;
+}
+
 hipError_t launch_igemm(const IgemmArgs& a, int is_bf16, int cfg, hipStream_t st) {
   if (!conv_kernel_ok(a, is_bf16)) {
     set_err("launch_igemm: the arguments are outside the preconditions of the plan's kernel %s (%s, %d x %d x %d -> %d channels)",
diff --git a/voicepuppet_amd/csrc/conv_ops.h b/voicepuppet_amd/csrc/conv_ops.h
--- a/voicepuppet_amd/csrc/conv_ops.h
+++ b/voicepuppet_amd/csrc/conv_ops.h
@@ -3,6 +3,7 @@
 #include <string.h>
 
 #include "launch.h"
+#include "vp_hip.h"
 
 namespace vp {
 
@@ -121,6 +122,36 @@
 inline int& dc64_knob() { static int v = 1; return v; }
 inline int& s2c64_knob() { static int v = 512; return v; }
 inline int& s2c64_pair_knob() { static int v = 1; return v; }
+inline int& epi_spec_knob() { static int v = 1; return v; }
+
+enum EpiForm {
+  EPI_GENERIC = 0,
+  EPI_BIAS_RELU,
+  EPI_RAW,
+  EPI_RELU_REF,
+  EPI_LRELU_REF,
+  EPI_LRELU_REF_ACC,
+};
+inline const char* epi_form_name(int f) {
+  static const char* const names[] = {"generic", "bias_relu", "raw", "relu_ref", "lrelu_ref", "lrelu_ref_acc"};
+  return f >= 0 && f < 6 ? names[f] : "?";
+}
+inline int epi_form_of(const IgemmArgs& a, int is_bf16) {
+  if (!epi_spec_knob() || !is_bf16 || a.y_f32 || a.split_c || a.splitk > 1 || a.pool_out || a.bst_y2 || a.ref_a || a.ref_b || a.xa_lrelu || a.xa_relu ||
+      a.colsum_part || a.ldY % 8 || a.Cout % 8)
+    return EPI_GENERIC;
+  if (!a.ref) {
+    if (a.accumulate) return EPI_GENERIC;
+    if (a.bias && a.out_act == VP_ACT_RELU) return EPI_BIAS_RELU;
+    if (!a.bias && a.out_act == VP_ACT_NONE) return EPI_RAW;
+    return EPI_GENERIC;
+  }
+  if (a.bias || a.out_act != VP_ACT_NONE) return EPI_GENERIC;
+  if (a.ref_act == VP_ACT_RELU) return a.accumulate ? EPI_GENERIC : EPI_RELU_REF;
+  if (a.ref_act == VP_ACT_LRELU) return a.accumulate ? EPI_LRELU_REF_ACC : EPI_LRELU_REF;
+  return EPI_GENERIC;
+}
+
 constexpr int PATCH_MIN_BLOCKS_DEFAULT = 192;
 inline int& patch_minblk_knob() { static int v = PATCH_MIN_BLOCKS_DEFAULT; return v; }
 
@@ -298,6 +329,20 @@
   v.x.act = f.x_act;
   if (f.stats) v.bn_part = (double*)set;
   return v;
+}
+
+inline int epi_stat_chunks(const IgemmPlan& p, int batch, int groups) {
+  const IgemmArgs& a = p.a;
+  const int fam = conv_staging(a.kern);
+  if (a.splitk != 1 || fam == CK_SMALLP || fam == CK_S2C64 || batch % groups) return 0;
+  int bc, bp;
+  igemm_tile(p.cfg, &bc, &bp);
+  const int pg = (batch / groups) * a.Hg * a.Wg;
+  if (!(fam || groups == 1 || pg % bp == 0)) return 0;
+  int pth = 16, ptw = 16;
+  patch_tile_hw(bp, &pth, &ptw);
+  const int tpg = fam ? (batch / groups) * ((a.Hg + pth - 1) / pth) * ((a.Wg + ptw - 1) / ptw) : (pg + bp - 1) / bp;
+  return a.nclass * tpg;
 }
 
 enum { FAM_SMALLP = 1, FAM_PATCH = 2, FAM_PATCH2 = 4, FAM_S2C64 = 8, FAM_ALL = 15 };
diff --git a/voicepuppet_amd/csrc/conv_patch2.hip b/voicepuppet_amd/csrc/conv_patch2.hip
--- a/voicepuppet_amd/csrc/conv_patch2.hip
+++ b/voicepuppet_amd/csrc/conv_patch2.hip
@@ -10,7 +10,7 @@
 template <typename T, int WC, int WP, int TC, int TP, int TH, int TW>
 using Patch2Geom = PatchGeom<T, WC, WP, TC, TP, TH, TW, 1, 4>;
 
-template <typename T, int WC, int WP, int TC, int TP, int TH, int TW, int STATS, int OCC, bool TWOSRC>
+template <typename T, int WC, int WP, int TC, int TP, int TH, int TW, int STATS, int OCC, bool TWOSRC, typename EPI = EpiGeneric>
 __global__ __launch_bounds__(512, OCC) void igemm_patch2_kernel(const IgemmArgs a) {
   using G = Patch2Geom<T, WC, WP, TC, TP, TH, TW>;
   constexpr int NSTW = G::NSTW, NSTEP = 8;
@@ -114,13 +114,27 @@
   }
   asm volatile("s_waitcnt vmcnt(0)" ::: "memory");
 
-  staged_epilogue<T, TC, TP, G::BC, G::BP, G::NPASS, G::NT, STATS>(a, PatchTilePix<TW, true>{a, n, y0, x0, a.o0h[cls], a.o0w[cls]}, c_base, blkA0, blkB0,
+  staged_epilogue<T, TC, TP, G::BC, G::BP, G::NPASS, G::NT, STATS, 0, false, EPI>(a, PatchTilePix<TW, true>{a, n, y0, x0, a.o0h[cls], a.o0w[cls]}, c_base, blkA0, blkB0,
                                                                    acc, smem, tile.bt, cls);
+}
+
+int patch2_epi_form(const IgemmArgs& a, int is_bf16, int bc, int bp) {
+  if (a.kern != CK_PATCH2 || bc != 128 || bp != 256) return EPI_GENERIC;
+  const int f = epi_form_of(a, is_bf16);
+  const bool two = a.x.C[1] > 0;
+  if (f == EPI_LRELU_REF || f == EPI_LRELU_REF_ACC) return !two && a.bst_y && a.bn_part ? f : EPI_GENERIC;
+  return EPI_GENERIC;
 }
 
 template <typename T, int WC, int WP, int TC, int TP, int TH, int TW, int OCC>
 static hipError_t launch_patch2_t(const IgemmArgs& b, hipStream_t st) {
   const bool two = b.x.C[1] > 0;
+  if constexpr (sizeof(T) == 2 && TC == 4) {
+    using G = Patch2Geom<T, WC, WP, TC, TP, TH, TW>;
+    const int form = patch2_epi_form(b, 1, G::BC, G::BP);
+    if (form == EPI_LRELU_REF) return launch_patch_grid<G>(igemm_patch2_kernel<T, WC, WP, TC, TP, TH, TW, 2, OCC, false, EpiLreluRef>, b, b.nclass, st);
+    if (form == EPI_LRELU_REF_ACC) return launch_patch_grid<G>(igemm_patch2_kernel<T, WC, WP, TC, TP, TH, TW, 2, OCC, false, EpiLreluRefAcc>, b, b.nclass, st);
+  }
   const bool bst = b.bst_y != nullptr;
   if (bst && two) return hipErrorInvalidValue;
   auto kern = bst ? igemm_patch2_kernel<T, WC, WP, TC, TP, TH, TW, 2, OCC, false>
diff --git a/voicepuppet_amd/csrc/conv_patch3.hip b/voicepuppet_amd/csrc/conv_patch3.hip
--- a/voicepuppet_amd/csrc/conv_patch3.hip
+++ b/voicepuppet_amd/csrc/conv_patch3.hip
@@ -18,7 +18,7 @@
 template <typename T, int WC, int WP, int TC, int TP, int TH, int TW, int NSTW, int KW>
 using Patch3Geom = PatchGeom<T, WC, WP, TC, TP, TH, TW, KW - 1, NSTW>;
 
-template <typename T, int WC, int WP, int TC, int TP, int TH, int TW, int STATS, int OCC, int NSTW = 3, int KW = 3>
+template <typename T, int WC, int WP, int TC, int TP, int TH, int TW, int STATS, int OCC, int NSTW = 3, int KW = 3, typename EPI = EpiGeneric>
 __global__ __launch_bounds__(512, OCC) void igemm_patch3_kernel(const IgemmArgs a) {
   using G = Patch3Geom<T, WC, WP, TC, TP, TH, TW, NSTW, KW>;
   constexpr int E = G::E, KC = G::KC, NW = G::NW, LA = NSTW - 1;
@@ -126,11 +126,37 @@
 #else
   constexpr int NPASS16 = 0;
 #endif
-  if (!(VP_P3_ABL & 8) || acc[0][0][0] == 1.2345f) staged_epilogue<T, TC, TP, G::BC, G::BP, G::NPASS, G::NT, STATS, NPASS16>(a, PatchTilePix<TW>{a, n, y0, x0}, c_base, blkA0, blkB0, acc, smem, tile.bt, 0);
+  if (!(VP_P3_ABL & 8) || acc[0][0][0] == 1.2345f) staged_epilogue<T, TC, TP, G::BC, G::BP, G::NPASS, G::NT, STATS, NPASS16, false, EPI>(a, PatchTilePix<TW>{a, n, y0, x0}, c_base, blkA0, blkB0, acc, smem, tile.bt, 0);
+}
+
+int patch3_epi_form(const IgemmArgs& a, int is_bf16, int bc, int bp) {
+  const int f = epi_form_of(a, is_bf16);
+  if (a.bst_y || (a.bn_part && f != EPI_RAW)) return EPI_GENERIC;
+  if (a.kern == CK_PATCH4) return (f == EPI_RAW && a.bn_part) || f == EPI_LRELU_REF ? f : EPI_GENERIC;
+  if (a.kern != CK_PATCH3) return EPI_GENERIC;
+  if (bc == 256 && bp == 128) return f == EPI_BIAS_RELU || f == EPI_RELU_REF ? f : EPI_GENERIC;
+  return EPI_GENERIC;
+}
+
+template <typename EPI, int STATS, int WC, int WP, int TC, int TP, int TH, int TW, int OCC, int NSTW, int KW>
+static hipError_t launch_patch3_epi(const IgemmArgs& b, hipStream_t st) {
+  return launch_patch_grid<Patch3Geom<bf16, WC, WP, TC, TP, TH, TW, NSTW, KW>>(igemm_patch3_kernel<bf16, WC, WP, TC, TP, TH, TW, STATS, OCC, NSTW, KW, EPI>, b, 1, st);
 }
 
 template <typename T, int WC, int WP, int TC, int TP, int TH, int TW, int OCC, int NSTW = 3, int KW = 3>
 static hipError_t launch_patch3_t(const IgemmArgs& b, hipStream_t st) {
+  if constexpr (sizeof(T) == 2 && OCC == 4 && (KW == 4 || (NSTW == 3 && TC == 8 && TP == 2))) {
+#define VP_P3_EPI(EPI, STATS) launch_patch3_epi<EPI, STATS, WC, WP, TC, TP, TH, TW, OCC, NSTW, KW>(b, st)
+    const int form = patch3_epi_form(b, 1, WC * TC * 16, TH * TW);
+    if constexpr (KW == 4) {
+      if (form == EPI_RAW) return VP_P3_EPI(EpiRaw, 1);
+      if (form == EPI_LRELU_REF) return VP_P3_EPI(EpiLreluRef, 0);
+    } else {
+      if (form == EPI_BIAS_RELU) return VP_P3_EPI(EpiBiasRelu, 0);
+      if (form == EPI_RELU_REF) return VP_P3_EPI(EpiReluRef, 0);
+    }
+#undef VP_P3_EPI
+  }
   auto kern = b.bn_part ? igemm_patch3_kernel<T, WC, WP, TC, TP, TH, TW, 1, OCC, NSTW, KW> : igemm_patch3_kernel<T, WC, WP, TC, TP, TH, TW, 0, OCC, NSTW, KW>;
   if (b.bst_y) {
     if constexpr (KW == 4) kern = igemm_patch3_kernel<T, WC, WP, TC, TP, TH, TW, 2, OCC, NSTW, KW>;
diff --git a/voicepuppet_amd/csrc/igemm_device.h b/voicepuppet_amd/csrc/igemm_device.h
--- a/voicepuppet_amd/csrc/igemm_device.h
+++ b/voicepuppet_amd/csrc/igemm_device.h
@@ -60,6 +60,123 @@
   for (int np = 1; np <= WP; np *= 2)
     if ((BP / np) * (BC * 2 + 16) + (BP / np) * 8 <= ring_bytes) return np;
   return WP;
+}
+
+template <bool BIAS_, int OUT_ACT_, int REF_, int REF_ACT_, bool ACCUM_>
+struct EpiSpec {
+  static constexpr bool GENERIC = false, BIAS = BIAS_, ACCUM = ACCUM_;
+  static constexpr int OUT_ACT = OUT_ACT_, REF = REF_, REF_ACT = REF_ACT_;
+  static_assert(OUT_ACT == ACT_NONE || OUT_ACT == ACT_RELU || OUT_ACT == ACT_LRELU, "straight-line output activations");
+  static_assert(REF == 0 || (REF == 1 && (REF_ACT == ACT_RELU || REF_ACT == ACT_LRELU)), "reference product: none, or act' of an activated reference");
+};
+struct EpiGeneric {
+  static constexpr bool GENERIC = true, BIAS = false, ACCUM = false;
+  static constexpr int OUT_ACT = ACT_NONE, REF = 0, REF_ACT = ACT_NONE;
+};
+using EpiBiasRelu = EpiSpec<true, ACT_RELU, 0, ACT_NONE, false>;
+using EpiRaw = EpiSpec<false, ACT_NONE, 0, ACT_NONE, false>;
+using EpiReluRef = EpiSpec<false, ACT_NONE, 1, ACT_RELU, false>;
+using EpiLreluRef = EpiSpec<false, ACT_NONE, 1, ACT_LRELU, false>;
+using EpiLreluRefAcc = EpiSpec<false, ACT_NONE, 1, ACT_LRELU, true>;
+
+__device__ __forceinline__ void epi_landed(uint4& r) { asm volatile("" : "+v"(r.x), "+v"(r.y), "+v"(r.z), "+v"(r.w)); }
+template <typename T, typename EPI, int BC, int RP, int NT, int STATS, int NG>
+__device__ __forceinline__ void epi_store_pass(const IgemmArgs& a, const long long* otab, const char* smem, int c_base, int tid, float (&bv)[8],
+                                               float (&gs0)[NG], float (&gs1)[NG]) {
+#pragma clang fp contract(off)
+  static_assert(sizeof(T) == 2, "bf16 outputs");
+  constexpr int PITCH = BC * 4 + 16, CG = BC / 8, NI = RP * CG / NT, PS = NT / CG;
+  static_assert(NT % CG == 0 && (RP * CG) % NT == 0 && NI >= 1, "a thread keeps one channel group and has whole items");
+  constexpr int NSTREAM = (EPI::REF != 0) + EPI::ACCUM + (STATS == 2);
+  constexpr int NB = (NSTREAM >= 3 && NI % 4 == 0) ? NI / 4 : (NSTREAM >= 2 && NI % 2 == 0) ? NI / 2 : NI;
+  const int cgp = tid % CG, p0 = tid / CG, c0 = c_base + cgp * 8;
+  const bool cok = c0 < a.Cout;
+  if constexpr (EPI::BIAS) {
+#pragma unroll
+    for (int e = 0; e < 8; ++e) asm volatile("" : "+v"(bv[e]));
+  }
+#pragma unroll
+  for (int i0 = 0; i0 < NI; i0 += NB) {
+    bool ok[NB];
+    size_t off[NB];
+    uint4 rb[EPI::REF ? NB : 1], eb[EPI::ACCUM ? NB : 1], yb[STATS == 2 ? NB : 1];
+#pragma unroll
+    for (int i = 0; i < NB; ++i) {
+      const long long ot = otab[p0 + (i0 + i) * PS];
+      ok[i] = cok && ot >= 0;
+      off[i] = ok[i] ? (size_t)(ot >> 8) + c0 : 0;
+    }
+    if constexpr (EPI::REF != 0) {
+#pragma unroll
+      for (int i = 0; i < NB; ++i) rb[i] = *reinterpret_cast<const uint4*>(reinterpret_cast<const bf16*>(a.ref) + off[i]);
+    }
+    if constexpr (EPI::ACCUM) {
+#pragma unroll
+      for (int i = 0; i < NB; ++i) eb[i] = *reinterpret_cast<const uint4*>(reinterpret_cast<const bf16*>(a.Y) + off[i]);
+    }
+    if constexpr (STATS == 2) {
+#pragma unroll
+      for (int i = 0; i < NB; ++i) yb[i] = *reinterpret_cast<const uint4*>(reinterpret_cast<const bf16*>(a.bst_y) + off[i]);
+    }
+    if constexpr (EPI::REF != 0) {
+#pragma unroll
+      for (int i = 0; i < NB; ++i) epi_landed(rb[i]);
+    }
+    if constexpr (STATS == 2) {
+#pragma unroll
+      for (int i = 0; i < NB; ++i) epi_landed(yb[i]);
+    }
+    if constexpr (EPI::ACCUM) {
+#pragma unroll
+      for (int i = 0; i < NB; ++i) epi_landed(eb[i]);
+    }
+#pragma unroll
+    for (int i = 0; i < NB; ++i) {
+      const char* row = smem + (p0 + (i0 + i) * PS) * PITCH + cgp * 32;
+      const float4 v0 = *reinterpret_cast<const float4*>(row), v1 = *reinterpret_cast<const float4*>(row + 16);
+      float v[8] = {v0.x, v0.y, v0.z, v0.w, v1.x, v1.y, v1.z, v1.w};
+      if constexpr (EPI::BIAS) {
+#pragma unroll
+        for (int e = 0; e < 8; ++e) v[e] += bv[e];
+      }
+      if constexpr (EPI::OUT_ACT != ACT_NONE) {
+#pragma unroll
+        for (int e = 0; e < 8; ++e) v[e] = act_apply(EPI::OUT_ACT, v[e]);
+      }
+      if constexpr (EPI::REF != 0) {
+        float z[8];
+        Elem<bf16>::unpack(rb[i], z);
+#pragma unroll
+        for (int e = 0; e < 8; ++e) v[e] *= act_grad(EPI::REF_ACT, z[e]);
+      }
+      if constexpr (EPI::ACCUM) {
+        float y[8];
+        Elem<bf16>::unpack(eb[i], y);
+#pragma unroll
+        for (int e = 0; e < 8; ++e) v[e] += y[e];
+      }
+      const uint4 pk = Elem<bf16>::pack(v);
+      if (ok[i]) {
+        unsigned* yp = reinterpret_cast<unsigned*>(reinterpret_cast<bf16*>(a.Y) + off[i]);
+#ifdef VP_NT_STORE
+        __builtin_nontemporal_store(pk.x, yp); __builtin_nontemporal_store(pk.y, yp + 1);
+        __builtin_nontemporal_store(pk.z, yp + 2); __builtin_nontemporal_store(pk.w, yp + 3);
+#else
+        *reinterpret_cast<uint4*>(yp) = pk;
+#endif
+        if constexpr (STATS == 2) {
+          float fy[8], sv[8];
+          Elem<bf16>::unpack(yb[i], fy);
+          Elem<bf16>::unpack(pk, sv);
+#pragma unroll
+          for (int e = 0; e < 8; ++e) {
+            gs0[e] += sv[e];
+            gs1[e] = fmaf(sv[e], fy[e], gs1[e]);
+          }
+        }
+      }
+    }
+  }
 }
 
 template <typename T, bool DUAL = false>
@@ -137,10 +254,11 @@
   return m > 0.f ? 1u + best : 0u;
 }
 
-template <typename T, int TC, int TP, int BC, int BP, int NPASS, int NT, int STATS = 0, int NPASS16 = 0, bool DUAL = false, typename PixFn>
+template <typename T, int TC, int TP, int BC, int BP, int NPASS, int NT, int STATS = 0, int NPASS16 = 0, bool DUAL = false, typename EPI = EpiGeneric, typename PixFn>
 __device__ __forceinline__ void staged_epilogue(const IgemmArgs& a, const PixFn& pixfn, int c_base, int blkA0, int blkB0,
                                                 f32x4 (&acc)[TC][TP], char* smem, int pt = 0, int cls = 0) {
-  if constexpr (NPASS16 > 0 && sizeof(T) == 2 && STATS == 0) {
+  static_assert(EPI::GENERIC || (sizeof(T) == 2 && !DUAL), "specialised forms: bf16, one output");
+  if constexpr (NPASS16 > 0 && sizeof(T) == 2 && STATS == 0 && EPI::GENERIC) {
     if (!a.ref && !a.accumulate && !a.y_f32 && (a.out_act == ACT_NONE || a.out_act == ACT_RELU)) {
       constexpr int PITCHB = BC * 2 + 16, CGB = BC / 8, RPB = BP / NPASS16;
       static_assert(RPB % (TP * 16) == 0, "a wave's pixel rows must fall into one pass");
@@ -255,6 +373,12 @@
     for (int e = 0; e < 8; ++e) { gs0[e] = 0.f; gs1[e] = 0.f; }
     if (yb && c0 < ct) gy = reinterpret_cast<const T*>(yb);
   }
+  float bv[8] = {0.f, 0.f, 0.f, 0.f, 0.f, 0.f, 0.f, 0.f};
+  if constexpr (!EPI::GENERIC && EPI::BIAS) {
+    const int c0 = c_base + (tid % CG) * 8, cb = c0 < a.Cout ? c0 : 0;
+#pragma unroll
+    for (int e = 0; e < 8; ++e) bv[e] = a.bias[cb + e];
+  }
 #pragma unroll
   for (int ps = 0; ps < NPASS; ++ps) {
     __syncthreads();
@@ -280,6 +404,9 @@
         bsum += x; bsq = fmaf(x, x, bsq);
       }
     }
+    if constexpr (!EPI::GENERIC) {
+      epi_store_pass<T, EPI, BC, RP, NT, STATS>(a, otab, smem, c_base, tid, bv, gs0, gs1);
+    } else {
     bool store_y = true;
     if constexpr (pix_has_pool<PixFn>::value) store_y = !(a.pool_out != nullptr && a.pool_only);
     if (store_y)
@@ -379,6 +506,7 @@
         }
       }
     }
+    }
   }
   if constexpr (STATS == 2) {
     __syncthreads();
diff --git a/voicepuppet_amd/csrc/ops_api.hip b/voicepuppet_amd/csrc/ops_api.hip
--- a/voicepuppet_amd/csrc/ops_api.hip
+++ b/voicepuppet_amd/csrc/ops_api.hip
@@ -96,6 +96,7 @@
       {"thin_blocks_dcout8", &thin_blocks_knob(1), TUNE_POSITIVE},
       {"thin_blocks_cout4", &thin_blocks_knob(2), TUNE_POSITIVE},
       {"thin_blocks_cin8", &thin_blocks_knob(3), TUNE_POSITIVE},
+      {"epi_spec", &epi_spec_knob(), TUNE_PLAIN},
   };
   if (!strcmp(key, "phase_marks")) { vp_phase_marks_enable(value); return VP_OK; }
   for (const TuneRow& r : rows) {
@@ -192,6 +193,80 @@
   return VP_OK;
 }
 
+static int conv_epi_op(const char* who, const vp_conv_desc* d, int backward, const void* x, const float* w, const vp_conv_epi* e, void* y, void* workspace,
+                       void* stream, char* query, size_t cap, int* rows = nullptr) {
+  if (!conv_desc_ok(d) || !e || d->in_act != ACT_NONE || (!query && !rows && (!x || !w || !y || !workspace)) || (backward && (d->cout < 8 || (d->cout & (d->cout - 1)))) ||
+      (e->bn_part && (e->bn_groups < 1 || d->n % e->bn_groups || (backward != 0) != (e->bst_y != nullptr))) || (e->bst_y && !e->bn_part) || (e->ref && !backward) ||
+      (e->x2 && (backward || d->cin % 2))) {
+    set_err("%s: bad argument", who);
+    return VP_ERR_ARG;
+  }
+  const int bf = d->dtype == VP_BF16, es = bf ? 2 : 4;
+  hipStream_t st = (hipStream_t)stream;
+  const ConvGeomX g = geom_of(d);
+  IgemmPlan p;
+  LaunchForm f;
+  if (backward) {
+    p = plan_bwd_data(g, 0, 0, d->cin, d->cin, d->cin, bf);
+    p.a.ref_act = e->ref_act;
+    f.ref = e->ref != nullptr; f.ref_act = e->ref_act;
+    plan_kernel(p, d->cin, bf, d->cout, 0, FAM_SMALLP | FAM_PATCH | FAM_PATCH2, f);
+  } else {
+    p = plan_fwd(g, 0, bf);
+    p.a.out_act = d->out_act;
+    f.bias = e->bias != nullptr; f.stats = e->bn_part != nullptr;
+    const int c1 = e->x2 ? d->cin / 2 : 0;
+    plan_kernel(p, g.Cout, bf, d->cin - c1, c1, FAM_SMALLP | FAM_PATCH | FAM_PATCH2 | (d->out_act == ACT_NONE ? FAM_S2C64 : 0), f);
+  }
+  IgemmArgs a = p.a;
+  set_single_src(a.x, x, backward ? d->cout : d->cin, nullptr, nullptr, ACT_NONE, 0);
+  if (e->x2) { a.x.ptr[1] = e->x2; a.x.C[0] = a.x.C[1] = d->cin / 2; }
+  a.Y = y; a.bias = e->bias;
+  a.ref = e->ref; a.ref_act = e->ref_act; a.accumulate = e->accumulate ? 1 : 0;
+  if (rows) {
+    *rows = a.kern == CK_SMALLP || e->bn_groups < 1 || d->n % e->bn_groups ? 0 : epi_stat_chunks(p, d->n, e->bn_groups);
+    return VP_OK;
+  }
+  if (e->bn_part) {
+    const int chunks = epi_stat_chunks(p, d->n, e->bn_groups);
+    if (chunks <= 0 || a.kern == CK_SMALLP || a.y_f32 || a.ldY % 8 || a.Cout % 8 || (e->bst_y && a.kern != CK_IGEMM && a.kern != CK_PATCH4 && a.kern != CK_PATCH2)) { set_err("%s: the launch has no statistics epilogue", who); return VP_ERR_ARG; }
+    a.bn_part = e->bn_part; a.bn_tpg = chunks / a.nclass; a.bn_nchunk = chunks;
+    a.bst_y = e->bst_y;
+    a.ref_group_n = d->n / e->bn_groups;
+  }
+  if (query) {
+    int bc, bp;
+    igemm_tile(p.cfg, &bc, &bp);
+    IgemmArgs v = a;
+    v.zeros = &v;
+    snprintf(query, cap, "%s_%dx%d %s", conv_kernel_name(a.kern), bc, bp, epi_form_name(conv_epi_form(v, bf, p.cfg)));
+    return VP_OK;
+  }
+  if ((a.kern == CK_SMALLP || a.splitk > 1) && (e->ref || e->accumulate || e->bn_part)) { set_err("%s: few-pixel and K-split launches take no reference / accumulation / statistics here", who); return VP_ERR_ARG; }
+  char* ws = (char*)workspace;
+  VP_HIP_CHECK(launch_pack_weights_one(p.pack, w, ws, bf, st));
+  a.Wp = ws;
+  a.partial = (float*)(ws + align256(p.pack_elems * es));
+  a.zeros = zero_page(ws, align256(p.pack_elems * es) + p.partial_bytes, st);
+  if (a.kern == CK_SMALLP) a.sp_cnt = smallp_counter_page(ws, align256(p.pack_elems * es) + p.partial_bytes, a, st);
+  VP_HIP_CHECK(launch_igemm(a, bf, p.cfg, st));
+  return VP_OK;
+}
+int vp_conv_fwd_epi(const vp_conv_desc* d, const void* x, const float* w, const vp_conv_epi* e, void* y, void* workspace, void* stream) {
+  return conv_epi_op("vp_conv_fwd_epi", d, 0, x, w, e, y, workspace, stream, nullptr, 0);
+}
+int vp_conv_bwd_data_epi(const vp_conv_desc* d, const void* dy, const float* w, const vp_conv_epi* e, void* dx, void* workspace, void* stream) {
+  return conv_epi_op("vp_conv_bwd_data_epi", d, 1, dy, w, e, dx, workspace, stream, nullptr, 0);
+}
+int vp_conv_epi_query(const vp_conv_desc* d, int backward, const vp_conv_epi* e, char* buf, size_t cap) {
+  if (!buf || cap < 64) { set_err("vp_conv_epi_query: bad argument"); return VP_ERR_ARG; }
+  return conv_epi_op("vp_conv_epi_query", d, backward, nullptr, nullptr, e, nullptr, nullptr, nullptr, buf, cap);
+}
+int vp_conv_epi_stat_rows(const vp_conv_desc* d, int backward, const vp_conv_epi* e) {
+  int rows = 0;
+  return conv_epi_op("vp_conv_epi_stat_rows", d, backward, nullptr, nullptr, e, nullptr, nullptr, nullptr, nullptr, 0, &rows) == VP_OK ? rows : 0;
+}
+
 static bool pooled_desc_ok(const vp_conv_desc* d) {
   return conv_desc_ok(d) && d->kind == 0 && d->ksize == 3 && d->stride == 1 && d->pad == 1 && d->dtype == VP_BF16 && d->cin == d->cout &&
          (d->cin == 64 || d->cin == 128) && d->h % 4 == 0 && d->w % 16 == 0 && d->h >= 16;
diff --git a/voicepuppet_amd/csrc/plan_pixrefer.hip b/voicepuppet_amd/csrc/plan_pixrefer.hip
--- a/voicepuppet_amd/csrc/plan_pixrefer.hip
+++ b/voicepuppet_amd/csrc/plan_pixrefer.hip
@@ -275,7 +275,6 @@
   add_layer(n, P, "conv3/conv3_3", 0, 3, 1, 1, {c32}, 256, 256, false, ACT_NONE, ACT_RELU, "weights", "biases");
 }
 
-static int epi_stat_chunks(const IgemmPlan& p, int batch, int groups);
 static bool first_layer_shape(int bf16, const Net& n, const Layer& L) {
   if (!bf16 || L.has_bn || L.tapgemm || L.out_act != ACT_NONE) return false;
   const Tens& to = n.t[L.out];
@@ -651,20 +650,6 @@
   return tw == 16 && th % 2 == 0;
 }
 
-static int epi_stat_chunks(const IgemmPlan& p, int batch, int groups) {
-  const IgemmArgs& a = p.a;
-  const int fam = conv_staging(a.kern);
-  if (a.splitk != 1 || fam == CK_SMALLP || fam == CK_S2C64 || batch % groups) return 0;
-  int bc, bp;
-  igemm_tile(p.cfg, &bc, &bp);
-  const int pg = (batch / groups) * a.Hg * a.Wg;
-  if (!(fam || groups == 1 || pg % bp == 0)) return 0;
-  int pth = 16, ptw = 16;
-  patch_tile_hw(bp, &pth, &ptw);
-  const int tpg = fam ? (batch / groups) * ((a.Hg + pth - 1) / pth) * ((a.Wg + ptw - 1) / ptw) : (pg + bp - 1) / bp;
-  return a.nclass * tpg;
-}
-
 static int run_layer_fwd_half(vp_pixrefer* h, Net& n, Layer& L, int half, const Lane& ln, void* pool_out = nullptr, bool pool_only = false,
                               unsigned char* pool_code = nullptr) {
   IgemmArgs a = L.fwd_half.a;
@@ -1171,6 +1156,56 @@
   return n;
 }
 
+long vp_pixrefer_epilogue_forms(const vp_pixrefer_desc* d, char* buf, size_t cap) {
+  if (!valid_desc(d)) return VP_ERR_ARG;
+  vp_pixrefer* h = new vp_pixrefer{};
+  init_handle(h, d);
+  carve_all(h, nullptr, 0);
+  std::string out;
+  static const char* const net_names[3] = {"G", "D", "V"};
+  int ni = 0;
+  for (Net* n : {&h->G, &h->D, &h->V}) {
+    const char* nn = net_names[ni++];
+    if (n->t.empty()) continue;
+    for (const Layer& L : n->l) {
+      auto show = [&](const IgemmPlan& p, const char* what, bool stats, bool grad) {
+        LaunchForm f = p.form;
+        if (stats) f.stats = true;
+        const bool can_sum = grad && !p.a.split_c && (p.a.kern == CK_IGEMM || p.a.kern == CK_PATCH4 || (p.a.kern == CK_PATCH2 && p.a.x.C[1] == 0));
+        for (int var = 0; var < (grad ? (can_sum ? 4 : 2) : 1); ++var) {
+          const int acc = var & 1, sums = var >> 1;
+          IgemmArgs v = launch_view(p, f);
+          v.accumulate = acc;
+          if (v.split_c) v.accumulate2 = acc;
+          if (sums) { v.bst_y = v.Y; v.bn_part = (double*)v.Y; }
+          int bc, bp;
+          igemm_tile(p.cfg, &bc, &bp);
+          char line[256];
+          snprintf(line, sizeof(line), "%s/%s:%s%s %s_%dx%d %s\n", nn, L.scope.c_str(), what, acc ? (sums ? "+acc+sums" : "+acc") : (sums ? "+sums" : ""), conv_kernel_name(v.kern), bc, bp,
+                   epi_form_name(conv_epi_form(v, h->bf16, p.cfg)));
+          out += line;
+        }
+      };
+      show(L.fwd, "fwd", L.fwd_stats, false);
+      if (L.has_fwd_half) show(L.fwd_half, "fwd_half", false, false);
+      if (!d->training) continue;
+      if (L.has_pair) show(L.bwd_pair, "bwd_pair", false, true);
+      for (int s2 = 0; s2 < L.nsrc; ++s2) {
+        if (!L.need_bwd[s2]) continue;
+        show(L.bwd[s2], "bwd", false, true);
+        if (n == &h->D || n == &h->V) show(L.bwd_alt[s2], "bwdG", false, true);
+      }
+    }
+  }
+  delete h;
+  if (buf && cap) {
+    const size_t k = out.size() < cap - 1 ? out.size() : cap - 1;
+    memcpy(buf, out.data(), k);
+    buf[k] = 0;
+  }
+  return (long)out.size();
+}
+
 int vp_pixrefer_validate_plan(const vp_pixrefer_desc* d) {
   if (!valid_desc(d)) return VP_ERR_ARG;
   vp_pixrefer* h = new vp_pixrefer{};
```

New measurement: 4709 frames/s (median of 6 runs). +2.2%, better.
